# NingZhang1/pyscf_isdf

Hardware: AMD Instinct MI355X
Metric: isdf_build_plus_get_jk_wall_time (lower is better)
Workload: dtype f64

## Files before the change

include/mi355_isdf.h:

```cpp
#ifndef MI355_ISDF_H
#define MI355_ISDF_H

#include <stdint.h>

#ifdef __cplusplus
extern "C" {
#endif

typedef struct isdf_ctx* isdf_handle;

#define ISDF_OK 0
#define ISDF_ERR_ARG 1
#define ISDF_ERR_HIP 2
#define ISDF_ERR_LIB 3
#define ISDF_ERR_NUM 4

int isdf_abi_version(void);

int isdf_create(int device_id, isdf_handle* out);
int isdf_destroy(isdf_handle h);
int isdf_set_stream(isdf_handle h, void* hip_stream);
const char* isdf_last_error(isdf_handle h);
int64_t isdf_workspace_bytes(isdf_handle h);
int isdf_release_workspace(isdf_handle h);
// ... 65 lines not shown

int isdf_fit_prepare(isdf_handle h, const double* d_ao, int nao, int64_t ld,
                     const int64_t* d_ip, int P, double reg_rel, double* d_aoP, double* d_chol,
                     double* reg_used);
int isdf_fit_apply(isdf_handle h, const double* d_chol, const double* d_aoP, int P, int nao,
                   const double* d_ao, int64_t ng, int64_t ld, int forward_only,
                   double* d_theta, int64_t ldt);
int isdf_fit_prepare_cplx(isdf_handle h, const double* d_ao, int nao, int nh, int64_t ld,
                          const int64_t* d_ip, int P, double reg_rel, double* d_aoP, double* d_chol,
                          double* reg_used);
int isdf_fit_apply_cplx(isdf_handle h, const double* d_chol, const double* d_aoP, int P, int nao, int nh,
                        const double* d_ao, int64_t ng, int64_t ld, int forward_only,
                        double* d_theta, int64_t ldt);
int isdf_fit_global(isdf_handle h, const double* d_ao, int nao, int64_t ngrids, int64_t ld,
                    const int64_t* d_ip, int P, double reg_rel, double* d_theta, int64_t ldt,
                    double* d_aoP, double* reg_used);

int isdf_gather_aoP(isdf_handle h, const double* d_ao, int nao, int64_t ld, const int64_t* d_ip, int P,
                    double* d_aoP);
int isdf_gram_sq(isdf_handle h, const double* d_aoP, int P, int nao, int nh, double* d_A);
int isdf_pair_gram_rows(isdf_handle h, const double* d_aoP, int P, int nao, int nh, const double* d_ao,
                        int64_t ng, int64_t ld, double* d_B, int64_t ldb);
int isdf_block_chol(isdf_handle h, const double* d_A, int P, int nblk, const int32_t* blk_off,
                    double shift_rel, double* d_D, double* shift_used);
int isdf_block_solve(isdf_handle h, const double* d_D, int P, int nblk, const int32_t* blk_off, int side,
                     int trans, double* d_X, int64_t n, int64_t ldx);
int isdf_block_invert(isdf_handle h, const double* d_D, int P, int nblk, const int32_t* blk_off, double* d_Dinv);
int isdf_block_apply(isdf_handle h, const double* d_Dinv, int64_t ldd, int nblk, const int32_t* blk_off,
                     double* d_X, int64_t n, int64_t ldx);
int isdf_pair_rows_block_apply(isdf_handle h, const double* d_aoP, int P, int nao, const double* d_ao, int64_t ng,
                               int64_t ld, const double* d_Dinv, int64_t ldd, int nblk, const int32_t* blk_off,
                               double* d_B, int64_t ldb);
int isdf_pair_rows_squared(isdf_handle h, const double* d_aoP, int rows, int nao, const double* d_ao, int64_t ng,
                           int64_t ld, int* squared);
int isdf_pair_rows_frontier(isdf_handle h, const double* d_aoP, int nnew, int nao, const double* d_ao, int64_t ng,
                            int64_t ld, int squared, const double* d_Dinv, int64_t ldd, int nblk, const int32_t* blk_off,
                            double* d_B, int64_t ldb, int have);

int isdf_gram_prod(isdf_handle h, const double* d_aoP, int P, int nao, const double* d_psiP, int nocc, double* d_A);
int isdf_pair_prod_rows(isdf_handle h, const double* d_aoP, int P, int nao, const double* d_psiP, int nocc,
                        const double* d_ao, int64_t ld, const double* d_psi, int64_t ldpsi, int64_t ng,
                        double* d_B, int64_t ldb);
int isdf_factor_solve_half(isdf_handle h, const double* d_fac, int P, int backward, double* d_X, int64_t n, int64_t ldx);
int isdf_gram_prod_cplx(isdf_handle h, const double* d_aoP, int P, int nao, int nh, const double* d_psiP, int npsi, int npsi_h,
                        double* d_A);
int isdf_pair_prod_rows_cplx(isdf_handle h, const double* d_aoP, int P, int nao, int nh, const double* d_psiP, int npsi,
                             int npsi_h, const double* d_ao, int64_t ld, const double* d_psi, int64_t ldpsi, int64_t ng,
                             double* d_B, int64_t ldb);

int isdf_shift_diag(isdf_handle h, double* d_A, int P, double shift_rel);
int isdf_chol_inplace(isdf_handle h, double* d_A, int P, double shift_rel, double* d_scratch, double* reg_used);

int isdf_factor_solve(isdf_handle h, const double* d_fac, int P, double* d_X, int64_t n, int64_t ldx);

int isdf_bj_probe_vectors(isdf_handle h, double* d_T, int n, const double* d_fac, const double* d_D, int P,
                          int nblk, const int32_t* blk_off);
int isdf_rows_combine(isdf_handle h, const double* d_E, int n, int64_t ldE, int rows, const double* d_Y,
                      int64_t ng, int64_t ldy, double* d_F, int64_t ldf, int accumulate);

int isdf_bj_probe_rows(isdf_handle h, double* d_T, int n, const double* d_fac, const double* d_D, int P, int nblk,
                       const int32_t* blk_off, const double* d_Yp, int64_t ng, int64_t ldy, double* d_F, int64_t ldf);

int isdf_gather_T(isdf_handle h, const double* d_L, int k, int64_t ldL, const int64_t* d_piv,
                  double* d_T);
int isdf_W_from_factor(isdf_handle h, const double* d_F, int P, int kind, double* d_M, int64_t ldm);

int isdf_coulomb_W(isdf_handle h, const double* d_theta, int P, int64_t ldt,
                   const int32_t mesh[3], const double a[9],
                   int row0, int nrows, int batch, int upper_only, double* d_W, int64_t ldw);
int isdf_coulG_half(isdf_handle h, const int32_t mesh[3], const double a[9], double* d_out);
int isdf_spectral_supported(isdf_handle h, const int32_t mesh[3], int batch, int* ok);
int isdf_spectral_rows(isdf_handle h, const double* d_in, int nrows, int64_t ld, const int32_t mesh[3], const int32_t* d_idx,
                       const double* d_scale, int npts, int batch, double* d_out, int64_t ldx);
int isdf_coulomb_rows(isdf_handle h, const double* d_in, int nrows, int64_t ld,
                      const int32_t mesh[3], const double a[9], int batch, double* d_out, int64_t ldo);
int isdf_symmetrize_upper(isdf_handle h, double* d_W, int P, int64_t ldw);
int isdf_symmetrize_mean(isdf_handle h, double* d_W, int P, int64_t ldw, int antisymmetric);

int isdf_get_j(isdf_handle h, const double* d_ao, int nao, int64_t ngrids, int64_t ld,
               const int32_t mesh[3], const double a[9],
               const double* d_dm, int nset, double* d_vj);
int isdf_rho(isdf_handle h, const double* d_ao, int nao, int64_t ng, int64_t ld,
             const double* d_dm, int nset, double* d_rho, int64_t ldrho);
int isdf_coulomb_potential(isdf_handle h, double* d_rho_inout, int nset, int64_t ldrho,
                           const int32_t mesh[3], const double a[9]);
int isdf_vj_from_vR(isdf_handle h, const double* d_ao, int nao, int64_t ng, int64_t ld,
                    const double* d_vR, int nset, int64_t ldv, double* d_vj);

int isdf_get_k_exact(isdf_handle h, const double* d_ao, int nao, int64_t ngrids, int64_t ld,
                     const double* d_C, int nocc, const int32_t mesh[3], const double a[9],
                     int i0, int ni, int max_rows, double* d_vk);

int isdf_get_k(isdf_handle h, const double* d_aoP, int P, int nao,
               const double* d_W, int64_t ldw, int row0, int nrows,
               const double* d_dm, int nset, double* d_vk);

int isdf_coulG_q(isdf_handle h, const int32_t mesh[3], const double a[9], const double q[3], int wrap_around,
                 double omega, double* d_out);

int isdf_coulomb_Wq(isdf_handle h, const double* d_theta, int P, int64_t ldt, const int32_t mesh[3],
                    const double* d_coulG, double weight, int row0, int nrows, int batch,
                    int upper_only, double* d_Wre, double* d_Wim, int64_t ldw);
int isdf_symmetrize_hermitian(isdf_handle h, double* d_Wre, double* d_Wim, int P, int64_t ldw);
int isdf_finish_Wq(isdf_handle h, const double* d_Wre, const double* d_Wim, int P, int64_t ldw,
                   const double* d_phase, double* d_Wc);
int isdf_get_k_pair(isdf_handle h, const double* d_A1, const double* d_A2, const double* d_D2,
                    const double* d_Wq, int P, int nao, double scale, double* d_vk);

int isdf_get_k_exact_kpt(isdf_handle h, const double* d_u1r, const double* d_u1i, int nao, int64_t ld1,
                         const double* d_m2r, const double* d_m2i, int nocc, int64_t ld2, const int32_t mesh[3],
                         const double* d_coulG, double weight, int i0, int ni, int max_rows, double* d_vk_re,
                         double* d_vk_im);

int isdf_coulomb_rows_q(isdf_handle h, const double* d_rows, int nrows, int64_t ld, const int32_t mesh[3],
                        const double* d_coulG, double* d_re, double* d_im);
int isdf_nyquist_spectra(isdf_handle h, const double* d_rows, int nrows, int64_t ld, const int32_t mesh[3], int axis,
                         double* d_re, double* d_im);
int isdf_zhadamard_planes(isdf_handle h, double* d_Ar, double* d_Ai, int64_t lda, const double* d_Br, const double* d_Bi,
                          int64_t ldb, int rows, int64_t cols);
int isdf_rho_k(isdf_handle h, const double* d_ur, const double* d_ui, int nao, int64_t ng, int64_t ld,
               const double* d_DTr, const double* d_DTi, double scale, double* d_rho);
int isdf_vj_k(isdf_handle h, const double* d_ur, const double* d_ui, int nao, int64_t ng, int64_t ld,
              const double* d_vR, double* d_vj_re, double* d_vj_im);

int isdf_pp_local_potential(isdf_handle h, int natm, const double* coords, const double* pp_par,
                            const int32_t mesh[3], const double a[9], double* d_vlocR);
int isdf_pp_projector_overlaps(isdf_handle h, const int32_t* atm, int natm, const int32_t* bas, int nbas,
                               const double* env, int nenv, const double* coords, const double kpt[3],
                               const int32_t* proj_tab, const double* proj_rl, int nproj,
                               const int32_t mesh[3], const double a[9], double* d_out);

int isdf_pp_local_force(isdf_handle h, const double* d_rho, int nset, int64_t ldrho, int natm, const double* coords,
                        const double* pp_par, const int32_t mesh[3], const double a[9], double* d_out);
int isdf_pp_projector_overlaps_ip(isdf_handle h, const int32_t* atm, int natm, const int32_t* bas, int nbas,
                                  const double* env, int nenv, const double* coords, const double kpt[3],
                                  const int32_t* proj_tab, const double* proj_rl, int nproj,
                                  const int32_t mesh[3], const double a[9], double* d_out);
int isdf_rowdot3(isdf_handle h, int M, int64_t K, double alpha, const double* d_A, int64_t lda, int64_t astride, const double* d_s,
                 const double* d_B, int64_t ldb, int accumulate, double* d_out, int64_t ldo);

int isdf_gemm_nn(isdf_handle h, int M, int64_t N, int K, double alpha, const double* d_A, int64_t lda, const double* d_B,
                 int64_t ldb, double beta, double* d_C, int64_t ldc);
int isdf_hadamard_rows(isdf_handle h, double* d_X, int64_t ldx, const double* d_Y, int64_t ldy, int rows, int64_t cols);

int isdf_uniform_grid(isdf_handle h, const int32_t mesh[3], const double a[9], double* d_coords_soa);
int isdf_rho_pair(isdf_handle h, const double* d_aoA, int nA, const double* d_aoB, int nB, int64_t ng, int64_t ld,
                  const double* d_dm, int nset, double* d_rho, int64_t ldrho);
int isdf_mg_embed_density(isdf_handle h, const double* d_field, int nset, const int32_t mesh_sub[3], double scale,
                          double* d_spec, const int32_t mesh[3], int accumulate);
int isdf_mg_restrict_potential(isdf_handle h, const double* d_spec, int nset, const int32_t mesh[3],
                               const int32_t mesh_sub[3], double scale, double* d_field);
int isdf_mg_coulomb_kernel(isdf_handle h, double* d_spec, int nset, const int32_t mesh[3], const double a[9]);
int isdf_lda_exchange(isdf_handle h, const double* d_rho, int64_t n, double* d_exc, double* d_vxc);
int isdf_lda_vwn_add(isdf_handle h, const double* d_rho, int64_t n, double* d_exc, double* d_vxc);
int isdf_gga_b88(isdf_handle h, const double* d_rho, const double* d_grad, int64_t gstride, int64_t n, double* d_exc,
                 double* d_vrho, double* d_w, int64_t wstride);
int isdf_xc_fused(isdf_handle h, const double* d_rho, const double* d_grad, int64_t gstride, int64_t n, double c_slater, double c_b88,
                  double c_vwn, int vwn_rpa, double c_lyp, double* d_exc, double* d_vrho, double* d_w, int64_t wstride);
int isdf_gga_lyp_polarised(isdf_handle h, const double* d_rho, const double* d_grad, int64_t gcstride, int64_t sstride, int64_t n,
                           double weight, int accumulate, double* d_ec, double* d_vrho, double* d_w, int64_t wcstride,
                           int64_t osstride);
int isdf_lda_exchange_fxc(isdf_handle h, const double* d_rho, int64_t n, double* d_fxc);
int isdf_lda_vwn_fxc_add(isdf_handle h, const double* d_rho, int64_t n, double* d_fxc);
int isdf_gga_b88_fxc(isdf_handle h, const double* d_rho0, int64_t r0stride, int64_t n, const double* d_rho1, int64_t r1xstride,
                     int64_t r1nstride, int nset, double* d_wv, int64_t wxstride, int64_t wnstride, double* d_fxc, int64_t fstride);
int isdf_xc_fxc_apply(isdf_handle h, int nx, const double* d_fxc, int64_t fxstride, int64_t fystride, int64_t n, const double* d_rho1,
                      int64_t r1xstride, int64_t r1nstride, int nset, double* d_wv, int64_t wxstride, int64_t wnstride, int accumulate);
int isdf_dot(isdf_handle h, const double* d_x, const double* d_y, int64_t n, double* result);

int isdf_pack_table_pm(isdf_handle h, const double* d_tab, const int32_t mesh[3], const int32_t* d_idx, int npts, double scale,
                       double* d_s, double* d_a, int64_t ldx);
int isdf_herm_kscale_nt(isdf_handle h, int M, int N, int64_t K, double alpha, const double* d_A, int64_t lda, const double* d_B,
                        int64_t ldb, const double* d_s, const double* d_a, double beta, double* d_Cre, double* d_Cim, int64_t ldc);

int isdf_gemm_nt(isdf_handle h, int M, int N, int64_t K, double alpha, const double* d_A, int64_t lda,
                 const double* d_B, int64_t ldb, const double* d_kscale, double beta, double* d_C,
                 int64_t ldc);

int isdf_gemm_nt_had3(isdf_handle h, int M, int N, int64_t K, double alpha, const double* d_A, int64_t lda, const double* d_H,
                      int64_t ldh, const double* d_B, int64_t ldb, int64_t bstride, double beta, double* d_C, int64_t ldc,
                      int64_t cstride);

#ifdef __cplusplus
}
#endif
#endif
```

pyscf_isdf_amd/backend.py:

```python
import ctypes
import os
import numpy as np
import torch
from . import lib as _lib

_vp = ctypes.c_void_p


def _np_ptr(a):
    return a.ctypes.data_as(_vp)


class HipBackend:
    name = 'hip-gfx950'

    def __init__(self, device=0):
        if not torch.cuda.is_available():
            raise _lib.IsdfError('no GPU visible to torch; the ISDF path has no CPU fallback')
        self.device = torch.device('cuda', device)
        torch.cuda.set_device(self.device)
        self.handle = _lib.Handle(device)
        if os.environ.get('ISDF_TRSM') == 'subst':
            self.set_option('trsm_substitution', 1)
        if os.environ.get('ISDF_OWN_FFT') in ('0', '1', '2'):
# ... 330 lines not shown
                         len(blk_off) - 1, _np_ptr(blk_off))

    def rows_combine(self, E, Y, F, accumulate=False):
        self._stream()
        assert E.stride(1) == 1 and Y.stride(1) == 1 and F.stride(1) == 1 and E.shape[1] == Y.shape[0]
        self.handle.call('isdf_rows_combine', self._p(E), E.shape[0], E.stride(0), E.shape[1], self._p(Y), Y.shape[1],
                         Y.stride(0), self._p(F), F.stride(0), int(bool(accumulate)))

    def gather_T(self, L, k, piv, T):
        self._stream()
        assert T.is_contiguous() and T.shape == (k, k)
        self.handle.call('isdf_gather_T', self._p(L), int(k), L.stride(0), self._p(piv), self._p(T))

    def W_from_factor(self, F, kind, M):
        self._stream()
        assert F.is_contiguous()
        self.handle.call('isdf_W_from_factor', self._p(F), M.shape[0], int(kind), self._p(M), M.stride(0))

    def fit_global(self, ao, ngrids, ip, reg_rel, theta, aoP):
        self._stream()
        assert ip.dtype == torch.int64 and aoP.is_contiguous()
        reg = ctypes.c_double(0.0)
        self.handle.call('isdf_fit_global', self._p(ao), ao.shape[0], int(ngrids), ao.stride(0), self._p(ip),
                         ip.numel(), float(reg_rel), self._p(theta), theta.stride(0), self._p(aoP), ctypes.byref(reg))
        return reg.value

    def coulomb_W(self, theta, mesh, a, row0, nrows, batch, W, upper_only=False):
        self._stream()
        mesh = np.ascontiguousarray(mesh, dtype=np.int32)
        a = np.ascontiguousarray(a, dtype=np.float64)
        self.handle.call('isdf_coulomb_W', self._p(theta), theta.shape[0], theta.stride(0), _np_ptr(mesh), _np_ptr(a),
                         int(row0), int(nrows), int(batch), int(bool(upper_only)), self._p(W), W.stride(0))

    def coulomb_rows(self, rows, mesh, a, batch, out=None):
        self._stream()
        out = rows if out is None else out
        mesh = np.ascontiguousarray(mesh, dtype=np.int32)
        a = np.ascontiguousarray(a, dtype=np.float64)
        self.handle.call('isdf_coulomb_rows', self._p(rows), rows.shape[0], rows.stride(0), _np_ptr(mesh), _np_ptr(a),
                         int(batch), self._p(out), out.stride(0))

    def spectral_supported(self, mesh, batch=512):
        ok = ctypes.c_int(0)
        mesh = np.ascontiguousarray(mesh, dtype=np.int32)
        self.handle.call('isdf_spectral_supported', _np_ptr(mesh), int(batch), ctypes.byref(ok))
        return bool(ok.value)

    def coulG_half(self, mesh, a):
        self._stream()
        mesh = np.ascontiguousarray(mesh, dtype=np.int32)
        a = np.ascontiguousarray(a, dtype=np.float64)
        out = self.empty((int(mesh[0]) * int(mesh[1]) * (int(mesh[2]) // 2 + 1),))
        self.handle.call('isdf_coulG_half', _np_ptr(mesh), _np_ptr(a), self._p(out))
        return self.to_host(out).reshape(int(mesh[0]), int(mesh[1]), int(mesh[2]) // 2 + 1)

    def spectral_rows(self, rows, mesh, idx, scale, out, batch=512):
        self._stream()
        mesh = np.ascontiguousarray(mesh, dtype=np.int32)
        assert rows.is_contiguous() and out.stride(1) == 1 and idx.dtype == torch.int32 and out.stride(0) % 2 == 0
        self.handle.call('isdf_spectral_rows', self._p(rows), rows.shape[0], rows.stride(0), _np_ptr(mesh), self._p(idx),
                         self._p(scale), int(idx.numel()), int(batch), self._p(out), out.stride(0))

    def symmetrize_upper(self, W):
        self._stream()
        self.handle.call('isdf_symmetrize_upper', self._p(W), W.shape[0], W.stride(0))

    def symmetrize_mean(self, W, antisymmetric=False):
        self._stream()
        self.handle.call('isdf_symmetrize_mean', self._p(W), W.shape[0], W.stride(0), int(bool(antisymmetric)))

    def get_j(self, ao, ngrids, mesh, a, dm, vj):
        self._stream()
        mesh = np.ascontiguousarray(mesh, dtype=np.int32)
        a = np.ascontiguousarray(a, dtype=np.float64)
        assert dm.is_contiguous() and vj.is_contiguous()
        self.handle.call('isdf_get_j', self._p(ao), ao.shape[0], int(ngrids), ao.stride(0), _np_ptr(mesh), _np_ptr(a),
                         self._p(dm), dm.shape[0], self._p(vj))

    def rho(self, ao, ng, dm, rho):
        self._stream()
        self.handle.call('isdf_rho', self._p(ao), ao.shape[0], int(ng), ao.stride(0), self._p(dm), dm.shape[0],
                         self._p(rho), rho.stride(0))

    def coulomb_potential(self, rho, mesh, a):
        self._stream()
        mesh = np.ascontiguousarray(mesh, dtype=np.int32)
        a = np.ascontiguousarray(a, dtype=np.float64)
        self.handle.call('isdf_coulomb_potential', self._p(rho), rho.shape[0], rho.stride(0), _np_ptr(mesh), _np_ptr(a))

    def vj_from_vR(self, ao, ng, vR, vj):
        self._stream()
        self.handle.call('isdf_vj_from_vR', self._p(ao), ao.shape[0], int(ng), ao.stride(0), self._p(vR), vR.shape[0],
                         vR.stride(0), self._p(vj))

    def get_k(self, aoP, W, row0, nrows, dm, vk):
        self._stream()
        assert aoP.is_contiguous() and dm.is_contiguous() and vk.is_contiguous()
        self.handle.call('isdf_get_k', self._p(aoP), aoP.shape[0], aoP.shape[1], self._p(W), W.stride(0), int(row0),
                         int(nrows), self._p(dm), dm.shape[0], self._p(vk))

    def get_k_exact(self, ao, ngrids, C, mesh, a, i0, ni, max_rows, vk):
        self._stream()
        mesh = np.ascontiguousarray(mesh, dtype=np.int32)
        a = np.ascontiguousarray(a, dtype=np.float64)
        assert C.is_contiguous() and vk.is_contiguous()
        self.handle.call('isdf_get_k_exact', self._p(ao), ao.shape[0], int(ngrids), ao.stride(0), self._p(C), C.shape[1],
                         _np_ptr(mesh), _np_ptr(a), int(i0), int(ni), int(max_rows), self._p(vk))

    def gemm_nn(self, A, B, C, alpha=1.0, beta=0.0):
        self._stream()
        self.handle.call('isdf_gemm_nn', A.shape[0], B.shape[1], A.shape[1], float(alpha), self._p(A), A.stride(0), self._p(B),
                         B.stride(0), float(beta), self._p(C), C.stride(0))

    def hadamard_rows(self, X, Y):
        self._stream()
        self.handle.call('isdf_hadamard_rows', self._p(X), X.stride(0), self._p(Y), Y.stride(0), X.shape[0], X.shape[1])

    def gemm_nt(self, A, B, C, alpha=1.0, beta=0.0, kscale=None):
        self._stream()
        M, K = A.shape
        N = B.shape[0]
        assert B.shape[1] == K and tuple(C.shape) == (M, N) and A.stride(1) == 1 and B.stride(1) == 1 and C.stride(1) == 1
        ks = self._p(kscale) if kscale is not None else _vp(0)
        self.handle.call('isdf_gemm_nt', M, N, K, float(alpha), self._p(A), A.stride(0), self._p(B), B.stride(0), ks,
                         float(beta), self._p(C), C.stride(0))

    def gemm_nt_had3(self, A, H, B3, C3, alpha=1.0, beta=0.0):
        self._stream()
        M, K = A.shape
        N = B3.shape[1]
        assert tuple(B3.shape) == (3, N, K) and tuple(C3.shape) == (3, M, N) and A.stride(1) == 1 and B3.stride(2) == 1 and C3.stride(2) == 1
        assert H is None or (tuple(H.shape) == (M, K) and H.stride(1) == 1)
        self.handle.call('isdf_gemm_nt_had3', M, N, K, float(alpha), self._p(A), A.stride(0), self._p(H) if H is not None else _vp(0),
                         H.stride(0) if H is not None else 0, self._p(B3), B3.stride(1), B3.stride(0), float(beta), self._p(C3),
                         C3.stride(1), C3.stride(0))

    def pack_table_pm(self, table, mesh, idx, scale, s, a):
        self._stream()
        mesh = np.ascontiguousarray(mesh, dtype=np.int32)
        assert idx.dtype == torch.int32 and table.is_contiguous() and table.numel() == int(np.prod(mesh))
        assert s.is_contiguous() and a.is_contiguous() and s.numel() == a.numel()
        self.handle.call('isdf_pack_table_pm', self._p(table), _np_ptr(mesh), self._p(idx), int(idx.numel()), float(scale),
                         self._p(s), self._p(a), int(s.numel()))

    def herm_kscale_nt(self, A, B, s, a, Cre, Cim, alpha=1.0, beta=0.0):
        self._stream()
        M, K = A.shape
        N = B.shape[0]
        assert B.shape[1] == K and tuple(Cre.shape) == (M, N) and tuple(Cim.shape) == (M, N) and Cre.stride() == Cim.stride()
        assert A.stride(1) == 1 and B.stride(1) == 1 and Cre.stride(1) == 1 and s.numel() >= K and a.numel() >= K
        self.handle.call('isdf_herm_kscale_nt', M, N, K, float(alpha), self._p(A), A.stride(0), self._p(B), B.stride(0),
                         self._p(s), self._p(a), float(beta), self._p(Cre), self._p(Cim), Cre.stride(0))

    def uniform_grid(self, mesh, a):
        self._stream()
        mesh = np.ascontiguousarray(mesh, dtype=np.int32)
        a = np.ascontiguousarray(a, dtype=np.float64)
        out = self.empty((3, int(np.prod(mesh))))
        self.handle.call('isdf_uniform_grid', _np_ptr(mesh), _np_ptr(a), self._p(out))
        return out

    def rho_pair(self, aoA, aoB, ng, dm, rho):
        self._stream()
        assert aoA.stride(0) == aoB.stride(0) and aoA.stride(1) == 1 and aoB.stride(1) == 1 and dm.is_contiguous()
        assert tuple(dm.shape[1:]) == (aoA.shape[0], aoB.shape[0])
        self.handle.call('isdf_rho_pair', self._p(aoA), aoA.shape[0], self._p(aoB), aoB.shape[0], int(ng), aoA.stride(0),
                         self._p(dm), dm.shape[0], self._p(rho), rho.stride(0))

    def mg_embed_density(self, field, mesh_sub, scale, spec, mesh, accumulate=True):
        self._stream()
        mesh_sub = np.ascontiguousarray(mesh_sub, dtype=np.int32)
        mesh = np.ascontiguousarray(mesh, dtype=np.int32)
        assert field.is_contiguous() and spec.is_contiguous() and spec.dtype == torch.complex128
        assert field.shape[1] == int(np.prod(mesh_sub)) and spec.shape[1] == int(mesh[0]) * int(mesh[1]) * (int(mesh[2]) // 2 + 1)
        self.handle.call('isdf_mg_embed_density', self._p(field), field.shape[0], _np_ptr(mesh_sub), float(scale), self._p(spec),
                         _np_ptr(mesh), int(bool(accumulate)))

    def mg_restrict_potential(self, spec, mesh, mesh_sub, scale, field):
        self._stream()
        mesh_sub = np.ascontiguousarray(mesh_sub, dtype=np.int32)
        mesh = np.ascontiguousarray(mesh, dtype=np.int32)
        assert field.is_contiguous() and spec.is_contiguous() and spec.dtype == torch.complex128
        assert field.shape[1] == int(np.prod(mesh_sub)) and spec.shape[1] == int(mesh[0]) * int(mesh[1]) * (int(mesh[2]) // 2 + 1)
        self.handle.call('isdf_mg_restrict_potential', self._p(spec), spec.shape[0], _np_ptr(mesh), _np_ptr(mesh_sub), float(scale),
                         self._p(field))

    def mg_coulomb_kernel(self, spec, mesh, a):
        self._stream()
        mesh = np.ascontiguousarray(mesh, dtype=np.int32)
        a = np.ascontiguousarray(a, dtype=np.float64)
        assert spec.is_contiguous() and spec.dtype == torch.complex128
        self.handle.call('isdf_mg_coulomb_kernel', self._p(spec), spec.shape[0], _np_ptr(mesh), _np_ptr(a))

    def lda_exchange(self, rho, exc, vxc):
        self._stream()
        assert rho.is_contiguous() and exc.is_contiguous() and vxc.is_contiguous()
        self.handle.call('isdf_lda_exchange', self._p(rho), rho.numel(), self._p(exc), self._p(vxc))

    def lda_vwn_add(self, rho, exc, vxc):
        self._stream()
        assert rho.is_contiguous() and exc.is_contiguous() and vxc.is_contiguous()
        self.handle.call('isdf_lda_vwn_add', self._p(rho), rho.numel(), self._p(exc), self._p(vxc))

    def gga_b88(self, rho, grad, exc, vrho, w):
        self._stream()
        assert rho.is_contiguous() and exc.is_contiguous() and vrho.is_contiguous() and grad.stride(1) == 1 and w.stride(1) == 1
        self.handle.call('isdf_gga_b88', self._p(rho), self._p(grad), grad.stride(0), rho.numel(), self._p(exc), self._p(vrho),
# ... 203 lines not shown
```

pyscf_isdf_amd/csrc/common.h:

```cpp
#pragma once
#include <hip/hip_runtime.h>
#include <rocblas/rocblas.h>
#include <rocsolver/rocsolver.h>
#include <hipfft/hipfft.h>
#include <cstdint>
#include <cstdio>
#include <cstring>
#include <string>
#include <vector>
#include <map>
#include "../../include/mi355_isdf.h"

struct FftPlan {
  hipfftHandle fwd = 0, bwd = 0;
  size_t work_bytes = 0;
};

struct ProfRec {
  hipEvent_t e0 = nullptr, e1 = nullptr;
};
struct ProfEntry {
  std::vector<ProfRec> recs;
  double work = 0.0;
  double ms = 0.0;
  int64_t launches = 0;
};

struct WsKernel {
  double alpha = 0.0;
  double ak[9] = {0};
  int mesh[3] = {0, 0, 0};
  double maxq[3] = {0, 0, 0};
  const double* vq = nullptr;
};

struct isdf_ctx {
  int profiling = 0;
  std::map<std::string, ProfEntry> prof;
  int device = 0;
  hipStream_t stream = nullptr;
  rocblas_handle blas = nullptr;
  std::string err;
  std::map<std::vector<int>, FftPlan> plans;
  std::map<std::string, std::pair<void*, size_t>> ws;
  int num_cu = 256;
  int trsm_substitution = 0;
  int own_fft = 2;
  int gemm_nn_own = 0;
  int attr_gemm_b = 0, attr_gemm_nn = 0, attr_gram_tri = 0, attr_herm = 0;
  int cand_gram = 1;
  int conv_pipe = 1;
  int conv_sub_rows = 0;
  int gram_pivot_tpb = 256;
  int gram_compact = 1;
  int gram_compact_permille = 875;
  int block_apply_waves = 16;
  int block_apply_reg = 1;
  double coul_omega = 0.0;
  double coul_rc = 0.0;
  int coul_sphere = 0;
  WsKernel wsk;
};

int isdf_fail(isdf_handle h, int code, const char* fmt, ...);
void* isdf_ws(isdf_handle h, const char* name, size_t bytes);
int isdf_get_plan(isdf_handle h, const int32_t mesh[3], int batch, FftPlan** out);
int get_coulG_half(isdf_handle h, const int32_t mesh[3], const double a[9], double extra_scale, double** out);
bool conv_rows_own_supported(const int32_t mesh[3], int nb);
bool conv_rows_q_own_supported(isdf_handle h, const int32_t mesh[3], int nb);
bool spectral_rows_own_supported(isdf_handle h, const int32_t mesh[3], int nb);
int spectral_rows_own(isdf_handle h, const double* d_in, int nb, const int32_t mesh[3], const int32_t* d_idx, const double* d_scale,
                      int npts, double* d_out, int64_t ldx, HIP_vector_type<double, 2u>* zbuf);
int conv_rows_q_own(isdf_handle h, const double* d_in, double* d_re, double* d_im, int nb, const int32_t mesh[3], const double* tab,
                    double2* zhalf, double2* zfull);
int conv_rows_own(isdf_handle h, const double* d_in, double* d_out, int nb, const int32_t mesh[3], const double* cg,
                  double2* zbuf);

#define HIP_TRY(h, expr)                                                                    \
  do {                                                                                      \
    hipError_t e_ = (expr);                                                                 \
    if (e_ != hipSuccess)                                                                   \
      return isdf_fail(h, ISDF_ERR_HIP, "%s:%d %s -> %s", __FILE__, __LINE__, #expr,        \
                       hipGetErrorString(e_));                                              \
  } while (0)
#define BLAS_TRY(h, expr)                                                                   \
  do {                                                                                      \
    rocblas_status s_ = (expr);                                                             \
    if (s_ != rocblas_status_success)                                                       \
      return isdf_fail(h, ISDF_ERR_LIB, "%s:%d %s -> rocblas status %d", __FILE__, __LINE__, \
                       #expr, (int)s_);                                                     \
  } while (0)
#define FFT_TRY(h, expr)                                                                    \
  do {                                                                                      \
    hipfftResult r_ = (expr);                                                               \
    if (r_ != HIPFFT_SUCCESS)                                                               \
      return isdf_fail(h, ISDF_ERR_LIB, "%s:%d %s -> hipfft result %d", __FILE__, __LINE__,  \
                       #expr, (int)r_);                                                     \
  } while (0)
#define KERNEL_CHECK(h) HIP_TRY(h, hipGetLastError())
#define ARG_CHECK(h, cond)                                                                  \
  do {                                                                                      \
    if (!(cond)) return isdf_fail(h, ISDF_ERR_ARG, "%s:%d argument check failed: %s",       \
                                  __FILE__, __LINE__, #cond);                               \
  } while (0)

static inline int64_t cdiv(int64_t a, int64_t b) { return (a + b - 1) / b; }

struct ProfScope {
  isdf_handle h;
  ProfRec rec;
  ProfEntry* ent = nullptr;
  ProfScope(isdf_handle h_, const char* name, double work, int64_t launches = 1) : h(h_) {
    if (!h || !h->profiling) return;
    ent = &h->prof[name];
    ent->work += work;
    ent->launches += launches;
    if (hipEventCreate(&rec.e0) != hipSuccess || hipEventCreate(&rec.e1) != hipSuccess) { ent = nullptr; return; }
    (void)hipEventRecord(rec.e0, h->stream);
  }
  ~ProfScope() {
    if (!ent) return;
    (void)hipEventRecord(rec.e1, h->stream);
    ent->recs.push_back(rec);
  }
};

int gemm_nt_f64(isdf_handle h, int M, int N, int64_t K, double alpha, const double* A, int64_t lda,
                const double* B, int64_t ldb, double beta, double* C, int64_t ldc);
int gemm_nt_f64_scaled(isdf_handle h, int M, int N, int64_t K, double alpha, const double* A, int64_t lda,
                       const double* B, int64_t ldb, const double* kscale, double beta, double* C,
                       int64_t ldc);
int trsm_lower_left(isdf_handle h, bool trans, int m, int64_t n, const double* L, int64_t ldl, double* X, int64_t ldx);
int trsm_lower_right(isdf_handle h, bool trans, int m, int64_t n, const double* L, int64_t ldl, double* X, int64_t ldx);
int block_forward_solve(isdf_handle h, const double* D, int64_t ldd, int nblk, const int32_t* blk_off_host, double* X,
                        int64_t ldx, int64_t n);
int block_apply_inverse(isdf_handle h, const double* Dinv, int64_t ldd, int nblk, const int32_t* blk_off_host, double* X,
                        int64_t ldx, int64_t n, bool square_input = false);
int transpose_rm(isdf_handle h, const double* src, int64_t lds, int64_t rows, int64_t cols, double* dst, int64_t ldd);
int tri_left(isdf_handle h, bool trans, int m, int64_t n, const double* L, int64_t ldl, double* X, int64_t ldx);
int tri_right(isdf_handle h, bool trans, int m, int64_t n, const double* L, int64_t ldl, double* X, int64_t ldx);
bool gemm_nn_f64_supported(isdf_handle h, int64_t M, int64_t N, int64_t K, const double* A, int64_t lda, const double* B,
                           int64_t ldb);
int gemm_nn_f64(isdf_handle h, int64_t M, int64_t N, int64_t K, const double* A, int64_t lda, const double* B, int64_t ldb,
                double* C, int64_t ldc, bool square);
int gemm_rm(isdf_handle h, char opA, char opB, int64_t M, int64_t N, int64_t K, double alpha,
            const double* A, int64_t lda, const double* B, int64_t ldb, double beta, double* C,
            int64_t ldc);

__host__ __device__ inline int64_t gram_tri_row(int64_t r) {
  const int64_t tm = r >> 8;
  return 32768 * tm * (tm + 1) + (r & 255) * ((tm + 1) << 8);
}
static inline int64_t gram_tri_size(int64_t m) { return m > 0 ? gram_tri_row(m - 1) + (((m - 1) >> 8) + 1) * 256 : 0; }
struct GramTriUnit { int blk, tm, tn, pad; };
int gram_tri_blocks(isdf_handle h, const double* X, int64_t ldx, int K, const GramTriUnit* d_units, int64_t nunits,
                    const int64_t* d_blk_off, int64_t row0, const int64_t* d_tri_off, double* S, double flop);
```

pyscf_isdf_amd/csrc/coulomb.hip:

```cpp
#include "common.h"

namespace {

struct Recip { double b[9]; };
__device__ inline double g2_of(int ix, int iy, int iz, int n0, int n1, int n2, const Recip& r) {
  const double fx = (ix < (n0 + 1) / 2) ? ix : ix - n0;
  const double fy = (iy < (n1 + 1) / 2) ? iy : iy - n1;
  const double fz = (iz < (n2 + 1) / 2) ? iz : iz - n2;
  const double gx = fx * r.b[0] + fy * r.b[3] + fz * r.b[6];
  const double gy = fx * r.b[1] + fy * r.b[4] + fz * r.b[7];
  const double gz = fx * r.b[2] + fy * r.b[5] + fz * r.b[8];
  return gx * gx + gy * gy + gz * gz;
}

__device__ inline double range_factor(double g2, double omega) {
  if (omega == 0.0) return 1.0;
  const double e = exp(-0.25 * g2 / (omega * omega));
  return omega > 0.0 ? e : 1.0 - e;
}
__device__ inline double kernel_value(double g2, double omega, double rc) {
  const double fourpi = 4.0 * 3.14159265358979323846;
  if (rc > 0.0) return g2 == 0.0 ? 0.5 * fourpi * rc * rc : fourpi / g2 * (1.0 - cos(sqrt(g2) * rc));
  return g2 == 0.0 ? 0.0 : fourpi / g2 * range_factor(g2, omega);
}
// ... 151 lines not shown
  if (rc) return rc;
  double qf[3];
  for (int i = 0; i < 3; ++i)
    qf[i] = (q[0] * a[3 * i] + q[1] * a[3 * i + 1] + q[2] * a[3 * i + 2]) / (2.0 * 3.14159265358979323846);
  const bool nonzero = fabs(q[0]) + fabs(q[1]) + fabs(q[2]) > 1e-9;
  const int wrap = (wrap_around && nonzero) ? 1 : 0;
  if (wrap)
    for (int i = 0; i < 3; ++i)
      if (fabs(rint(qf[i] / (mesh[i] / 2 + 0.5) * 1e9)) >= 1e9)
        return isdf_fail(h, ISDF_ERR_ARG, "isdf_coulG_q: q lies outside the first FFT box (pyscf/pbc/tools/pbc.py:281)");
  if (!nonzero) qf[0] = qf[1] = qf[2] = 0.0;
  const int64_t G = (int64_t)mesh[0] * mesh[1] * mesh[2];
  hipLaunchKernelGGL(coulG_q_kernel, dim3((unsigned)cdiv(G, 256)), dim3(256), 0, h->stream, d_out, mesh[0], mesh[1],
                     mesh[2], rr, qf[0], qf[1], qf[2], wrap, omega, h->coul_rc, h->wsk);
  KERNEL_CHECK(h);
  return ISDF_OK;
}

static int convolve_rows(isdf_handle h, const double* d_in, double* d_out, int nb, const int32_t mesh[3],
                         const double* cg, double2* zbuf) {
  const int64_t gc = (int64_t)mesh[0] * mesh[1] * (mesh[2] / 2 + 1);
  if (h->own_fft && conv_rows_own_supported(mesh, nb)) return conv_rows_own(h, d_in, d_out, nb, mesh, cg, zbuf);
  FftPlan* plan = nullptr;
  int rc = isdf_get_plan(h, mesh, nb, &plan);
  if (rc) return rc;
  const int64_t Gfull = (int64_t)mesh[0] * mesh[1] * mesh[2];
  ProfScope ps(h, "coulomb_conv_d2z_mul_z2d[byte]", 32.0 * (double)Gfull * nb, 3);
  FFT_TRY(h, hipfftExecD2Z(plan->fwd, (hipfftDoubleReal*)d_in, (hipfftDoubleComplex*)zbuf));
  const int64_t total = gc * nb;
  const unsigned nblocks = (unsigned)std::min<int64_t>(cdiv(total, 256), (int64_t)h->num_cu * 16);
  hipLaunchKernelGGL(mul_half_kernel, dim3(nblocks), dim3(256), 0, h->stream, zbuf, cg, gc, total);
  KERNEL_CHECK(h);
  FFT_TRY(h, hipfftExecZ2D(plan->bwd, (hipfftDoubleComplex*)zbuf, (hipfftDoubleReal*)d_out));
  return ISDF_OK;
}

namespace {
__global__ void mirror_upper_kernel(double* __restrict__ W, int P, int64_t ldw) {
  __shared__ double tile[32][33];
  const int bx = blockIdx.x, by = blockIdx.y;
  if (bx < by) return;
  const int tx = threadIdx.x, ty = threadIdx.y;
  for (int i = ty; i < 32; i += 8) {
    const int r = by * 32 + i, cc = bx * 32 + tx;
    tile[i][tx] = (r < P && cc < P) ? W[(int64_t)r * ldw + cc] : 0.0;
  }
  __syncthreads();
  for (int i = ty; i < 32; i += 8) {
    const int r = bx * 32 + i, cc = by * 32 + tx;
    if (r < P && cc < P && r > cc) W[(int64_t)r * ldw + cc] = tile[tx][i];
  }
}
__global__ void mean_symmetric_kernel(double* __restrict__ W, int P, int64_t ldw, double sign) {
  __shared__ double up[32][33], lo[32][33];
  const int bx = blockIdx.x, by = blockIdx.y;
  if (bx < by) return;
  const int tx = threadIdx.x, ty = threadIdx.y;
  for (int i = ty; i < 32; i += 8) {
    const int r = by * 32 + i, cc = bx * 32 + tx;
    up[i][tx] = (r < P && cc < P) ? W[(int64_t)r * ldw + cc] : 0.0;
    const int r2 = bx * 32 + i, c2 = by * 32 + tx;
    lo[i][tx] = (r2 < P && c2 < P) ? W[(int64_t)r2 * ldw + c2] : 0.0;
  }
  __syncthreads();
  for (int i = ty; i < 32; i += 8) {
    const int r = by * 32 + i, cc = bx * 32 + tx;
    if (r < P && cc < P) W[(int64_t)r * ldw + cc] = 0.5 * (up[i][tx] + sign * lo[tx][i]);
    const int r2 = bx * 32 + i, c2 = by * 32 + tx;
    if (bx != by && r2 < P && c2 < P) W[(int64_t)r2 * ldw + c2] = 0.5 * (lo[i][tx] + sign * up[tx][i]);
  }
}
}

extern "C" int isdf_symmetrize_mean(isdf_handle h, double* d_W, int P, int64_t ldw, int antisymmetric) {
  if (!h) return ISDF_ERR_ARG;
  ARG_CHECK(h, d_W && P > 0 && ldw >= P);
  const unsigned nt = (unsigned)cdiv(P, 32);
  hipLaunchKernelGGL(mean_symmetric_kernel, dim3(nt, nt), dim3(32, 8), 0, h->stream, d_W, P, ldw,
                     antisymmetric ? -1.0 : 1.0);
  KERNEL_CHECK(h);
  return ISDF_OK;
}

extern "C" int isdf_symmetrize_upper(isdf_handle h, double* d_W, int P, int64_t ldw) {
  if (!h) return ISDF_ERR_ARG;
  ARG_CHECK(h, d_W && P > 0 && ldw >= P);
  const unsigned nt = (unsigned)cdiv(P, 32);
  hipLaunchKernelGGL(mirror_upper_kernel, dim3(nt, nt), dim3(32, 8), 0, h->stream, d_W, P, ldw);
  KERNEL_CHECK(h);
  return ISDF_OK;
}

extern "C" int isdf_coulomb_W(isdf_handle h, const double* d_theta, int P, int64_t ldt,
                              const int32_t mesh[3], const double a[9], int row0, int nrows,
                              int batch, int upper_only, double* d_W, int64_t ldw) {
  if (!h) return ISDF_ERR_ARG;
  ARG_CHECK(h, d_theta && mesh && a && d_W && P > 0 && batch > 0 && ldw >= P);
  ARG_CHECK(h, row0 >= 0 && nrows >= 0 && row0 + nrows <= P);
  const int64_t G = (int64_t)mesh[0] * mesh[1] * mesh[2];
  const int64_t gc = (int64_t)mesh[0] * mesh[1] * (mesh[2] / 2 + 1);
  ARG_CHECK(h, ldt == G);
  if (nrows == 0) return ISDF_OK;
  if (batch > nrows) batch = nrows;
  double* cg = nullptr;
  int rc = get_coulG_half(h, mesh, a, 1.0, &cg);
  if (rc) return rc;
  double* V = (double*)isdf_ws(h, "coul_V", sizeof(double) * (size_t)batch * G);
  double2* Z = (double2*)isdf_ws(h, "coul_Z", sizeof(double2) * (size_t)batch * gc);
  if (!V || !Z) return ISDF_ERR_HIP;
  const double det = a[0] * (a[4] * a[8] - a[5] * a[7]) - a[1] * (a[3] * a[8] - a[5] * a[6]) +
                     a[2] * (a[3] * a[7] - a[4] * a[6]);
  const double w = fabs(det) / (double)G;
  for (int r = row0; r < row0 + nrows; r += batch) {
    const int nb = std::min(batch, row0 + nrows - r);
    rc = convolve_rows(h, d_theta + (int64_t)r * ldt, V, nb, mesh, cg, Z);
    if (rc) return rc;
    const int c0 = upper_only ? r : 0;
    rc = gemm_nt_f64(h, nb, P - c0, G, w, V, G, d_theta + (int64_t)c0 * ldt, ldt, 0.0,
                     d_W + (int64_t)r * ldw + c0, ldw);
    if (rc) return rc;
  }
  return ISDF_OK;
}

extern "C" int isdf_coulomb_potential(isdf_handle h, double* d_rho, int nset, int64_t ldrho,
                                      const int32_t mesh[3], const double a[9]) {
  if (!h) return ISDF_ERR_ARG;
  ARG_CHECK(h, d_rho && mesh && a && nset > 0);
  const int64_t G = (int64_t)mesh[0] * mesh[1] * mesh[2];
  const int64_t gc = (int64_t)mesh[0] * mesh[1] * (mesh[2] / 2 + 1);
  ARG_CHECK(h, ldrho == G);
  const double det = a[0] * (a[4] * a[8] - a[5] * a[7]) - a[1] * (a[3] * a[8] - a[5] * a[6]) +
                     a[2] * (a[3] * a[7] - a[4] * a[6]);
  double* cg = nullptr;
  int rc = get_coulG_half(h, mesh, a, fabs(det) / (double)G, &cg);
  if (rc) return rc;
  double2* Z = (double2*)isdf_ws(h, "coul_Z", sizeof(double2) * (size_t)nset * gc);
  if (!Z) return ISDF_ERR_HIP;
  return convolve_rows(h, d_rho, d_rho, nset, mesh, cg, Z);
}

extern "C" int isdf_coulomb_rows(isdf_handle h, const double* d_in, int nrows, int64_t ld,
                                 const int32_t mesh[3], const double a[9], int batch, double* d_out,
                                 int64_t ldo) {
  if (!h) return ISDF_ERR_ARG;
  ARG_CHECK(h, d_in && d_out && mesh && a && nrows >= 0 && batch > 0);
  const int64_t G = (int64_t)mesh[0] * mesh[1] * mesh[2];
  const int64_t gc = (int64_t)mesh[0] * mesh[1] * (mesh[2] / 2 + 1);
  ARG_CHECK(h, ld == G && ldo == G);
  if (nrows == 0) return ISDF_OK;
  if (batch > nrows) batch = nrows;
  double* cg = nullptr;
  int rc = get_coulG_half(h, mesh, a, 1.0, &cg);
  if (rc) return rc;
  double2* Z = (double2*)isdf_ws(h, "coul_Z", sizeof(double2) * (size_t)batch * gc);
  if (!Z) return ISDF_ERR_HIP;
  for (int r = 0; r < nrows; r += batch) {
    const int nb = std::min(batch, nrows - r);
    rc = convolve_rows(h, d_in + (int64_t)r * ld, d_out + (int64_t)r * ldo, nb, mesh, cg, Z);
    if (rc) return rc;
  }
  return ISDF_OK;
}

extern "C" int isdf_coulG_half(isdf_handle h, const int32_t mesh[3], const double a[9], double* d_out) {
  if (!h) return ISDF_ERR_ARG;
  ARG_CHECK(h, mesh && a && d_out);
  double* cg = nullptr;
  int rc = get_coulG_half(h, mesh, a, 1.0, &cg);
  if (rc) return rc;
  const int64_t gc = (int64_t)mesh[0] * mesh[1] * (mesh[2] / 2 + 1);
  HIP_TRY(h, hipMemcpyAsync(d_out, cg, sizeof(double) * gc, hipMemcpyDeviceToDevice, h->stream));
  return ISDF_OK;
}

extern "C" int isdf_spectral_supported(isdf_handle h, const int32_t mesh[3], int batch, int* ok) {
  if (!h) return ISDF_ERR_ARG;
  ARG_CHECK(h, mesh && ok && batch > 0);
  *ok = spectral_rows_own_supported(h, mesh, batch) ? 1 : 0;
  return ISDF_OK;
}

extern "C" int isdf_spectral_rows(isdf_handle h, const double* d_in, int nrows, int64_t ld, const int32_t mesh[3],
                                  const int32_t* d_idx, const double* d_scale, int npts, int batch, double* d_out, int64_t ldx) {
  if (!h) return ISDF_ERR_ARG;
  ARG_CHECK(h, d_in && d_out && mesh && d_idx && d_scale && nrows >= 0 && batch > 0 && npts > 0);
  const int64_t G = (int64_t)mesh[0] * mesh[1] * mesh[2];
  const int64_t gc = (int64_t)mesh[0] * mesh[1] * (mesh[2] / 2 + 1);
  ARG_CHECK(h, ld == G && npts <= gc);
  if (nrows == 0) return ISDF_OK;
  if (batch > nrows) batch = nrows;
  if (!spectral_rows_own_supported(h, mesh, batch))
    return isdf_fail(h, ISDF_ERR_ARG, "isdf_spectral_rows: mesh %d x %d x %d is not covered by the plane FFT", mesh[0], mesh[1], mesh[2]);
  double2* Z = (double2*)isdf_ws(h, "coul_Z", sizeof(double2) * (size_t)batch * gc);
  if (!Z) return ISDF_ERR_HIP;
  for (int r = 0; r < nrows; r += batch) {
    const int nb = std::min(batch, nrows - r);
    int rc = spectral_rows_own(h, d_in + (int64_t)r * ld, nb, mesh, d_idx, d_scale, npts, d_out + (int64_t)r * ldx, ldx, Z);
    if (rc) return rc;
  }
  return ISDF_OK;
}
// ... 1 lines not shown
```

pyscf_isdf_amd/csrc/fft_conv.hip:

```cpp
#include "common.h"
#include <type_traits>

namespace {

constexpr int TPB = 256;
constexpr int MAXSTAGE = 12;

struct Axis {
  int n;
  int nstage;
  int radix[MAXSTAGE];
  const double2* tw;
};

__device__ inline double2 cadd(double2 a, double2 b) { return make_double2(a.x + b.x, a.y + b.y); }
__device__ inline double2 csub(double2 a, double2 b) { return make_double2(a.x - b.x, a.y - b.y); }
__device__ inline double2 cmul(double2 a, double2 b) { return make_double2(a.x * b.x - a.y * b.y, a.x * b.y + a.y * b.x); }
template <int SIGN>
__device__ inline double2 mul_si(double2 a) { return SIGN > 0 ? make_double2(-a.y, a.x) : make_double2(a.y, -a.x); }
template <int SIGN>
__device__ inline double2 twid(const double2* __restrict__ tw, int idx) {
  double2 w = tw[idx];
  if (SIGN > 0) w.y = -w.y;
  return w;
// ... 390 lines not shown
      z = stockham_all<1>(z, (z == x) ? y : x, ax, ZC, M);
    }
  }
  for (int c = threadIdx.x; c < n * ZC; c += TPB) {
    const int e = c / ZC, m = c - e * ZC;
    if (m < M) base[(int64_t)e * es + m] = z[c];
  }
}

template <int SIGN, int ZCT>
__device__ inline void fft_fast(double2* buf, const Axis& ax, int Ls, const double2* tw) {
  fft<SIGN, TPB, 2048 / TPB, true, FixedLines<ZCT>>(buf, ax, Ls, ZCT, tw);
}

template <int ZCT>
__global__ __launch_bounds__(TPB) void z_r2c_fast_kernel(const double* __restrict__ in, double2* __restrict__ out,
                                                         int64_t nlines, Axis ax) {
  extern __shared__ double2 lds[];
  const int n = ax.n, nh = n / 2 + 1;
  constexpr int Ls = ZCT + 1;
  double2* x = lds;
  double2* tw = lds + n * Ls;
  for (int k = threadIdx.x; k < n; k += TPB) tw[k] = ax.tw[k];
  const int64_t line0 = (int64_t)blockIdx.x * 2 * ZCT;
  const int nl = (int)min((int64_t)2 * ZCT, nlines - line0);
  const double* src = in + line0 * n;
  const float inv_n = 1.0f / (float)n;
  for (int c = threadIdx.x; c < 2 * ZCT * n; c += TPB) {
    const int l = (int)(((float)c + 0.5f) * inv_n), e = c - l * n;
    const double v = (l < nl) ? src[c] : 0.0;
    ((double*)(x + e * Ls + (l >> 1)))[l & 1] = v;
  }
  __syncthreads();
  fft_fast<-1, ZCT>(x, ax, Ls, tw);
  double2* dstc = out + line0 * nh;
  const float inv_nh = 1.0f / (float)nh;
  for (int c = threadIdx.x; c < nl * nh; c += TPB) {
    const int l = (int)(((float)c + 0.5f) * inv_nh), k = c - l * nh;
    const int m = l >> 1;
    const double2 zk = x[k * Ls + m];
    const double2 zn = x[(k == 0 ? 0 : n - k) * Ls + m];
    double2 r;
    if ((l & 1) == 0) r = make_double2(0.5 * (zk.x + zn.x), 0.5 * (zk.y - zn.y));
    else r = make_double2(0.5 * (zk.y + zn.y), -0.5 * (zk.x - zn.x));
    dstc[c] = r;
  }
}

template <int ZCT>
__global__ __launch_bounds__(TPB) void z_c2r_fast_kernel(const double2* __restrict__ in, double* __restrict__ out,
                                                         int64_t nlines, Axis ax) {
  extern __shared__ double2 lds[];
  const int n = ax.n, nh = n / 2 + 1;
  constexpr int Ls = ZCT + 1;
  double2* x = lds;
  double2* tw = lds + n * Ls;
  for (int k = threadIdx.x; k < n; k += TPB) tw[k] = ax.tw[k];
  const int64_t line0 = (int64_t)blockIdx.x * 2 * ZCT;
  const int nl = (int)min((int64_t)2 * ZCT, nlines - line0);
  const int M = (nl + 1) / 2;
  const double2* src = in + line0 * nh;
  const float inv_nh = 1.0f / (float)nh;
  for (int c = threadIdx.x; c < M * nh; c += TPB) {
    const int m = (int)(((float)c + 0.5f) * inv_nh), k = c - m * nh;
    double2 a = src[(int64_t)(2 * m) * nh + k];
    double2 b = (2 * m + 1 < nl) ? src[(int64_t)(2 * m + 1) * nh + k] : make_double2(0.0, 0.0);
    const bool selfconj = (k == 0) || (2 * k == n);
    if (selfconj) { a.y = 0.0; b.y = 0.0; }
    x[k * Ls + m] = make_double2(a.x - b.y, a.y + b.x);
    if (!selfconj) x[(n - k) * Ls + m] = make_double2(a.x + b.y, -a.y + b.x);
  }
  __syncthreads();
  fft_fast<1, ZCT>(x, ax, Ls, tw);
  double* dst = out + line0 * n;
  const float inv_n = 1.0f / (float)n;
  for (int c = threadIdx.x; c < nl * n; c += TPB) {
    const int l = (int)(((float)c + 0.5f) * inv_n), e = c - l * n;
    dst[c] = ((const double*)(x + e * Ls + (l >> 1)))[l & 1];
  }
}

template <int MODE, int ZCT>
__global__ __launch_bounds__(TPB) void strided_fft_fast_kernel(double2* __restrict__ data, int64_t os, int64_t es, int Mtot,
                                                               Axis ax, int ntile, const double* __restrict__ table) {
  extern __shared__ double2 lds[];
  const int n = ax.n;
  double2* x = lds;
  double2* tw = lds + n * ZCT;
  for (int k = threadIdx.x; k < n; k += TPB) tw[k] = ax.tw[k];
  const int nouter = gridDim.x / ntile;
  const int64_t outer = (MODE == 2) ? blockIdx.x % nouter : blockIdx.x / ntile;
  const int m0 = (int)((MODE == 2) ? blockIdx.x / nouter : blockIdx.x % ntile) * ZCT;
  const int M = min(ZCT, Mtot - m0);
  double2* base = data + outer * os + m0;
  for (int c = threadIdx.x; c < n * ZCT; c += TPB) {
    const int e = c / ZCT, m = c & (ZCT - 1);
    if (m < M) x[c] = base[(int64_t)e * es + m];
  }
  __syncthreads();
  if (MODE == 1) {
    fft_fast<1, ZCT>(x, ax, ZCT, tw);
  } else {
    fft_fast<-1, ZCT>(x, ax, ZCT, tw);
    if (MODE == 2) {
      const double* tb = table + m0;
      for (int c = threadIdx.x; c < n * ZCT; c += TPB) {
        const int e = c / ZCT, m = c & (ZCT - 1);
        if (m < M) {
          const double g = tb[(int64_t)e * es + m];
          double2 v = x[c];
          v.x *= g;
          v.y *= g;
          x[c] = v;
        }
      }
      __syncthreads();
      fft_fast<1, ZCT>(x, ax, ZCT, tw);
    }
  }
  for (int c = threadIdx.x; c < n * ZCT; c += TPB) {
    const int e = c / ZCT, m = c & (ZCT - 1);
    if (m < M) base[(int64_t)e * es + m] = x[c];
  }
}

constexpr int TPBP = 1024;
constexpr int PLANE_ENTRIES = 10240;
constexpr int PIPE_NT = 768;

template <int SIGN, int NT, int N, int RA, int RB, int MMAX>
__device__ __forceinline__ void fft_plane_fixed(double2* buf, int Ls, int M, const double2* tw) {
  static_assert(RA * RB == N, "two stages");
  stage<SIGN, RA, NT, ((N / RA) * MMAX + NT - 1) / NT, true, AnyLines>(buf, N, N, 1, Ls, M, tw, opaque_tid());
  stage<SIGN, RB, NT, ((N / RB) * MMAX + NT - 1) / NT, true, AnyLines>(buf, N, N / RA, RA, Ls, M, tw, opaque_tid());
}

struct PlaneAny {
  static constexpr int NT = TPBP, PER = PLANE_ENTRIES / TPBP;
  static constexpr int KS_HALF = PER, KS_PAIR = PER / 2 + 1, KS_FULL = PER;
  int n1, n2, n2h, npair;
  __device__ PlaneAny(const Axis& az, const Axis& ay) : n1(ay.n), n2(az.n), n2h(az.n / 2 + 1), npair((ay.n + 1) / 2) {}
  __device__ static int tid() { return threadIdx.x; }
  template <int SIGN, bool FULL>
  __device__ __forceinline__ static void transform(double2* buf, const Axis& ax, int Ls, int M, const double2* tw) {
    fft<SIGN, NT, PER, false, AnyLines>(buf, ax, Ls, M, tw);
  }
};
template <int N, int RA, int RB>
struct PlaneSquare {
  static constexpr int NT = PIPE_NT, n1 = N, n2 = N, n2h = N / 2 + 1, npair = (N + 1) / 2;
  static constexpr int KS_HALF = (n1 * n2h + NT - 1) / NT, KS_PAIR = (npair * n2h + NT - 1) / NT, KS_FULL = (N * N + NT - 1) / NT;
  constexpr PlaneSquare() = default;
  __device__ static int tid() { return opaque_tid(); }
  template <int SIGN, bool FULL>
  __device__ __forceinline__ static void transform(double2* buf, const Axis&, int Ls, int M, const double2* tw) {
    fft_plane_fixed<SIGN, NT, N, RA, RB, FULL ? N : N / 2 + 1>(buf, Ls, M, tw);
  }
};

__device__ inline double zero_of(const double*) { return 0.0; }
__device__ inline double2 zero_of(const double2*) { return make_double2(0.0, 0.0); }
template <int NT, int NPRE, class T>
__device__ __forceinline__ void prefetch(T (&pre)[NPRE], const T* __restrict__ src, int count, int tid) {
#pragma unroll
  for (int u = 0; u < NPRE; ++u) {
    const int c = tid + u * NT;
    pre[u] = c < count ? src[c] : zero_of(src);
  }
// ... 319 lines not shown
    static const int big[] = {16, 15, 12, 10, 9, 8, 6, 5, 4, 3, 2};
    int best[MAXSTAGE], nbest = MAXSTAGE + 1, bestmax = 1 << 30;
    int cur[MAXSTAGE];
    struct Rec {
      static void go(int rest, int maxr, int depth, int* cur, int* best, int& nbest, int& bestmax) {
        if (rest == 1) {
          const int mx = depth ? cur[0] : 1;
          if (depth < nbest || (depth == nbest && mx < bestmax)) {
            nbest = depth; bestmax = mx;
            for (int i = 0; i < depth; ++i) best[i] = cur[i];
          }
          return;
        }
        if (depth + 1 > nbest || depth >= MAXSTAGE) return;
        for (int r : big)
          if (r <= maxr && rest % r == 0) { cur[depth] = r; go(rest / r, r, depth + 1, cur, best, nbest, bestmax); }
      }
    };
    Rec::go(n, 16, 0, cur, best, nbest, bestmax);
    if (nbest <= MAXSTAGE) {
      ax->nstage = nbest;
      for (int i = 0; i < nbest; ++i) ax->radix[i] = best[i];
      return true;
    }
  }
  const int order[4] = {4, 2, 3, 5};
  for (int r : order)
    while (n % r == 0 && n > 1) {
      if (ax->nstage >= MAXSTAGE) return false;
      ax->radix[ax->nstage++] = r;
      n /= r;
    }
  for (int p = 7; n > 1 && p <= 13; p += 2)
    while (n % p == 0) {
      if (ax->nstage >= MAXSTAGE) return false;
      ax->radix[ax->nstage++] = p;
      n /= p;
    }
  return n == 1;
}

int make_axes(isdf_handle h, const int32_t mesh[3], Axis ax[3], const char* who) {
  for (int d = 0; d < 3; ++d) {
    if (!factorise(mesh[d], &ax[d])) return isdf_fail(h, ISDF_ERR_ARG, "%s: unsupported mesh dimension %d", who, mesh[d]);
    char name[32];
    snprintf(name, sizeof(name), "fft_tw_%d", mesh[d]);
    const bool fresh = h->ws.find(name) == h->ws.end();
    double2* tw = (double2*)isdf_ws(h, name, sizeof(double2) * (size_t)mesh[d]);
    if (!tw) return ISDF_ERR_HIP;
    if (fresh) {
      std::vector<double2> host(mesh[d]);
      for (int k = 0; k < mesh[d]; ++k) {
        const double t = -2.0 * 3.14159265358979323846 * (double)k / (double)mesh[d];
        host[k] = make_double2(cos(t), sin(t));
      }
      HIP_TRY(h, hipMemcpyAsync(tw, host.data(), sizeof(double2) * (size_t)mesh[d], hipMemcpyHostToDevice, h->stream));
      HIP_TRY(h, hipStreamSynchronize(h->stream));
    }
    ax[d].tw = tw;
  }
  return ISDF_OK;
}

template <bool FWD, class IN, class OUT>
void launch_z(isdf_handle h, bool fast, int L, const IN* in, OUT* out, int64_t nlines, const Axis& ax) {
  const dim3 grid((unsigned)cdiv(nlines, 2 * L));
  const size_t n = ax.n;
  if (fast) {
    const size_t lds = sizeof(double2) * (n * (L + 1) + n);
    with_lines(L, [&](auto z) {
      constexpr int ZCT = decltype(z)::value;
      if constexpr (FWD) z_r2c_fast_kernel<ZCT><<<grid, dim3(TPB), lds, h->stream>>>(in, out, nlines, ax);
      else z_c2r_fast_kernel<ZCT><<<grid, dim3(TPB), lds, h->stream>>>(in, out, nlines, ax);
    });
  } else {
    const size_t lds = sizeof(double2) * 2 * n * (L + 1);
    if constexpr (FWD) z_r2c_kernel<<<grid, dim3(TPB), lds, h->stream>>>(in, out, nlines, ax, L);
    else z_c2r_kernel<<<grid, dim3(TPB), lds, h->stream>>>(in, out, nlines, ax, L);
  }
}

template <int MODE>
void launch_strided(isdf_handle h, bool fast, int L, double2* data, int64_t nouter, int64_t os, int64_t es, int Mtot, const Axis& ax,
                    const double* table) {
  const int nt = (int)cdiv(Mtot, L);
  const dim3 grid((unsigned)(nouter * nt));
  const size_t n = ax.n;
  if (fast)
    with_lines(L, [&](auto z) {
      strided_fft_fast_kernel<MODE, decltype(z)::value><<<grid, dim3(TPB), sizeof(double2) * (n * L + n), h->stream>>>(
          data, os, es, Mtot, ax, nt, table);
    });
  else
    strided_fft_kernel<MODE><<<grid, dim3(TPB), sizeof(double2) * 2 * n * L, h->stream>>>(data, os, es, Mtot, ax, L, nt, table);
}

#define ISDF_PLANE_SIZES(X) X(64, 8, 8) X(72, 9, 8) X(80, 10, 8) X(96, 12, 8) X(100, 10, 10) X(108, 12, 9) X(120, 12, 10)
constexpr int PIPE_ANY = 1024, PIPE_Q_MAX = 96;

template <class F>
bool with_pipe_size(isdf_handle h, const Axis& az, const Axis& ay, int nmax, F f) {
  if (h->conv_pipe == 0 || ay.n != az.n || ay.n > nmax || ay.nstage != 2) return false;
#define ISDF_PLANE_SIZE(NN, RA, RB)                                \
  if (ay.n == NN && ay.radix[0] == RA && ay.radix[1] == RB) {      \
    f(PlaneSquare<NN, RA, RB>{});                                  \
    return true;                                                   \
  }
  ISDF_PLANE_SIZES(ISDF_PLANE_SIZE)
#undef ISDF_PLANE_SIZE
  return false;
}

template <class K>
int raise_lds(isdf_handle h, K kernel) {
  HIP_TRY(h, hipFuncSetAttribute((const void*)kernel, hipFuncAttributeMaxDynamicSharedMemorySize, LDS_MAX));
  return ISDF_OK;
}
dim3 pipe_grid(isdf_handle h, int nplanes) { return dim3((unsigned)std::min<int64_t>(nplanes, h->num_cu)); }

int launch_plane_fwd(isdf_handle h, const double* in, double2* out, const Axis* ax, const PlaneGeo& g, int nplanes, int pipe_max) {
  int rc = ISDF_OK;
  const bool piped = with_pipe_size(h, ax[2], ax[1], pipe_max, [&](auto d) {
    auto kernel = plane_fwd_pipe_kernel<decltype(d)>;
    if ((rc = raise_lds(h, kernel)) == ISDF_OK)
      kernel<<<pipe_grid(h, nplanes), dim3(PIPE_NT), g.bytes, h->stream>>>(in, out, ax[2], ax[1], g.Lz, g.bufsz, nplanes);
  });
  if (!piped && (rc = raise_lds(h, plane_fwd_kernel)) == ISDF_OK)
    plane_fwd_kernel<<<dim3((unsigned)nplanes), dim3(TPBP), g.bytes, h->stream>>>(in, out, ax[2], ax[1], g.Lz, g.bufsz);
  return rc;
}

int launch_plane_inv(isdf_handle h, const double2* in, double* out, const Axis* ax, const PlaneGeo& g, int nplanes, int pipe_max) {
  int rc = ISDF_OK;
  const bool piped = with_pipe_size(h, ax[2], ax[1], pipe_max, [&](auto d) {
    auto kernel = plane_inv_pipe_kernel<decltype(d)>;
    if ((rc = raise_lds(h, kernel)) == ISDF_OK)
      kernel<<<pipe_grid(h, nplanes), dim3(PIPE_NT), g.bytes, h->stream>>>(in, out, ax[2], ax[1], g.Lz, g.bufsz, nplanes);
  });
  if (!piped && (rc = raise_lds(h, plane_inv_kernel)) == ISDF_OK)
    plane_inv_kernel<<<dim3((unsigned)nplanes), dim3(TPBP), g.bytes, h->stream>>>(in, out, ax[2], ax[1], g.Lz, g.bufsz);
  return rc;
}

int launch_plane_c2c_inv(isdf_handle h, const double2* in, double* out_re, double* out_im, const Axis* ax, const PlaneGeo& g,
                         int nplanes) {
  int rc = ISDF_OK;
  const bool piped = with_pipe_size(h, ax[2], ax[1], PIPE_Q_MAX, [&](auto d) {
    if constexpr (decltype(d)::n1 <= PIPE_Q_MAX) {
      auto kernel = plane_c2c_inv_pipe_kernel<decltype(d)>;
      if ((rc = raise_lds(h, kernel)) == ISDF_OK)
        kernel<<<pipe_grid(h, nplanes), dim3(PIPE_NT), g.bytes, h->stream>>>(in, out_re, out_im, ax[2], ax[1], g.Lz, g.bufsz, nplanes);
    } else {
      rc = isdf_fail(h, ISDF_ERR_ARG, "launch_plane_c2c_inv: no pipelined kernel for %d^2", (int)decltype(d)::n1);
    }
  });
  if (!piped && (rc = raise_lds(h, plane_c2c_inv_kernel)) == ISDF_OK)
    plane_c2c_inv_kernel<<<dim3((unsigned)nplanes), dim3(TPBP), g.bytes, h->stream>>>(in, out_re, out_im, ax[2], ax[1], g.Lz, g.bufsz);
  return rc;
}

}

bool conv_rows_own_supported(const int32_t mesh[3], int nb) {
  if (nb < 1 || (int64_t)nb * mesh[0] * mesh[1] * 4 >= 2147483647LL || (int64_t)nb * mesh[1] * (mesh[2] / 2 + 1) >= 2147483647LL)
    return false;
  for (int d = 0; d < 3; ++d) {
    Axis ax;
    if (mesh[d] < 1 || mesh[d] > 1024 || !factorise(mesh[d], &ax)) return false;
    if (lines_per_tile(mesh[d], d == 2 ? 1 : 0) < 1) return false;
  }
  return true;
}

int conv_rows_own(isdf_handle h, const double* d_in, double* d_out, int nb, const int32_t mesh[3], const double* cg,
                  double2* zbuf) {
  const int n0 = mesh[0], n1 = mesh[1], n2 = mesh[2], n2h = n2 / 2 + 1;
  Axis ax[3];
  if (int rc = make_axes(h, mesh, ax, "conv_rows_own")) return rc;
  const int64_t gc = (int64_t)n0 * n1 * n2h;
  const int64_t nlines = (int64_t)nb * n0 * n1;
  ARG_CHECK(h, nlines * 4 < 2147483647LL && (int64_t)nb * cdiv((int64_t)n1 * n2h, 1) < 2147483647LL);
  const int LP = lines_per_tile(n2, 1);
  const int ZY = lines_per_tile(n1, 0), ZX = lines_per_tile(n0, 0);
  if (LP < 1 || ZY < 1 || ZX < 1) return isdf_fail(h, ISDF_ERR_ARG, "conv_rows_own: mesh too large for the LDS tiles");
  const int64_t G = (int64_t)n0 * n1 * n2;
  const int FZ = fast_lines(n2), FY = fast_lines(n1), FX = fast_lines(n0);
  const bool smooth = smooth235(ax[0]) && smooth235(ax[1]) && smooth235(ax[2]);
  const PlaneGeo geo = (h->own_fft == 2 && smooth && FX >= 1) ? plane_geometry(n1, n2, false) : PlaneGeo{0, 0, 0};
  ProfScope ps(h, geo.bytes ? "coulomb_conv_own_3pass[byte]" : "coulomb_conv_own_5pass[byte]", 32.0 * (double)G * nb,
               geo.bytes ? 3 : 5);
  if (geo.bytes) {
    const int sub = h->conv_sub_rows > 0 ? std::min(nb, h->conv_sub_rows) : nb;
    for (int r0 = 0; r0 < nb; r0 += sub) {
      const int nr = std::min(sub, nb - r0);
      double2* zb = zbuf + (int64_t)r0 * gc;
      const int nplanes = (int)((int64_t)nr * n0);
      if (int rc = launch_plane_fwd(h, d_in + (int64_t)r0 * G, zb, ax, geo, nplanes, PIPE_ANY)) return rc;
      launch_strided<2>(h, true, FX, zb, nr, gc, (int64_t)n1 * n2h, n1 * n2h, ax[0], cg);
      if (int rc = launch_plane_inv(h, zb, d_out + (int64_t)r0 * G, ax, geo, nplanes, PIPE_ANY)) return rc;
    }
    KERNEL_CHECK(h);
    return ISDF_OK;
  }
  const bool fast = smooth && FZ >= 1 && FY >= 1 && FX >= 1;
  const int Lz = fast ? FZ : LP, Ly = fast ? FY : ZY, Lx = fast ? FX : ZX;
  launch_z<true>(h, fast, Lz, d_in, zbuf, nlines, ax[2]);
  launch_strided<0>(h, fast, Ly, zbuf, (int64_t)nb * n0, (int64_t)n1 * n2h, (int64_t)n2h, n2h, ax[1], nullptr);
  launch_strided<2>(h, fast, Lx, zbuf, nb, gc, (int64_t)n1 * n2h, n1 * n2h, ax[0], cg);
  launch_strided<1>(h, fast, Ly, zbuf, (int64_t)nb * n0, (int64_t)n1 * n2h, (int64_t)n2h, n2h, ax[1], nullptr);
  launch_z<false>(h, fast, Lz, zbuf, d_out, nlines, ax[2]);
  KERNEL_CHECK(h);
  return ISDF_OK;
}

__global__ void spectral_pack_kernel(const double2* __restrict__ z, int64_t gc, const int32_t* __restrict__ idx,
                                     const double* __restrict__ scale, int npts, double2* __restrict__ out, int64_t ldx2) {
  const int64_t j = (int64_t)blockIdx.x * blockDim.x + threadIdx.x;
  if (j >= ldx2) return;
  const int row = blockIdx.y;
  double2 v = make_double2(0.0, 0.0);
  if (j < npts) {
    const double2 t = z[(int64_t)row * gc + idx[j]];
    const double s = scale[j];
    v = make_double2(t.x * s, t.y * s);
  }
  out[(int64_t)row * ldx2 + j] = v;
}

bool spectral_rows_own_supported(isdf_handle h, const int32_t mesh[3], int nb) {
  if (h->own_fft != 2 || !conv_rows_own_supported(mesh, nb)) return false;
  Axis ax[3];
  for (int d = 0; d < 3; ++d)
    if (!factorise(mesh[d], &ax[d]) || !smooth235(ax[d])) return false;
  return fast_lines(mesh[0]) >= 1 && plane_geometry(mesh[1], mesh[2], false).bytes != 0;
}

int spectral_rows_own(isdf_handle h, const double* d_in, int nb, const int32_t mesh[3], const int32_t* d_idx,
                      const double* d_scale, int npts, double* d_out, int64_t ldx, double2* zbuf) {
  const int n0 = mesh[0], n1 = mesh[1], n2 = mesh[2], n2h = n2 / 2 + 1;
  Axis ax[3];
  if (int rc = make_axes(h, mesh, ax, "spectral_rows_own")) return rc;
  const int64_t gc = (int64_t)n0 * n1 * n2h;
  const PlaneGeo geo = plane_geometry(n1, n2, false);
  const int FX = fast_lines(n0);
  ARG_CHECK(h, geo.bytes && FX >= 1 && (int64_t)nb * n0 < 2147483647LL && nb <= 65535 && (ldx & 1) == 0 && ldx >= 2 * (int64_t)npts);
  ProfScope ps(h, "spectral_rows_own[byte]", (8.0 * (double)n0 * n1 * n2 + 8.0 * (double)ldx) * nb, 3);
  if (int rc = launch_plane_fwd(h, d_in, zbuf, ax, geo, (int)((int64_t)nb * n0), PIPE_ANY)) return rc;
  launch_strided<0>(h, true, FX, zbuf, nb, gc, (int64_t)n1 * n2h, n1 * n2h, ax[0], nullptr);
  const int64_t ldx2 = ldx / 2;
  spectral_pack_kernel<<<dim3((unsigned)cdiv(ldx2, 256), (unsigned)nb), dim3(256), 0, h->stream>>>(zbuf, gc, d_idx, d_scale, npts,
                                                                                                  (double2*)d_out, ldx2);
  KERNEL_CHECK(h);
  return ISDF_OK;
}

bool conv_rows_q_own_supported(isdf_handle h, const int32_t mesh[3], int nb) {
  if (!h->own_fft) return false;
  if (nb < 1 || nb > 65535 || (int64_t)nb * mesh[0] >= 2147483647LL) return false;
  Axis ax[3];
  for (int d = 0; d < 3; ++d)
    if (mesh[d] < 2 || mesh[d] > 1024 || !factorise(mesh[d], &ax[d]) || !smooth235(ax[d])) return false;
  return fast_lines(mesh[0]) >= 1 && plane_geometry(mesh[1], mesh[2], false).bytes && plane_geometry(mesh[1], mesh[2], true).bytes;
}

int conv_rows_q_own(isdf_handle h, const double* d_in, double* d_re, double* d_im, int nb, const int32_t mesh[3],
                    const double* tab, double2* zhalf, double2* zfull) {
  const int n0 = mesh[0], n1 = mesh[1], n2 = mesh[2], n2h = n2 / 2 + 1;
  Axis ax[3];
  if (int rc = make_axes(h, mesh, ax, "conv_rows_q_own")) return rc;
  const int64_t G = (int64_t)n0 * n1 * n2, gc = (int64_t)n0 * n1 * n2h;
  const PlaneGeo geo_r = plane_geometry(n1, n2, false), geo_c = plane_geometry(n1, n2, true);
  const int FX = fast_lines(n0);
  ARG_CHECK(h, geo_r.bytes && geo_c.bytes && FX >= 1 && (int64_t)nb * n0 < 2147483647LL && nb <= 65535);
  ProfScope ps(h, "coulomb_conv_q_own[byte]", 64.0 * (double)G * nb, 5);
  const int nplanes = (int)((int64_t)nb * n0);
  if (int rc = launch_plane_fwd(h, d_in, zhalf, ax, geo_r, nplanes, PIPE_Q_MAX)) return rc;
  launch_strided<0>(h, true, FX, zhalf, nb, gc, (int64_t)n1 * n2h, n1 * n2h, ax[0], nullptr);
  expand_mul_kernel<<<dim3((unsigned)cdiv(G, 256), (unsigned)nb), dim3(256), 0, h->stream>>>(zhalf, zfull, tab, n0, n1, n2,
                                                                                            1.0 / (double)G);
  launch_strided<1>(h, true, FX, zfull, nb, G, (int64_t)n1 * n2, n1 * n2, ax[0], nullptr);
  if (int rc = launch_plane_c2c_inv(h, zfull, d_re, d_im, ax, geo_c, nplanes)) return rc;
  KERNEL_CHECK(h);
  return ISDF_OK;
}
```

pyscf_isdf_amd/csrc/gemm_f64.hip:

```cpp
#include "common.h"
#include <cstdlib>

int gemm_rm(isdf_handle h, char opA, char opB, int64_t M, int64_t N, int64_t K, double alpha,
            const double* A, int64_t lda, const double* B, int64_t ldb, double beta, double* C,
            int64_t ldc) {
  ARG_CHECK(h, M < 2147483647LL && N < 2147483647LL && K < 2147483647LL && lda < 2147483647LL &&
                   ldb < 2147483647LL && ldc < 2147483647LL);
  const rocblas_operation ta = (opA == 'N') ? rocblas_operation_none : rocblas_operation_transpose;
  const rocblas_operation tb = (opB == 'N') ? rocblas_operation_none : rocblas_operation_transpose;
  ProfScope ps(h, "rocblas_dgemm[flop]", 2.0 * M * N * (double)K);
  BLAS_TRY(h, rocblas_dgemm(h->blas, tb, ta, (rocblas_int)N, (rocblas_int)M, (rocblas_int)K, &alpha, B,
                            (rocblas_int)ldb, A, (rocblas_int)lda, &beta, C, (rocblas_int)ldc));
  return ISDF_OK;
}

namespace {

typedef double d4 __attribute__((ext_vector_type(4)));

constexpr int BM = 128, BN = 128, BK = 16;
constexpr int LDT = 17;
constexpr int TPB = 256;

struct GemmArgs {
  const double* A; int64_t lda;
  const double* B; int64_t ldb;
  const double* kscale;
  double* P;
  int64_t ldp, slab_stride;
  int M, N;
  int64_t K, kslab;
  int ntm, ntn, nslab;
  int64_t nunits, nunits_pad;
  double alpha, beta;
  int direct;
};

__device__ __forceinline__ int64_t xcd_unit(int64_t nunits_pad) {
  const int64_t bid = blockIdx.x;
  const int64_t per_xcd = nunits_pad / 8;
  return (bid % 8) * per_xcd + bid / 8;
}

struct Tile { int tm, tn, slab; };
struct KRange { int64_t k0, k1; };

__device__ __forceinline__ Tile decode_tile(int64_t unit, int ntm, int ntn) {
  return {(int)(unit % ntm), (int)((unit / ntm) % ntn), (int)(unit / ((int64_t)ntm * ntn))};
}

__device__ __forceinline__ KRange slab_range(int slab, int64_t kslab, int64_t K) {
  const int64_t k0 = (int64_t)slab * kslab;
  return {k0, (k0 + kslab < K) ? k0 + kslab : K};
}

#define ISDF_STORE_ACC(NI, NJ, ROW0, COL0, M, N, STORE)                                       \
  _Pragma("unroll") for (int i = 0; i < NI; ++i) {                                            \
    _Pragma("unroll") for (int r = 0; r < 4; ++r) {                                           \
      const int row = ROW0 + i * 16 + (lane >> 4) + 4 * r;                                    \
      if (row >= M) continue;                                                                 \
      _Pragma("unroll") for (int j = 0; j < NJ; ++j) {                                        \
        const int col = COL0 + j * 16 + (lane & 15);                                          \
        if (col >= N) continue;                                                               \
        STORE                                                                                 \
      }                                                                                       \
    }                                                                                         \
  }
#define ISDF_SLAB_STORE                                                                       \
  {                                                                                           \
    double* q = out + (int64_t)row * g.ldp + col;                                             \
    const double v = acc[i][j][r];                                                            \
    if (g.direct) *q = (g.beta == 0.0) ? g.alpha * v : g.alpha * v + g.beta * (*q);           \
    else *q = v;                                                                              \
  }

#define ISDF_MFMA16(AF, BF)                                                                   \
    _Pragma("unroll") for (int i = 0; i < 4; ++i)                                             \
      _Pragma("unroll") for (int j = 0; j < 4; ++j)                                           \
        acc[i][j] = __builtin_amdgcn_mfma_f64_16x16x4f64(AF[i], BF[j], acc[i][j], 0, 0, 0);
#define ISDF_ISSUE(XMASK, NX) _Pragma("unroll") for (int q_ = 0; q_ < 8; ++q_) {              \
    __builtin_amdgcn_sched_group_barrier(0x008, 2, 0); __builtin_amdgcn_sched_group_barrier(0x100, 1, 0);                \
    if (q_ < (NX)) __builtin_amdgcn_sched_group_barrier(XMASK, 1, 0); }

template <bool FAST>
__global__ __launch_bounds__(TPB, 2) void gemm_nt_mfma_kernel(GemmArgs g) {
  __shared__ double sA[2][BM * LDT];
  __shared__ double sB[2][BN * LDT];

  const int64_t unit = xcd_unit(g.nunits_pad);
  if (unit >= g.nunits) return;
  const Tile t = decode_tile(unit, g.ntm, g.ntn);
  const KRange kr = slab_range(t.slab, g.kslab, g.K);
  const int64_t k0 = kr.k0, k1 = kr.k1;
  const int nchunks = (int)((k1 - k0 + BK - 1) / BK);

  const int tid = threadIdx.x;
  const int lane = tid & 63, wave = tid >> 6;
  const int wm = wave >> 1, wn = wave & 1;

  const int srow = tid >> 3;
  const int sseg = tid & 7;
  const int arow0 = t.tm * BM + srow, brow0 = t.tn * BN + srow;
  const int mlast = g.M - 1, nlast = g.N - 1;
  const double* __restrict__ Ag = g.A;
  const double* __restrict__ Bg = g.B;
  const int64_t lda = g.lda, ldb = g.ldb;

  double2 ra0, ra1, ra2, ra3, rb0, rb1, rb2, rb3;
#define ISDF_LOAD_ONE(I, RA, RB)                                                              \
  {                                                                                           \
    const int ra = min(arow0 + 32 * I, mlast), rb = min(brow0 + 32 * I, nlast);               \
    const double* pa = Ag + (int64_t)ra * lda + k;                                            \
    const double* pb = Bg + (int64_t)rb * ldb + k;                                            \
    if (FAST) {                                                                               \
      RA = *reinterpret_cast<const double2*>(pa);                                             \
      RB = *reinterpret_cast<const double2*>(pb);                                             \
    } else {                                                                                  \
      RA.x = v0 ? pa[0] : 0.0; RA.y = v1 ? pa[1] : 0.0;                                       \
      RB.x = v0 ? pb[0] : 0.0; RB.y = v1 ? pb[1] : 0.0;                                       \
    }                                                                                         \
    RB.x *= s0; RB.y *= s1;                                                                   \
  }
#define ISDF_LOAD_CHUNK(C)                                                                    \
  {                                                                                           \
    const int64_t k = k0 + (int64_t)(C) * BK + sseg * 2;                                      \
    const bool v0 = FAST || (k < k1), v1 = FAST || (k + 1 < k1);                              \
    double s0 = 1.0, s1 = 1.0;                                                                \
    if (g.kscale) { if (v0) s0 = g.kscale[k]; if (v1) s1 = g.kscale[k + 1]; }                 \
    ISDF_LOAD_ONE(0, ra0, rb0) ISDF_LOAD_ONE(1, ra1, rb1)                                     \
    ISDF_LOAD_ONE(2, ra2, rb2) ISDF_LOAD_ONE(3, ra3, rb3)                                     \
  }
#define ISDF_STORE_ONE(BUF, I, RA, RB)                                                        \
  { double* qa = &sA[BUF][(srow + 32 * I) * LDT + sseg * 2];                                  \
    double* qb = &sB[BUF][(srow + 32 * I) * LDT + sseg * 2];                                  \
    qa[0] = RA.x; qa[1] = RA.y; qb[0] = RB.x; qb[1] = RB.y; }
#define ISDF_STORE_CHUNK(BUF)                                                                 \
  { ISDF_STORE_ONE(BUF, 0, ra0, rb0) ISDF_STORE_ONE(BUF, 1, ra1, rb1)                         \
    ISDF_STORE_ONE(BUF, 2, ra2, rb2) ISDF_STORE_ONE(BUF, 3, ra3, rb3) }

  d4 acc[4][4];
#pragma unroll
  for (int i = 0; i < 4; ++i)
#pragma unroll
    for (int j = 0; j < 4; ++j) acc[i][j] = (d4){0.0, 0.0, 0.0, 0.0};

  const int frow = lane & 15, fk = lane >> 4;
  ISDF_LOAD_CHUNK(0)
  ISDF_STORE_CHUNK(0)
  __syncthreads();
  for (int c = 0; c < nchunks; ++c) {
    const int buf = c & 1;
    if (c + 1 < nchunks) ISDF_LOAD_CHUNK(c + 1)
    const double* pa = &sA[buf][(wm * 64 + frow) * LDT + fk];
    const double* pb = &sB[buf][(wn * 64 + frow) * LDT + fk];
    double a0[4], b0[4], a1[4], b1[4];
#define ISDF_FRAGS(KK, AF, BF)                                                                \
    _Pragma("unroll") for (int i = 0; i < 4; ++i) {                                           \
      AF[i] = pa[i * 16 * LDT + (KK) * 4];                                                    \
      BF[i] = pb[i * 16 * LDT + (KK) * 4];                                                    \
    }
    ISDF_FRAGS(0, a0, b0)
    ISDF_FRAGS(1, a1, b1)
    ISDF_MFMA16(a0, b0)
    ISDF_FRAGS(2, a0, b0)
    ISDF_MFMA16(a1, b1)
    ISDF_FRAGS(3, a1, b1)
    ISDF_MFMA16(a0, b0)
    ISDF_MFMA16(a1, b1)
    if (c + 1 < nchunks) ISDF_STORE_CHUNK(buf ^ 1)
    __syncthreads();
  }
  double* out = g.P + (int64_t)t.slab * g.slab_stride;
  ISDF_STORE_ACC(4, 4, t.tm * BM + wm * 64, t.tn * BN + wn * 64, g.M, g.N, ISDF_SLAB_STORE)
#undef ISDF_LOAD_ONE
// ... 34 lines not shown
    A0 = *reinterpret_cast<const double2*>(pA0 + off);                                        \
    A1 = *reinterpret_cast<const double2*>(pA1 + off);                                        \
    A2 = *reinterpret_cast<const double2*>(pA2 + off);                                        \
    A3 = *reinterpret_cast<const double2*>(pA3 + off);                                        \
    B0 = *reinterpret_cast<const double2*>(pB0 + off);                                        \
    B1 = *reinterpret_cast<const double2*>(pB1 + off);                                        \
    if (SCALED) {                                                                             \
      const double2 sc = *reinterpret_cast<const double2*>(pS + off);                         \
      B0.x *= sc.x; B0.y *= sc.y; B1.x *= sc.x; B1.y *= sc.y;                                 \
    }                                                                                         \
  }
#define ISDF_ST1(P, R) { double* q_ = (P); q_[0] = R.x; q_[1] = R.y; }
#define ISDF_STOREB(BUF, A0, A1, A2, A3, B0, B1)                                              \
  {                                                                                           \
    double* qa = sA + (BUF) * BM2 * LDT + srow * LDT + sseg * 2;                              \
    double* qb = sB + (BUF) * BN * LDT + srow * LDT + sseg * 2;                               \
    ISDF_ST1(qa, A0) ISDF_ST1(qa + 64 * LDT, A1) ISDF_ST1(qa + 128 * LDT, A2)                 \
    ISDF_ST1(qa + 192 * LDT, A3) ISDF_ST1(qb, B0) ISDF_ST1(qb + 64 * LDT, B1)                 \
  }

#pragma unroll
  for (int i = 0; i < 4; ++i)
#pragma unroll
    for (int j = 0; j < 4; ++j) acc[i][j] = (d4){0.0, 0.0, 0.0, 0.0};
  const int frow = lane & 15, fk = lane >> 4;

  const int aoff = (wm * 64 + frow) * LDT + fk, boff = (wn * 64 + frow) * LDT + fk;
  double a0[4], b0[4], a1[4], b1[4];
#define ISDF_FRAGQ(BUF, KK, AF, BF)                                                           \
  {                                                                                           \
    const double* pa = sA + (BUF) * BM2 * LDT + aoff;                                         \
    const double* pb = sB + (BUF) * BN * LDT + boff;                                          \
    _Pragma("unroll") for (int i = 0; i < 4; ++i) {                                           \
      AF[i] = pa[i * 16 * LDT + (KK) * 4];                                                    \
      BF[i] = pb[i * 16 * LDT + (KK) * 4];                                                    \
    }                                                                                         \
  }
#define ISDF_CHUNKB(BUF, LOAD_AHEAD, STORE_NEXT)                                              \
  {                                                                                           \
    ISDF_FRAGQ(BUF, 1, a1, b1)                                                                \
    LOAD_AHEAD                                                                                \
    ISDF_MFMA16(a0, b0)                                                                       \
    ISDF_ISSUE(0x020, 6)                                                                      \
    __builtin_amdgcn_sched_barrier(0);                                                        \
    ISDF_FRAGQ(BUF, 2, a0, b0)                                                                \
    ISDF_MFMA16(a1, b1)                                                                       \
    ISDF_ISSUE(0, 0)                                                                          \
    __builtin_amdgcn_sched_barrier(0);                                                        \
    ISDF_FRAGQ(BUF, 3, a1, b1)                                                                \
    STORE_NEXT                                                                                \
    ISDF_MFMA16(a0, b0)                                                                       \
    ISDF_ISSUE(0x200, 6)                                                                      \
    __builtin_amdgcn_sched_barrier(0);                                                        \
    __syncthreads();                                                                          \
    ISDF_FRAGQ(1 - (BUF), 0, a0, b0)                                                          \
    ISDF_MFMA16(a1, b1)                                                                       \
    ISDF_ISSUE(0, 0)                                                                          \
    __builtin_amdgcn_sched_barrier(0);                                                        \
  }

  ISDF_LOADB(0, xa0, xa1, xa2, xa3, xb0, xb1)
  ISDF_LOADB(1, ya0, ya1, ya2, ya3, yb0, yb1)
  ISDF_STOREB(0, xa0, xa1, xa2, xa3, xb0, xb1)
  __syncthreads();
  ISDF_FRAGQ(0, 0, a0, b0)
  __builtin_amdgcn_sched_barrier(0);
  for (int c = 0; c < nchunks; c += 2) {
    ISDF_CHUNKB(0, ISDF_LOADB(min(c + 2, last), xa0, xa1, xa2, xa3, xb0, xb1), ISDF_STOREB(1, ya0, ya1, ya2, ya3, yb0, yb1))
    ISDF_CHUNKB(1, ISDF_LOADB(min(c + 3, last), ya0, ya1, ya2, ya3, yb0, yb1), ISDF_STOREB(0, xa0, xa1, xa2, xa3, xb0, xb1))
  }
#undef ISDF_LOADB
#undef ISDF_ST1
#undef ISDF_STOREB
#undef ISDF_FRAGQ
#undef ISDF_CHUNKB
}

template <bool SCALED>
__global__ __launch_bounds__(TPB2, 2) void gemm_nt_mfma_kernel_b(GemmArgs g) {
  extern __shared__ double smem[];
  const int64_t unit = xcd_unit(g.nunits_pad);
  if (unit >= g.nunits) return;
  const Tile t = decode_tile(unit, g.ntm, g.ntn);
  const KRange kr = slab_range(t.slab, g.kslab, g.K);
  d4 acc[4][4];
  tile_256x128<SCALED>(g.A, g.lda, g.B, g.ldb, g.kscale, g.M, g.N, t.tm, t.tn, kr.k0, (int)((kr.k1 - kr.k0) / BK), smem, acc);
  const int lane = threadIdx.x & 63, wave = threadIdx.x >> 6;
  double* out = g.P + (int64_t)t.slab * g.slab_stride;
  ISDF_STORE_ACC(4, 4, t.tm * BM2 + (wave >> 1) * 64, t.tn * BN + (wave & 1) * 64, g.M, g.N, ISDF_SLAB_STORE)
}

struct GramTriArgs {
  const double* X; int64_t ldx; int K;
  const GramTriUnit* units;
  const int64_t* blk_off;
  int64_t row0;
  const int64_t* tri_off;
  double* S;
  int64_t nunits, nunits_pad;
};

__global__ __launch_bounds__(TPB2, 2) void gram_tri_mfma_kernel(GramTriArgs t) {
  extern __shared__ double smem[];
  const int64_t unit = xcd_unit(t.nunits_pad);
  if (unit >= t.nunits) return;
  const GramTriUnit u = t.units[unit];
  const int64_t r0 = t.blk_off[u.blk];
  const double* X = t.X + (r0 - t.row0) * t.ldx;
  const int m = (int)(t.blk_off[u.blk + 1] - r0);
  const int64_t ldp = (int64_t)(u.tm + 1) * BM2;
  double* S = t.S + t.tri_off[u.blk] + (gram_tri_row((int64_t)u.tm * BM2) - (int64_t)u.tm * BM2 * ldp);
  d4 acc[4][4];
  tile_256x128<false>(X, t.ldx, X, t.ldx, nullptr, m, m, u.tm, u.tn, 0, t.K / BK, smem, acc);
  const int lane = threadIdx.x & 63, wave = threadIdx.x >> 6;
  ISDF_STORE_ACC(4, 4, u.tm * BM2 + (wave >> 1) * 64, u.tn * BN + (wave & 1) * 64, m, m, S[(int64_t)row * ldp + col] = acc[i][j][r];)
}

constexpr int TPBD = 256;

template <bool SCALED>
__global__ __launch_bounds__(TPBD, 2) void gemm_nt_mfma_kernel_d(GemmArgs g) {
  __shared__ double sB[2][BN * LDT];
  const int64_t unit = xcd_unit(g.nunits_pad);
  if (unit >= g.nunits) return;
  const Tile t = decode_tile(unit, g.ntm, g.ntn);
  const int tm = t.tm, tn = t.tn;
  const KRange kr = slab_range(t.slab, g.kslab, g.K);
  const int64_t k0 = kr.k0;
  const int nchunks = (int)((kr.k1 - k0) / BK);
  const int last = nchunks - 1;

  const int tid = threadIdx.x;
  const int lane = tid & 63, wave = tid >> 6;
  const int frow = lane & 15, fkq = lane >> 4;
  const int mlast = g.M - 1, nlast = g.N - 1;
  const double* pA0 = g.A + (int64_t)min(tm * BM + wave * 32 + frow, mlast) * g.lda + k0 + 4 * fkq;
  const double* pA1 = g.A + (int64_t)min(tm * BM + wave * 32 + 16 + frow, mlast) * g.lda + k0 + 4 * fkq;
  const int srow = tid >> 2, sseg = tid & 3;
  const double* pB0 = g.B + (int64_t)min(tn * BN + srow, nlast) * g.ldb + k0 + 4 * sseg;
  const double* pB1 = g.B + (int64_t)min(tn * BN + srow + 64, nlast) * g.ldb + k0 + 4 * sseg;
  const double* pS = SCALED ? g.kscale + k0 + 4 * sseg : nullptr;

  double2 xa00, xa01, xa10, xa11, xb00, xb01, xb10, xb11;
  double2 ya00, ya01, ya10, ya11, yb00, yb01, yb10, yb11;
#define ISDF_LOADD(C, A00, A01, A10, A11, B00, B01, B10, B11)                                 \
  {                                                                                           \
    const int off = (C) * BK;                                                                 \
    A00 = *reinterpret_cast<const double2*>(pA0 + off);                                       \
    A01 = *reinterpret_cast<const double2*>(pA0 + off + 2);                                   \
    A10 = *reinterpret_cast<const double2*>(pA1 + off);                                       \
    A11 = *reinterpret_cast<const double2*>(pA1 + off + 2);                                   \
    B00 = *reinterpret_cast<const double2*>(pB0 + off);                                       \
    B01 = *reinterpret_cast<const double2*>(pB0 + off + 2);                                   \
    B10 = *reinterpret_cast<const double2*>(pB1 + off);                                       \
    B11 = *reinterpret_cast<const double2*>(pB1 + off + 2);                                   \
    if (SCALED) {                                                                             \
      const double2 s0 = *reinterpret_cast<const double2*>(pS + off);                         \
      const double2 s1 = *reinterpret_cast<const double2*>(pS + off + 2);                     \
      B00.x *= s0.x; B00.y *= s0.y; B01.x *= s1.x; B01.y *= s1.y;                             \
      B10.x *= s0.x; B10.y *= s0.y; B11.x *= s1.x; B11.y *= s1.y;                             \
    }                                                                                         \
  }
#define ISDF_STORED(BUF, B00, B01, B10, B11)                                                  \
  {                                                                                           \
    double* q0 = &sB[BUF][srow * LDT + 4 * sseg];                                             \
    double* q1 = &sB[BUF][(srow + 64) * LDT + 4 * sseg];                                      \
    q0[0] = B00.x; q0[1] = B00.y; q0[2] = B01.x; q0[3] = B01.y;                               \
    q1[0] = B10.x; q1[1] = B10.y; q1[2] = B11.x; q1[3] = B11.y;                               \
  }

  d4 acc[2][8];
#pragma unroll
  for (int i = 0; i < 2; ++i)
#pragma unroll
    for (int j = 0; j < 8; ++j) acc[i][j] = (d4){0.0, 0.0, 0.0, 0.0};

  double bf0[8], bf1[8];
#define ISDF_FRAGD(BUF, J, BF)                                                                \
  {                                                                                           \
    const double* pb = &sB[BUF][frow * LDT + 4 * fkq + (J)];                                  \
    _Pragma("unroll") for (int jn = 0; jn < 8; ++jn) BF[jn] = pb[jn * 16 * LDT];              \
  }
#define ISDF_MFMAD(AV0, AV1, BF)                                                              \
    _Pragma("unroll") for (int jn = 0; jn < 8; ++jn) {                                        \
      acc[0][jn] = __builtin_amdgcn_mfma_f64_16x16x4f64(AV0, BF[jn], acc[0][jn], 0, 0, 0);    \
      acc[1][jn] = __builtin_amdgcn_mfma_f64_16x16x4f64(AV1, BF[jn], acc[1][jn], 0, 0, 0);    \
    }
#define ISDF_CHUNKD(BUF, A00, A01, A10, A11, LOAD_AHEAD, STORE_NEXT)                          \
  {                                                                                           \
    ISDF_FRAGD(BUF, 1, bf1)                                                                   \
    ISDF_MFMAD(A00.x, A10.x, bf0)                                                             \
    ISDF_ISSUE(0, 0)                                                                          \
    __builtin_amdgcn_sched_barrier(0);                                                        \
    ISDF_FRAGD(BUF, 2, bf0)                                                                   \
    ISDF_MFMAD(A00.y, A10.y, bf1)                                                             \
    ISDF_ISSUE(0, 0)                                                                          \
    __builtin_amdgcn_sched_barrier(0);                                                        \
    ISDF_FRAGD(BUF, 3, bf1)                                                                   \
    STORE_NEXT                                                                                \
    ISDF_MFMAD(A01.x, A11.x, bf0)                                                             \
    ISDF_ISSUE(0x200, 4)                                                                      \
    __builtin_amdgcn_sched_barrier(0);                                                        \
    __syncthreads();                                                                          \
    ISDF_FRAGD(1 - (BUF), 0, bf0)                                                             \
    ISDF_MFMAD(A01.y, A11.y, bf1)                                                             \
    LOAD_AHEAD                                                                                \
    ISDF_ISSUE(0x020, 8)                                                                      \
    __builtin_amdgcn_sched_barrier(0);                                                        \
// ... 227 lines not shown
    const int off = (C) * BK;                                                                 \
    const int64_t offb = (C) * bstep;                                                         \
    A0 = *reinterpret_cast<const double2*>(pA0 + off);                                        \
    A1 = *reinterpret_cast<const double2*>(pA1 + off);                                        \
    A2 = *reinterpret_cast<const double2*>(pA2 + off);                                        \
    A3 = *reinterpret_cast<const double2*>(pA3 + off);                                        \
    B0 = *reinterpret_cast<const double2*>(pB0 + offb);                                       \
    B1 = *reinterpret_cast<const double2*>(pB1 + offb);                                       \
  }
#define ISDF_NN_ST1(P, R) { double* q_ = (P); q_[0] = R.x; q_[1] = R.y; }
#define ISDF_NN_STORE(BUF, A0, A1, A2, A3, B0, B1)                                            \
  {                                                                                           \
    double* qa = sA + (BUF) * BM2 * LDT + srow * LDT + sseg * 2;                              \
    double* qb = sB + (BUF) * BK * LDN + krow * LDN + 2 * nseg;                               \
    ISDF_NN_ST1(qa, A0) ISDF_NN_ST1(qa + 64 * LDT, A1) ISDF_NN_ST1(qa + 128 * LDT, A2)        \
    ISDF_NN_ST1(qa + 192 * LDT, A3)                                                           \
    *reinterpret_cast<double2*>(qb) = B0;                                                     \
    *reinterpret_cast<double2*>(qb + 8 * LDN) = B1;                                           \
  }

  d4 acc[4][4];
#pragma unroll
  for (int i = 0; i < 4; ++i)
#pragma unroll
    for (int j = 0; j < 4; ++j) acc[i][j] = (d4){0.0, 0.0, 0.0, 0.0};
  const int frow = lane & 15, fk = lane >> 4;
  const int aoff = (wm * 64 + frow) * LDT + fk, boff = fk * LDN + wn * 64 + frow;
  double a0[4], b0[4], a1[4], b1[4];
#define ISDF_NN_FRAG(BUF, KK, AF, BF)                                                         \
  {                                                                                           \
    const double* pa = sA + (BUF) * BM2 * LDT + aoff;                                         \
    const double* pb = sB + (BUF) * BK * LDN + boff;                                          \
    _Pragma("unroll") for (int i = 0; i < 4; ++i) {                                           \
      AF[i] = pa[i * 16 * LDT + (KK) * 4];                                                    \
      BF[i] = pb[(KK) * 4 * LDN + i * 16];                                                    \
    }                                                                                         \
  }
#define ISDF_NN_CHUNK(BUF, LOAD_AHEAD, STORE_NEXT)                                            \
  {                                                                                           \
    ISDF_NN_FRAG(BUF, 1, a1, b1)                                                              \
    LOAD_AHEAD                                                                                \
    ISDF_MFMA16(a0, b0)                                                                       \
    ISDF_ISSUE(0x020, 6)                                                                      \
    __builtin_amdgcn_sched_barrier(0);                                                        \
    ISDF_NN_FRAG(BUF, 2, a0, b0)                                                              \
    ISDF_MFMA16(a1, b1)                                                                       \
    ISDF_ISSUE(0, 0)                                                                          \
    __builtin_amdgcn_sched_barrier(0);                                                        \
    ISDF_NN_FRAG(BUF, 3, a1, b1)                                                              \
    STORE_NEXT                                                                                \
    ISDF_MFMA16(a0, b0)                                                                       \
    ISDF_ISSUE(0x200, 6)                                                                      \
    __builtin_amdgcn_sched_barrier(0);                                                        \
    __syncthreads();                                                                          \
    ISDF_NN_FRAG(1 - (BUF), 0, a0, b0)                                                        \
    ISDF_MFMA16(a1, b1)                                                                       \
    ISDF_ISSUE(0, 0)                                                                          \
    __builtin_amdgcn_sched_barrier(0);                                                        \
  }

  ISDF_NN_LOAD(0, xa0, xa1, xa2, xa3, xb0, xb1)
  ISDF_NN_LOAD(1, ya0, ya1, ya2, ya3, yb0, yb1)
  ISDF_NN_STORE(0, xa0, xa1, xa2, xa3, xb0, xb1)
  __syncthreads();
  ISDF_NN_FRAG(0, 0, a0, b0)
  __builtin_amdgcn_sched_barrier(0);
  for (int c = 0; c < nchunks; c += 2) {
    ISDF_NN_CHUNK(0, ISDF_NN_LOAD(min(c + 2, last), xa0, xa1, xa2, xa3, xb0, xb1), ISDF_NN_STORE(1, ya0, ya1, ya2, ya3, yb0, yb1))
    ISDF_NN_CHUNK(1, ISDF_NN_LOAD(min(c + 3, last), ya0, ya1, ya2, ya3, yb0, yb1), ISDF_NN_STORE(0, xa0, xa1, xa2, xa3, xb0, xb1))
  }
  ISDF_STORE_ACC(4, 4, tm * BM2 + wm * 64, tn * BN + wn * 64, g.M, g.N,
                 { const double v = acc[i][j][r]; g.C[(int64_t)row * g.ldc + col] = SQ ? v * v : v; })
#undef ISDF_NN_LOAD
#undef ISDF_NN_ST1
#undef ISDF_NN_STORE
#undef ISDF_NN_FRAG
#undef ISDF_NN_CHUNK
}
#undef ISDF_MFMA16
#undef ISDF_ISSUE

__global__ void reduce_slabs_kernel(const double* __restrict__ P, int nslab, int64_t slab_stride,
                                    int M, int N, double alpha, double beta, double* __restrict__ C,
                                    int64_t ldc) {
  const int64_t idx = (int64_t)blockIdx.x * blockDim.x + threadIdx.x;
  if (idx >= (int64_t)M * N) return;
  const int m = (int)(idx / N), n = (int)(idx % N);
  double s = 0.0;
  for (int t = 0; t < nslab; ++t) s += P[(int64_t)t * slab_stride + idx];
  double* q = C + (int64_t)m * ldc + n;
  *q = (beta == 0.0) ? alpha * s : alpha * s + beta * (*q);
}

constexpr int TPBH = 512;

struct HermArgs {
  const double* A; int64_t lda;
  const double* B; int64_t ldb;
  const double* s; const double* a;
  double* Pre; double* Pim;
  int64_t ldp, slab_stride;
  int M, N;
  int64_t K, kslab;
  int ntm, ntn, nslab;
  int64_t nunits, nunits_pad;
  double alpha, beta;
  int direct;
};

__global__ __launch_bounds__(TPBH, 2) void herm_kscale_nt_kernel(HermArgs g) {
  extern __shared__ double smem[];
  double* sA = smem;
  double* sB = smem + 2 * BM * LDT;
  double* sT = smem + 2 * (BM + BN) * LDT;
  const int64_t unit = xcd_unit(g.nunits_pad);
  if (unit >= g.nunits) return;
  const Tile t = decode_tile(unit, g.ntm, g.ntn);
  const int tm = t.tm, tn = t.tn, slab = t.slab;
  const KRange kr = slab_range(slab, g.kslab, g.K);
  const int64_t k0 = kr.k0;
  const int nchunks = (int)((kr.k1 - k0) / BK);

  const int tid = threadIdx.x;
  const int lane = tid & 63, wave = tid >> 6;
  const int wm = wave >> 2, wn = wave & 3;
  const int srow = tid >> 3;
  const int sseg = tid & 7;
  const int mlast = g.M - 1, nlast = g.N - 1;
  const double* pA0 = g.A + (int64_t)min(tm * BM + srow, mlast) * g.lda + k0 + sseg * 2;
  const double* pA1 = g.A + (int64_t)min(tm * BM + srow + 64, mlast) * g.lda + k0 + sseg * 2;
  const double* pB0 = g.B + (int64_t)min(tn * BN + srow, nlast) * g.ldb + k0 + sseg * 2;
  const double* pB1 = g.B + (int64_t)min(tn * BN + srow + 64, nlast) * g.ldb + k0 + sseg * 2;
  const bool tload = tid < 16;
  const double* pT = (tid < 8 ? g.s : g.a) + k0 + sseg * 2;

  double2 ra0, ra1, rb0, rb1, rt = make_double2(0.0, 0.0);
#define ISDF_LOADH(C)                                                                         \
  {                                                                                           \
    const int off = (C) * BK;                                                                 \
    ra0 = *reinterpret_cast<const double2*>(pA0 + off);                                       \
    ra1 = *reinterpret_cast<const double2*>(pA1 + off);                                       \
    rb0 = *reinterpret_cast<const double2*>(pB0 + off);                                       \
    rb1 = *reinterpret_cast<const double2*>(pB1 + off);                                       \
    if (tload) rt = *reinterpret_cast<const double2*>(pT + off);                              \
  }
#define ISDF_STH(P, R) { double* q_ = (P); q_[0] = R.x; q_[1] = R.y; }
#define ISDF_STOREH(BUF)                                                                      \
  {                                                                                           \
    double* qa = sA + (BUF) * BM * LDT + srow * LDT + sseg * 2;                               \
    double* qb = sB + (BUF) * BN * LDT + srow * LDT + sseg * 2;                               \
    ISDF_STH(qa, ra0) ISDF_STH(qa + 64 * LDT, ra1) ISDF_STH(qb, rb0) ISDF_STH(qb + 64 * LDT, rb1) \
    if (tload) ISDF_STH(sT + (BUF) * 2 * BK + (tid >> 3) * BK + sseg * 2, rt)                 \
  }

  d4 cre[4][2], cim[4][2];
#pragma unroll
  for (int i = 0; i < 4; ++i)
#pragma unroll
    for (int j = 0; j < 2; ++j) { cre[i][j] = (d4){0.0, 0.0, 0.0, 0.0}; cim[i][j] = (d4){0.0, 0.0, 0.0, 0.0}; }

  const int frow = lane & 15, fk = lane >> 4;
  const double sgn = (fk & 1) ? 1.0 : -1.0;
  const int aoff = (wm * 64 + frow) * LDT, boff = (wn * 32 + frow) * LDT;
  ISDF_LOADH(0)
  ISDF_STOREH(0)
  __syncthreads();
  for (int c = 0; c < nchunks; ++c) {
    const int buf = c & 1;
    if (c + 1 < nchunks) ISDF_LOADH(c + 1)
    const double* pa = sA + buf * BM * LDT + aoff;
// ... 49 lines not shown
struct SlabPlan { int nslab; int64_t kslab, nunits, nunits_pad; };

SlabPlan plan_slabs(int64_t ntiles, int64_t slots, int M, int N, int64_t K, int out_bytes, int kmult, bool tune) {
  int64_t nslab = cdiv(8 * slots, ntiles);
  const int64_t cap = std::max<int64_t>(1, std::min<int64_t>(std::max<int64_t>(1, K / 2048),
                                                             std::max<int64_t>(1, ((int64_t)2 << 30) / ((int64_t)M * N * out_bytes))));
  nslab = std::max<int64_t>(1, std::min<int64_t>(nslab, cap));
  if (tune && ntiles * nslab > slots) {
    double best = 1e30;
    int64_t pick = nslab;
    for (int64_t c = nslab; c <= std::min<int64_t>(2 * nslab, cap); ++c) {
      const double units = (double)ntiles * c;
      const double waste = (double)(cdiv((int64_t)units, slots) * slots) / units;
      if (waste < best - 1e-9) { best = waste; pick = c; }
    }
    nslab = pick;
  }
  SlabPlan p;
  p.kslab = cdiv(cdiv(K, nslab), kmult) * kmult;
  p.nslab = (int)cdiv(K, p.kslab);
  p.nunits = ntiles * p.nslab;
  p.nunits_pad = cdiv(p.nunits, 8) * 8;
  return p;
}

bool rows_aligned16(const double* p, int64_t ld = 0) { return ld % 2 == 0 && ((uintptr_t)p) % 16 == 0; }

template <class... Kernels>
int raise_lds_once(isdf_handle h, int& done, size_t lds, Kernels... kernels) {
  if (done) return ISDF_OK;
  for (const void* k : {(const void*)kernels...})
    HIP_TRY(h, hipFuncSetAttribute(k, hipFuncAttributeMaxDynamicSharedMemorySize, (int)lds));
  done = 1;
  return ISDF_OK;
}

}

extern "C" int isdf_herm_kscale_nt(isdf_handle h, int M, int N, int64_t K, double alpha, const double* d_A, int64_t lda,
                                   const double* d_B, int64_t ldb, const double* d_s, const double* d_a, double beta,
                                   double* d_Cre, double* d_Cim, int64_t ldc) {
  if (!h) return ISDF_ERR_ARG;
  ARG_CHECK(h, M > 0 && N > 0 && K > 0 && d_A && d_B && d_s && d_a && d_Cre && d_Cim && lda >= K && ldb >= K && ldc >= N);
  ARG_CHECK(h, K % BK == 0 && rows_aligned16(d_A, lda) && rows_aligned16(d_B, ldb) && rows_aligned16(d_s) && rows_aligned16(d_a));
  HermArgs g;
  g.A = d_A; g.lda = lda; g.B = d_B; g.ldb = ldb; g.s = d_s; g.a = d_a;
  g.M = M; g.N = N; g.K = K;
  g.ntm = (int)cdiv(M, BM); g.ntn = (int)cdiv(N, BN);
  const SlabPlan p = plan_slabs((int64_t)g.ntm * g.ntn, h->num_cu, M, N, K, 16, BK, true);
  g.kslab = p.kslab; g.nslab = p.nslab; g.nunits = p.nunits; g.nunits_pad = p.nunits_pad;
  ARG_CHECK(h, g.nunits_pad < 2147483647LL);
  g.alpha = alpha; g.beta = beta;
  const int64_t plane = (int64_t)M * N;
  if (g.nslab == 1) {
    g.direct = 1; g.Pre = d_Cre; g.Pim = d_Cim; g.ldp = ldc; g.slab_stride = 0;
  } else {
    g.direct = 0;
    g.Pre = (double*)isdf_ws(h, "gemm_partials", sizeof(double) * (size_t)g.nslab * 2 * plane);
    if (!g.Pre) return ISDF_ERR_HIP;
    g.Pim = g.Pre + plane;
    g.ldp = N; g.slab_stride = 2 * plane;
  }
  const size_t lds = sizeof(double) * (2 * (BM + BN) * LDT + 4 * BK);
  if (int rc = raise_lds_once(h, h->attr_herm, lds, herm_kscale_nt_kernel)) return rc;
  {
    ProfScope ps(h, "herm_kscale_nt_kernel[flop]", 4.0 * M * N * (double)K);
    hipLaunchKernelGGL(herm_kscale_nt_kernel, dim3((unsigned)g.nunits_pad), dim3(TPBH), lds, h->stream, g);
    KERNEL_CHECK(h);
  }
  if (!g.direct) {
    ProfScope ps(h, "gemm_reduce_slabs_kernel[byte]", 16.0 * (double)plane * (g.nslab + 1));
    const unsigned nb = (unsigned)cdiv(plane, 256);
    hipLaunchKernelGGL(reduce_slabs_kernel, dim3(nb), dim3(256), 0, h->stream, g.Pre, g.nslab, g.slab_stride, M, N, alpha, beta,
                       d_Cre, ldc);
    hipLaunchKernelGGL(reduce_slabs_kernel, dim3(nb), dim3(256), 0, h->stream, g.Pim, g.nslab, g.slab_stride, M, N, alpha, beta,
                       d_Cim, ldc);
    KERNEL_CHECK(h);
  }
  return ISDF_OK;
}

int gemm_nt_f64_scaled(isdf_handle h, int M, int N, int64_t K, double alpha, const double* A, int64_t lda,
                       const double* B, int64_t ldb, const double* kscale, double beta, double* C,
                       int64_t ldc) {
  ARG_CHECK(h, M > 0 && N > 0 && K > 0 && A && B && C && lda >= K && ldb >= K && ldc >= N);
  GemmArgs g;
  g.A = A; g.lda = lda; g.B = B; g.ldb = ldb; g.kscale = kscale;
  g.M = M; g.N = N; g.K = K;
  static const int variant = getenv("ISDF_GEMM_VARIANT") ? atoi(getenv("ISDF_GEMM_VARIANT")) : -1;
  static const int tune = getenv("ISDF_GEMM_SLAB_TUNE") ? atoi(getenv("ISDF_GEMM_SLAB_TUNE")) : 1;
  const bool aligned = rows_aligned16(A, lda) && rows_aligned16(B, ldb) && rows_aligned16(kscale);
  const bool alignedB = aligned && K % 32 == 0, fast = aligned && K % BK == 0;
  const bool fitsB = (double)(cdiv(M, BM2) * BM2) <= 1.15 * (double)M;
  const bool useB = alignedB && M > BM && (variant == 1 || (variant == -1 && fitsB));
  const bool useD = alignedB && !useB && (variant == 3 || variant == -1);
  g.ntm = (int)cdiv(M, useB ? BM2 : BM); g.ntn = (int)cdiv(N, BN);
  const SlabPlan p = plan_slabs((int64_t)g.ntm * g.ntn, (int64_t)h->num_cu * (useB ? 1 : 2), M, N, K, 8, 2 * BK, tune != 0);
  g.kslab = p.kslab; g.nslab = p.nslab; g.nunits = p.nunits; g.nunits_pad = p.nunits_pad;
  g.alpha = alpha; g.beta = beta;
  if (g.nslab == 1) {
    g.direct = 1; g.P = C; g.ldp = ldc; g.slab_stride = 0;
  } else {
    g.direct = 0;
    g.P = (double*)isdf_ws(h, "gemm_partials", sizeof(double) * (size_t)g.nslab * M * N);
    if (!g.P) return ISDF_ERR_HIP;
    g.ldp = N; g.slab_stride = (int64_t)M * N;
  }
  ARG_CHECK(h, g.nunits_pad < 2147483647LL);
  const char* label = useD ? (kscale ? "gemm_nt_mfma_kernel_d<true>[flop]" : "gemm_nt_mfma_kernel_d<false>[flop]") : useB ? (kscale ? "gemm_nt_mfma_kernel_b<true>[flop]" : "gemm_nt_mfma_kernel_b<false>[flop]")
                           : (fast ? "gemm_nt_mfma_kernel<true>[flop]" : "gemm_nt_mfma_kernel<false>[flop]");
  {
    ProfScope ps(h, label, 2.0 * M * N * (double)K);
    if (useD) {
      if (kscale) hipLaunchKernelGGL(gemm_nt_mfma_kernel_d<true>, dim3((unsigned)g.nunits_pad), dim3(TPBD), 0, h->stream, g);
      else hipLaunchKernelGGL(gemm_nt_mfma_kernel_d<false>, dim3((unsigned)g.nunits_pad), dim3(TPBD), 0, h->stream, g);
    } else if (useB) {
      const size_t lds = sizeof(double) * 2 * (BM2 + BN) * LDT;
      if (int rc = raise_lds_once(h, h->attr_gemm_b, lds, gemm_nt_mfma_kernel_b<true>, gemm_nt_mfma_kernel_b<false>)) return rc;
      if (kscale) hipLaunchKernelGGL(gemm_nt_mfma_kernel_b<true>, dim3((unsigned)g.nunits_pad), dim3(TPB2), lds, h->stream, g);
      else hipLaunchKernelGGL(gemm_nt_mfma_kernel_b<false>, dim3((unsigned)g.nunits_pad), dim3(TPB2), lds, h->stream, g);
    } else if (fast) hipLaunchKernelGGL(gemm_nt_mfma_kernel<true>, dim3((unsigned)g.nunits_pad), dim3(TPB), 0, h->stream, g);
    else hipLaunchKernelGGL(gemm_nt_mfma_kernel<false>, dim3((unsigned)g.nunits_pad), dim3(TPB), 0, h->stream, g);
    KERNEL_CHECK(h);
  }
  if (!g.direct) {
    ProfScope ps(h, "gemm_reduce_slabs_kernel[byte]", 8.0 * (double)M * N * (g.nslab + 1));
    hipLaunchKernelGGL(reduce_slabs_kernel, dim3((unsigned)cdiv((int64_t)M * N, 256)), dim3(256), 0, h->stream,
                       g.P, g.nslab, g.slab_stride, M, N, alpha, beta, C, ldc);
    KERNEL_CHECK(h);
  }
  return ISDF_OK;
}

int gemm_nt_f64(isdf_handle h, int M, int N, int64_t K, double alpha, const double* A, int64_t lda,
                const double* B, int64_t ldb, double beta, double* C, int64_t ldc) {
  return gemm_nt_f64_scaled(h, M, N, K, alpha, A, lda, B, ldb, nullptr, beta, C, ldc);
}

extern "C" int isdf_gemm_nt(isdf_handle h, int M, int N, int64_t K, double alpha, const double* d_A,
                            int64_t lda, const double* d_B, int64_t ldb, const double* d_kscale,
                            double beta, double* d_C, int64_t ldc) {
  if (!h) return ISDF_ERR_ARG;
  return gemm_nt_f64_scaled(h, M, N, K, alpha, d_A, lda, d_B, ldb, d_kscale, beta, d_C, ldc);
}

extern "C" int isdf_gemm_nt_had3(isdf_handle h, int M, int N, int64_t K, double alpha, const double* d_A, int64_t lda,
                                 const double* d_H, int64_t ldh, const double* d_B, int64_t ldb, int64_t bstride, double beta,
                                 double* d_C, int64_t ldc, int64_t cstride) {
  if (!h) return ISDF_ERR_ARG;
  ARG_CHECK(h, M > 0 && N > 0 && K > 0 && d_A && d_B && d_C && lda >= K && (!d_H || ldh >= K) && ldb >= K && ldc >= N);
  ARG_CHECK(h, bstride >= 0 && cstride >= (int64_t)(M - 1) * ldc + N);
  const bool fused = K % BK == 0 && rows_aligned16(d_A, lda) && (!d_H || rows_aligned16(d_H, ldh)) && rows_aligned16(d_B, ldb) &&
                     bstride % 2 == 0;
  if (!fused) {
    const double* A = d_A;
    int64_t la = lda;
    if (d_H) {
      double* AH = (double*)isdf_ws(h, "had3_AH", sizeof(double) * (size_t)M * (size_t)K);
      if (!AH) return ISDF_ERR_HIP;
      HIP_TRY(h, hipMemcpy2DAsync(AH, sizeof(double) * (size_t)K, d_A, sizeof(double) * (size_t)lda, sizeof(double) * (size_t)K,
                                  (size_t)M, hipMemcpyDeviceToDevice, h->stream));
      for (int r0 = 0; r0 < M; r0 += 32768) {
        const int nr = M - r0 < 32768 ? M - r0 : 32768;
        if (int rc = isdf_hadamard_rows(h, AH + (int64_t)r0 * K, K, d_H + (int64_t)r0 * ldh, ldh, nr, K)) return rc;
      }
      A = AH; la = K;
    }
    for (int a = 0; a < 3; ++a)
      if (int rc = gemm_nt_f64(h, M, N, K, alpha, A, la, d_B + a * bstride, ldb, beta, d_C + a * cstride, ldc)) return rc;
    return ISDF_OK;
  }
  Had3Args g;
  g.A = d_A; g.lda = lda; g.H = d_H; g.ldh = ldh; g.B = d_B; g.ldb = ldb; g.bstride = bstride;
  g.M = M; g.N = N; g.K = K;
  g.ntm = (int)cdiv(M, BM); g.ntn = (int)cdiv(N, BN3);
  const SlabPlan p = plan_slabs((int64_t)g.ntm * g.ntn, (int64_t)h->num_cu * 2, M, N, K, 24, BK, true);
  g.kslab = p.kslab; g.nslab = p.nslab; g.nunits = p.nunits; g.nunits_pad = p.nunits_pad;
  ARG_CHECK(h, g.nunits_pad < 2147483647LL);
  g.alpha = alpha; g.beta = beta;
  const int64_t plane = (int64_t)M * N;
  if (g.nslab == 1) {
    g.direct = 1; g.P = d_C; g.ldp = ldc; g.pstride = cstride; g.slab_stride = 0;
  } else {
    g.direct = 0;
    g.P = (double*)isdf_ws(h, "gemm_partials", sizeof(double) * (size_t)g.nslab * 3 * plane);
    if (!g.P) return ISDF_ERR_HIP;
    g.ldp = N; g.pstride = plane; g.slab_stride = 3 * plane;
  }
  {
    ProfScope ps(h, d_H ? "gemm_nt_had3_kernel<true>[flop]" : "gemm_nt_had3_kernel<false>[flop]", 6.0 * M * N * (double)K);
    if (d_H) hipLaunchKernelGGL(gemm_nt_had3_kernel<true>, dim3((unsigned)g.nunits_pad), dim3(TPBD), 0, h->stream, g);
    else hipLaunchKernelGGL(gemm_nt_had3_kernel<false>, dim3((unsigned)g.nunits_pad), dim3(TPBD), 0, h->stream, g);
    KERNEL_CHECK(h);
  }
  if (!g.direct) {
    ProfScope ps(h, "gemm_reduce_slabs_kernel[byte]", 24.0 * (double)plane * (g.nslab + 1));
    for (int a = 0; a < 3; ++a)
      hipLaunchKernelGGL(reduce_slabs_kernel, dim3((unsigned)cdiv(plane, 256)), dim3(256), 0, h->stream, g.P + a * plane, g.nslab,
                         g.slab_stride, M, N, alpha, beta, d_C + a * cstride, ldc);
    KERNEL_CHECK(h);
  }
  return ISDF_OK;
}

int gram_tri_blocks(isdf_handle h, const double* X, int64_t ldx, int K, const GramTriUnit* d_units, int64_t nunits,
                    const int64_t* d_blk_off, int64_t row0, const int64_t* d_tri_off, double* S, double flop) {
  ARG_CHECK(h, X && d_units && d_blk_off && d_tri_off && S && nunits > 0 && K > 0 && K % 32 == 0 && ldx >= K &&
                   rows_aligned16(X, ldx));
  GramTriArgs t;
  t.X = X; t.ldx = ldx; t.K = K; t.units = d_units; t.blk_off = d_blk_off; t.row0 = row0; t.tri_off = d_tri_off; t.S = S;
  t.nunits = nunits; t.nunits_pad = cdiv(nunits, 8) * 8;
  ARG_CHECK(h, t.nunits_pad < 2147483647LL);
  const size_t lds = sizeof(double) * 2 * (BM2 + BN) * LDT;
  if (int rc = raise_lds_once(h, h->attr_gram_tri, lds, gram_tri_mfma_kernel)) return rc;
  ProfScope ps(h, "cand_gram_blocks[flop]", flop);
  hipLaunchKernelGGL(gram_tri_mfma_kernel, dim3((unsigned)t.nunits_pad), dim3(TPB2), lds, h->stream, t);
  KERNEL_CHECK(h);
  return ISDF_OK;
}

bool gemm_nn_f64_supported(isdf_handle h, int64_t M, int64_t N, int64_t K, const double* A, int64_t lda, const double* B,
                           int64_t ldb) {
  return h->gemm_nn_own && M > BM && (double)(cdiv(M, BM2) * BM2) <= 1.15 * (double)M && N >= 2 && N % 2 == 0 && K >= 32 && K % 32 == 0 &&
         rows_aligned16(A, lda) && rows_aligned16(B, ldb) && M < 2147483647LL && N < 2147483647LL && K < 2147483647LL;
}

// ... 22 lines not shown
```

pyscf_isdf_amd/csrc/handle.hip:

```cpp
#include "common.h"
#include <cstdarg>

int isdf_fail(isdf_handle h, int code, const char* fmt, ...) {
  char buf[1024];
  va_list ap;
  va_start(ap, fmt);
  vsnprintf(buf, sizeof(buf), fmt, ap);
  va_end(ap);
  if (h) h->err = buf;
  else fprintf(stderr, "mi355_isdf: %s\n", buf);
  return code;
}

void* isdf_ws(isdf_handle h, const char* name, size_t bytes) {
  auto& slot = h->ws[name];
  if (slot.second >= bytes && slot.first) return slot.first;
  if (slot.first) {
    (void)hipStreamSynchronize(h->stream);
    (void)hipFree(slot.first);
    slot.first = nullptr;
    slot.second = 0;
  }
  void* p = nullptr;
  hipError_t e = hipMalloc(&p, bytes ? bytes : 8);
// ... 6 lines not shown
  slot.second = bytes;
  return p;
}

int isdf_get_plan(isdf_handle h, const int32_t mesh[3], int batch, FftPlan** out) {
  std::vector<int> key = {mesh[0], mesh[1], mesh[2], batch};
  auto it = h->plans.find(key);
  if (it != h->plans.end()) {
    *out = &it->second;
    return ISDF_OK;
  }
  FftPlan p;
  int dims[3] = {mesh[0], mesh[1], mesh[2]};
  int64_t G = (int64_t)mesh[0] * mesh[1] * mesh[2];
  int64_t Gc = (int64_t)mesh[0] * mesh[1] * (mesh[2] / 2 + 1);
  ARG_CHECK(h, G < (int64_t)2147483647);
  FFT_TRY(h, hipfftPlanMany(&p.fwd, 3, dims, nullptr, 1, (int)G, nullptr, 1, (int)Gc, HIPFFT_D2Z, batch));
  hipfftResult r2 = hipfftPlanMany(&p.bwd, 3, dims, nullptr, 1, (int)Gc, nullptr, 1, (int)G, HIPFFT_Z2D, batch);
  if (r2 == HIPFFT_SUCCESS) r2 = hipfftSetStream(p.fwd, h->stream);
  if (r2 == HIPFFT_SUCCESS) r2 = hipfftSetStream(p.bwd, h->stream);
  if (r2 != HIPFFT_SUCCESS) {
    (void)hipfftDestroy(p.fwd);
    if (p.bwd) (void)hipfftDestroy(p.bwd);
    return isdf_fail(h, ISDF_ERR_LIB, "hipFFT plan (%d x %d x %d, batch %d) failed: result %d", mesh[0], mesh[1], mesh[2], batch,
                     (int)r2);
  }
  auto res = h->plans.emplace(key, p);
  *out = &res.first->second;
  return ISDF_OK;
}

extern "C" {

int isdf_abi_version(void) { return 21; }

int isdf_set_coulomb_omega(isdf_handle h, double omega) {
  if (!h) return ISDF_ERR_ARG;
  h->coul_omega = omega;
  return ISDF_OK;
}

int isdf_set_coulomb_cutoff(isdf_handle h, double rc) {
  if (!h) return ISDF_ERR_ARG;
  ARG_CHECK(h, rc >= 0.0);
  h->coul_rc = rc;
  return ISDF_OK;
}

int isdf_set_coulomb_ws(isdf_handle h, double alpha, const double ak[9], const int32_t mesh[3], const double maxq[3],
                        const double* d_vq) {
  if (!h) return ISDF_ERR_ARG;
  if (alpha <= 0.0) { h->wsk = WsKernel(); return ISDF_OK; }
  ARG_CHECK(h, ak && mesh && maxq && d_vq && mesh[0] > 0 && mesh[1] > 0 && mesh[2] > 0);
  h->wsk.alpha = alpha;
  for (int i = 0; i < 9; ++i) h->wsk.ak[i] = ak[i];
  for (int i = 0; i < 3; ++i) { h->wsk.mesh[i] = mesh[i]; h->wsk.maxq[i] = maxq[i]; }
  h->wsk.vq = d_vq;
  return ISDF_OK;
}

int isdf_set_option(isdf_handle h, const char* key, int value) {
  if (!h) return ISDF_ERR_ARG;
  ARG_CHECK(h, key != nullptr);
  if (std::string(key) == "trsm_substitution") { h->trsm_substitution = value ? 1 : 0; return ISDF_OK; }
  if (std::string(key) == "own_fft") { h->own_fft = value < 0 ? 0 : (value > 2 ? 2 : value); return ISDF_OK; }
  if (std::string(key) == "gemm_nn_own") { h->gemm_nn_own = value ? 1 : 0; return ISDF_OK; }
  if (std::string(key) == "coul_sphere") { h->coul_sphere = value < 0 ? 0 : value; return ISDF_OK; }
  if (std::string(key) == "conv_pipe") { h->conv_pipe = value != 0; return ISDF_OK; }
  if (std::string(key) == "conv_sub_rows") { h->conv_sub_rows = value < 0 ? 0 : value; return ISDF_OK; }
  if (std::string(key) == "gram_pivot_tpb") {
    if (value != 64 && value != 128 && value != 256) return ISDF_ERR_ARG;
    h->gram_pivot_tpb = value;
    return ISDF_OK;
  }
  if (std::string(key) == "cand_gram") { h->cand_gram = value ? 1 : 0; return ISDF_OK; }
  if (std::string(key) == "gram_compact") { h->gram_compact = value ? 1 : 0; return ISDF_OK; }
  if (std::string(key) == "gram_compact_permille") {
    if (value < 1 || value > 1000) return isdf_fail(h, ISDF_ERR_ARG, "isdf_set_option: gram_compact_permille %d not in [1, 1000]", value);
    h->gram_compact_permille = value;
    return ISDF_OK;
  }
  if (std::string(key) == "block_apply_waves") { h->block_apply_waves = value < 1 ? 1 : value; return ISDF_OK; }
  if (std::string(key) == "block_apply_reg") { h->block_apply_reg = value ? 1 : 0; return ISDF_OK; }
  return isdf_fail(h, ISDF_ERR_ARG, "isdf_set_option: unknown key '%s'", key);
}

int isdf_create(int device_id, isdf_handle* out) {
  if (!out) return ISDF_ERR_ARG;
  *out = nullptr;
  int ndev = 0;
  hipError_t e = hipGetDeviceCount(&ndev);
  if (e != hipSuccess || ndev == 0)
    return isdf_fail(nullptr, ISDF_ERR_HIP, "no HIP device visible (%s)", hipGetErrorString(e));
  if (device_id < 0 || device_id >= ndev)
    return isdf_fail(nullptr, ISDF_ERR_ARG, "device %d out of range (%d devices)", device_id, ndev);
  isdf_ctx* h = new isdf_ctx();
  h->device = device_id;
  if (hipSetDevice(device_id) != hipSuccess) { delete h; return ISDF_ERR_HIP; }
  hipDeviceProp_t prop;
  if (hipGetDeviceProperties(&prop, device_id) == hipSuccess) h->num_cu = prop.multiProcessorCount;
  if (rocblas_create_handle(&h->blas) != rocblas_status_success) {
    delete h;
    return isdf_fail(nullptr, ISDF_ERR_LIB, "rocblas_create_handle failed");
  }
  rocblas_set_pointer_mode(h->blas, rocblas_pointer_mode_host);
  *out = h;
  return ISDF_OK;
}

int isdf_release_workspace(isdf_handle h) {
  if (!h) return ISDF_ERR_ARG;
  (void)hipStreamSynchronize(h->stream);
  for (auto& kv : h->ws)
    if (kv.second.first) (void)hipFree(kv.second.first);
  h->ws.clear();
  for (auto& kv : h->plans) {
    if (kv.second.fwd) hipfftDestroy(kv.second.fwd);
    if (kv.second.bwd) hipfftDestroy(kv.second.bwd);
  }
  h->plans.clear();
  return ISDF_OK;
}

int isdf_destroy(isdf_handle h) {
  if (!h) return ISDF_OK;
  isdf_prof_reset(h);
  isdf_release_workspace(h);
  if (h->blas) rocblas_destroy_handle(h->blas);
  delete h;
  return ISDF_OK;
}

int isdf_set_stream(isdf_handle h, void* hip_stream) {
  if (!h) return ISDF_ERR_ARG;
  h->stream = (hipStream_t)hip_stream;
  BLAS_TRY(h, rocblas_set_stream(h->blas, h->stream));
  for (auto& kv : h->plans) {
    if (kv.second.fwd) FFT_TRY(h, hipfftSetStream(kv.second.fwd, h->stream));
    if (kv.second.bwd) FFT_TRY(h, hipfftSetStream(kv.second.bwd, h->stream));
  }
  return ISDF_OK;
}

const char* isdf_last_error(isdf_handle h) { return h ? h->err.c_str() : "null handle"; }

int isdf_prof_enable(isdf_handle h, int on) {
  if (!h) return ISDF_ERR_ARG;
  h->profiling = on ? 1 : 0;
  return ISDF_OK;
}

int isdf_prof_reset(isdf_handle h) {
  if (!h) return ISDF_ERR_ARG;
  (void)hipStreamSynchronize(h->stream);
  for (auto& kv : h->prof)
    for (auto& r : kv.second.recs) { (void)hipEventDestroy(r.e0); (void)hipEventDestroy(r.e1); }
  h->prof.clear();
  return ISDF_OK;
}

int isdf_prof_count(isdf_handle h) { return h ? (int)h->prof.size() : 0; }

int isdf_prof_get(isdf_handle h, int index, char* name, int name_cap, int64_t* launches, double* total_ms,
                  double* total_work) {
  if (!h || index < 0 || index >= (int)h->prof.size()) return ISDF_ERR_ARG;
  auto it = h->prof.begin();
// ... 23 lines not shown
```

pyscf_isdf_amd/csrc/jk.hip:

```cpp
#include "common.h"

namespace {

constexpr int64_t JCHUNK = 32768;

__global__ void rho_reduce_kernel(const double* __restrict__ T, int64_t ldT,
                                  const double* __restrict__ ao, int64_t ld, int nao, int64_t ng,
                                  double* __restrict__ rho) {
  const int64_t g = (int64_t)blockIdx.x * blockDim.x + threadIdx.x;
  if (g >= ng) return;
  double s = 0.0;
#pragma unroll 4
  for (int mu = 0; mu < nao; ++mu) s = fma(T[(int64_t)mu * ldT + g], ao[(int64_t)mu * ld + g], s);
  rho[g] = s;
}

__global__ void hadamard_kernel(double* __restrict__ M, int64_t ldm, const double* __restrict__ W,
                                int64_t ldw, int64_t rows, int64_t cols) {
  const int64_t c = (int64_t)blockIdx.x * blockDim.x + threadIdx.x;
  const int64_t r = blockIdx.y;
  if (c >= cols) return;
  M[r * ldm + c] *= W[r * ldw + c];
}

__global__ void pair_rows_kernel(const double* __restrict__ ao, int64_t ld, const double* __restrict__ mo, int64_t ldmo,
                                 int nocc, int64_t ng, double* __restrict__ R) {
  const int64_t g = (int64_t)blockIdx.x * blockDim.x + threadIdx.x;
  if (g >= ng) return;
  const int row = blockIdx.y;
  const int i = row / nocc, jj = row % nocc;
  R[(int64_t)row * ng + g] = ao[(int64_t)i * ld + g] * mo[(int64_t)jj * ldmo + g];
}

__global__ void pair_reduce_kernel(const double* __restrict__ R, const double* __restrict__ mo, int64_t ldmo, int nocc,
                                   int64_t ng, double* __restrict__ vdm) {
  const int64_t g = (int64_t)blockIdx.x * blockDim.x + threadIdx.x;
  if (g >= ng) return;
  const int i = blockIdx.y;
  double s = 0.0;
  for (int jj = 0; jj < nocc; ++jj) s = fma(R[((int64_t)i * nocc + jj) * ng + g], mo[(int64_t)jj * ldmo + g], s);
  vdm[(int64_t)i * ng + g] = s;
}

}

extern "C" int isdf_rho(isdf_handle h, const double* d_ao, int nao, int64_t ng, int64_t ld,
                        const double* d_dm, int nset, double* d_rho, int64_t ldrho) {
  if (!h) return ISDF_ERR_ARG;
  ARG_CHECK(h, d_ao && d_dm && d_rho && nao > 0 && ng > 0 && ld >= ng && nset > 0 && ldrho >= ng);
  double* T = (double*)isdf_ws(h, "jk_T", sizeof(double) * (size_t)nao * JCHUNK);
  if (!T) return ISDF_ERR_HIP;
  for (int i = 0; i < nset; ++i) {
    for (int64_t g0 = 0; g0 < ng; g0 += JCHUNK) {
      const int64_t nc = std::min(JCHUNK, ng - g0);
      int rc = gemm_rm(h, 'N', 'N', nao, nc, nao, 1.0, d_dm + (int64_t)i * nao * nao, nao, d_ao + g0, ld, 0.0, T, JCHUNK);
      if (rc) return rc;
      hipLaunchKernelGGL(rho_reduce_kernel, dim3((unsigned)cdiv(nc, 256)), dim3(256), 0, h->stream, T, JCHUNK,
                         d_ao + g0, ld, nao, nc, d_rho + (int64_t)i * ldrho + g0);
      KERNEL_CHECK(h);
    }
  }
  return ISDF_OK;
}

extern "C" int isdf_vj_from_vR(isdf_handle h, const double* d_ao, int nao, int64_t ng, int64_t ld,
                               const double* d_vR, int nset, int64_t ldv, double* d_vj) {
  if (!h) return ISDF_ERR_ARG;
  ARG_CHECK(h, d_ao && d_vR && d_vj && nao > 0 && ng > 0 && ld >= ng && nset > 0 && ldv >= ng);
  for (int i = 0; i < nset; ++i) {
    int rc = gemm_nt_f64_scaled(h, nao, nao, ng, 1.0, d_ao, ld, d_ao, ld, d_vR + (int64_t)i * ldv, 0.0,
                                d_vj + (int64_t)i * nao * nao, nao);
    if (rc) return rc;
  }
  return ISDF_OK;
}

extern "C" int isdf_get_j(isdf_handle h, const double* d_ao, int nao, int64_t ngrids, int64_t ld,
                          const int32_t mesh[3], const double a[9], const double* d_dm, int nset,
                          double* d_vj) {
  if (!h) return ISDF_ERR_ARG;
  ARG_CHECK(h, mesh && ngrids == (int64_t)mesh[0] * mesh[1] * mesh[2]);
  double* rho = (double*)isdf_ws(h, "jk_rho", sizeof(double) * (size_t)nset * ngrids);
  if (!rho) return ISDF_ERR_HIP;
  int rc = isdf_rho(h, d_ao, nao, ngrids, ld, d_dm, nset, rho, ngrids);
  if (rc) return rc;
  rc = isdf_coulomb_potential(h, rho, nset, ngrids, mesh, a);
  if (rc) return rc;
  return isdf_vj_from_vR(h, d_ao, nao, ngrids, ld, rho, nset, ngrids, d_vj);
}

extern "C" int isdf_get_k(isdf_handle h, const double* d_aoP, int P, int nao, const double* d_W,
                          int64_t ldw, int row0, int nrows, const double* d_dm, int nset,
                          double* d_vk) {
  if (!h) return ISDF_ERR_ARG;
  ARG_CHECK(h, d_aoP && d_W && d_dm && d_vk && P > 0 && nao > 0 && ldw >= P && nset > 0);
  ARG_CHECK(h, row0 >= 0 && nrows >= 0 && row0 + nrows <= P);
  const int RCH = 4096;
  const int rch = std::min(RCH, std::max(nrows, 1));
  double* X = (double*)isdf_ws(h, "k_X", sizeof(double) * (size_t)P * nao);
  double* M = (double*)isdf_ws(h, "k_M", sizeof(double) * (size_t)rch * P);
  double* Y = (double*)isdf_ws(h, "k_Y", sizeof(double) * (size_t)rch * nao);
  if (!X || !M || !Y) return ISDF_ERR_HIP;
  for (int i = 0; i < nset; ++i) {
    const double* dm = d_dm + (int64_t)i * nao * nao;
    double* vk = d_vk + (int64_t)i * nao * nao;
    int rc = gemm_rm(h, 'N', 'N', P, nao, nao, 1.0, d_aoP, nao, dm, nao, 0.0, X, nao);
    if (rc) return rc;
    if (nrows == 0) {
      HIP_TRY(h, hipMemsetAsync(vk, 0, sizeof(double) * (size_t)nao * nao, h->stream));
      continue;
    }
    for (int r = row0; r < row0 + nrows; r += rch) {
      const int nr = std::min(rch, row0 + nrows - r);
      rc = gemm_rm(h, 'N', 'T', nr, P, nao, 1.0, X + (int64_t)r * nao, nao, d_aoP, nao, 0.0, M, P);
      if (rc) return rc;
      hipLaunchKernelGGL(hadamard_kernel, dim3((unsigned)cdiv(P, 256), (unsigned)nr), dim3(256), 0, h->stream, M,
                         (int64_t)P, d_W + (int64_t)r * ldw, ldw, (int64_t)nr, (int64_t)P);
      KERNEL_CHECK(h);
      rc = gemm_rm(h, 'N', 'N', nr, nao, P, 1.0, M, P, d_aoP, nao, 0.0, Y, nao);
      if (rc) return rc;
      rc = gemm_rm(h, 'T', 'N', nao, nao, nr, 1.0, d_aoP + (int64_t)r * nao, nao, Y, nao, r == row0 ? 0.0 : 1.0, vk, nao);
      if (rc) return rc;
    }
  }
  return ISDF_OK;
}

extern "C" int isdf_get_k_exact(isdf_handle h, const double* d_ao, int nao, int64_t ngrids, int64_t ld,
                                const double* d_C, int nocc, const int32_t mesh[3], const double a[9],
                                int i0, int ni, int max_rows, double* d_vk) {
  if (!h) return ISDF_ERR_ARG;
  ARG_CHECK(h, d_ao && d_C && mesh && a && d_vk && nao > 0 && nocc > 0 && max_rows >= nocc);
  ARG_CHECK(h, ngrids == (int64_t)mesh[0] * mesh[1] * mesh[2] && ld >= ngrids);
  ARG_CHECK(h, i0 >= 0 && ni >= 0 && i0 + ni <= nao && nocc <= 65535);
  if (ni == 0) return ISDF_OK;
  const int64_t G = ngrids;
  const int bi = std::max(1, std::min(ni, max_rows / nocc));
  double* mo = (double*)isdf_ws(h, "kx_mo", sizeof(double) * (size_t)nocc * G);
  double* R = (double*)isdf_ws(h, "kx_R", sizeof(double) * (size_t)bi * nocc * G);
  double* vdm = (double*)isdf_ws(h, "kx_vdm", sizeof(double) * (size_t)bi * G);
  if (!mo || !R || !vdm) return ISDF_ERR_HIP;
  int rc = gemm_rm(h, 'T', 'N', nocc, G, nao, 1.0, d_C, nocc, d_ao, ld, 0.0, mo, G);
  if (rc) return rc;
  const double det = a[0] * (a[4] * a[8] - a[5] * a[7]) - a[1] * (a[3] * a[8] - a[5] * a[6]) +
                     a[2] * (a[3] * a[7] - a[4] * a[6]);
  const double w = fabs(det) / (double)G;
  for (int r = i0; r < i0 + ni; r += bi) {
    const int nb = std::min(bi, i0 + ni - r);
    ARG_CHECK(h, nb * nocc <= 65535);
    hipLaunchKernelGGL(pair_rows_kernel, dim3((unsigned)cdiv(G, 256), (unsigned)(nb * nocc)), dim3(256), 0, h->stream,
                       d_ao + (int64_t)r * ld, ld, mo, G, nocc, G, R);
    KERNEL_CHECK(h);
    rc = isdf_coulomb_rows(h, R, nb * nocc, G, mesh, a, nb * nocc, R, G);
    if (rc) return rc;
    hipLaunchKernelGGL(pair_reduce_kernel, dim3((unsigned)cdiv(G, 256), (unsigned)nb), dim3(256), 0, h->stream, R, mo, G,
                       nocc, G, vdm);
    KERNEL_CHECK(h);
    rc = gemm_nt_f64(h, nb, nao, G, w, vdm, G, d_ao, ld, 0.0, d_vk + (int64_t)r * nao, nao);
    if (rc) return rc;
  }
  return ISDF_OK;
}

namespace {
__global__ void hadamard_rows_kernel(double* __restrict__ X, int64_t ldx, const double* __restrict__ Y, int64_t ldy,
                                     int64_t cols) {
  const int64_t c = (int64_t)blockIdx.x * blockDim.x + threadIdx.x;
// ... 100 lines not shown
```

pyscf_isdf_amd/fit_route.py:

```python
import numpy as np


class FitRouteMixin:
    def _bj_prepare(self, ao, nh, d_ip, ip_off, aoP, scratch=None):
        be = self.backend
        P = aoP.shape[0]
        be.gather_aoP(ao, d_ip, aoP)
        A = self._buffer('factor', (P, P))
        if getattr(self, '_psi', None) is not None and not nh:
            be.gram_prod(aoP, self._psiP, A)
        else:
            be.gram_sq(aoP, A, nh)
        self._Dinv_key = None
        be.shift_diag(A, self.reg_rel)
        Dblk = self._buffer('Dblk', (P, P))
        self.block_shift_used = be.block_chol(A, ip_off, self.block_shift, Dblk)
        be.block_solve(Dblk, ip_off, 0, 0, A)
        be.block_solve(Dblk, ip_off, 1, 1, A)
        extra = be.chol_inplace(A, 0.0, scratch=scratch)
        self.reg_used = self.reg_rel + extra
        return A, Dblk

    def _block_inverse(self, Dblk, ip_off):
        if not self.block_apply_mfma or int(np.diff(np.asarray(ip_off)).max()) > 1100:
# ... 207 lines not shown
        import torch
        be = self.backend
        ao = getattr(self, 'ao', None)
        if ao is None:
            return np.inf
        nao, G = ao.shape
        rng = np.random.default_rng(7)
        cd = be.to_device(rng.standard_normal((2 * ntest, nao)) / np.sqrt(nao))
        rows = be.empty((2 * ntest, G))
        be.gemm_nn(cd, ao, rows)
        t = rows[:ntest].contiguous()
        be.hadamard_rows(t, rows[ntest:].contiguous())
        Gfull = int(np.prod(mesh))
        if G != Gfull:
            g0, g1 = self._slice
            full = be.zeros((ntest, Gfull))
            full[:, g0:g1] = t
            self.comm.all_reduce_sum(full)
            t = full
        idx = np.flatnonzero(box.ravel()).astype(np.int32)
        scale = np.sqrt(mult.ravel()[idx] * w * cg.ravel()[idx])
        ldx = -(-2 * len(idx) // 128) * 128
        X = be.empty((ntest, ldx))
        be.spectral_rows(t, mesh, be.to_device(idx), be.to_device(scale), X, batch=ntest)
        x = be.to_host(X)[:, :2 * len(idx)]
        e = x[:, 0::2] ** 2 + x[:, 1::2] ** 2
        outside = ~keep.ravel()[idx]
        tot = e.sum(axis=1)
        return float((e[:, outside].sum(axis=1) / np.where(tot > 0, tot, 1.0)).max())

    def _finish_W_spectral(self, W, probe=None):
        be, st = self.backend, self._fit_state
        plan = self._spectral_plan()
        ip_off = np.asarray(st['ip_off'], dtype=np.int64)
        P = W.shape[0]
        mesh = np.asarray(self.mesh, dtype=np.int32)
        G = int(np.prod(mesh))
        if plan is None:
            rows_avail = int(self._bufs['theta'].numel() // G)
            st2 = dict(st, kind='blockjacobi-paneled', rows=self._buffer('theta', (rows_avail, G)),
                       panels=self._panel_plan(ip_off, rows_avail))
            self._fit_state = st2
            try:
                return self._finish_W_paneled(W, probe=probe)
            finally:
                self._fit_state = st
        nbat = int(self.fft_batch or 512)
        big = int(np.diff(ip_off).max())
        self._last_fft_batch = nbat
        ldx = plan['ldx']
        X = self._buffer('theta', (P, ldx))
        piece = self._pair_rows_piece(big)
        scratch = self._buffer('rows_scratch', (nbat + big, G))
        self.w_spectral_fraction = plan['fraction']
        self._last_spectral_ldx = ldx
        if piece:
            self._spectral_rows_two_frontiers(X, scratch, piece, plan, probe)
            return self._spectral_W_finish(X, W, nbat)
        nxt, fill, g0 = 0, 0, 0
        while nxt < P or fill > 0:
            while fill < nbat and nxt < P:
                i = int(np.searchsorted(ip_off, nxt))
                j = i + 1
                while j + 1 < len(ip_off) and fill + (ip_off[j + 1] - nxt) <= nbat + big:
                    j += 1
                b1 = int(ip_off[j])
                self._bj_rows_range(nxt, b1, scratch[fill:fill + (b1 - nxt)])
                fill += b1 - nxt
                nxt = b1
            take = min(nbat, fill)
            rows = scratch[:take]
            if probe is not None:
                be.rows_combine(probe[0][:, g0:g0 + take], rows, probe[1], accumulate=g0 > 0)
            be.spectral_rows(rows, mesh, plan['idx'], plan['scale'], X[g0:g0 + take], batch=take)
            if fill > take:
                scratch[:fill - take].copy_(scratch[take:fill].clone() if fill - take > take else scratch[take:fill])
            g0 += take
            fill -= take
        self._spectral_W_finish(X, W, nbat)

    def _spectral_W_finish(self, X, W, nbat):
        be, st = self.backend, self._fit_state
        P = W.shape[0]
        for b0 in range(0, P, nbat):
            b1 = min(P, b0 + nbat)
            be.gemm_nt(X[b0:b1], X[b0:], W[b0:b1, b0:], alpha=1.0)
        be.symmetrize_upper(W)
        self._bj_finish(st['Afac'], st['Dblk'], st['ip_off'], W)

    def _pair_rows_piece(self, big):
        align = int(getattr(self, 'pair_rows_align', 0) or 0)
        if align <= 0 or not hasattr(self.backend, 'pair_rows_frontier') or getattr(self, '_psi', None) is not None \
                or not self.block_apply_mfma or big > 1100:
            return 0
        return int(self.fft_batch or 512) // align * align

    def _spectral_rows_two_frontiers(self, X, scratch, piece, plan, probe):
        be, st = self.backend, self._fit_state
        ip_off = np.asarray(st['ip_off'], dtype=np.int64)
        P = int(ip_off[-1])
        mesh = np.asarray(self.mesh, dtype=np.int32)
        G = self.ao.shape[1]
        Dinv = self._block_inverse(st['Dblk'], ip_off)
        nbat = int(self.fft_batch or 512)
        squared = be.pair_rows_squared(self.aoP, min(piece, P), self.ao, G)
        app, prod = 0, 0
        while app < P:
            new = min(piece, P - prod)
            j = int(np.searchsorted(ip_off, prod + new, side='right')) - 1
            i = int(np.searchsorted(ip_off, app))
            end = int(ip_off[j])
            be.pair_rows_frontier(self.aoP[prod:prod + new], self.ao, G, squared, Dinv[app:, app:],
                                  (ip_off[i:j + 1] - app).astype(np.int32), scratch, prod - app)
            prod += new
            if end > app:
                rows = scratch[:end - app]
                if probe is not None:
                    be.rows_combine(probe[0][:, app:end], rows, probe[1], accumulate=app > 0)
                be.spectral_rows(rows, mesh, plan['idx'], plan['scale'], X[app:end], batch=min(nbat, end - app))
                tail = prod - end
                if tail > 0:
                    src = scratch[end - app:prod - app]
                    scratch[:tail].copy_(src.clone() if tail > end - app else src)
                app = end

    def _bj_finish(self, Afac, Dblk, ip_off, W, antisymmetric=False):
        be = self.backend
        be.W_from_factor(Afac, 2, W)
        be.W_from_factor(Afac, 0, W)
        be.block_solve(Dblk, ip_off, 0, 1, W)
        be.block_solve(Dblk, ip_off, 1, 0, W)
        be.symmetrize_mean(W, antisymmetric)

    def _bj_clusters(self):
        cell = self.cell
        natm = cell.natm
        parent = list(range(natm))

        def find(i):
            while parent[i] != i:
                parent[i] = parent[parent[i]]
                i = parent[i]
            return i
        r = float(self.bj_cluster_radius or 0.0)
        if r > 0 and natm > 1:
            a = np.asarray(cell.lattice_vectors(), dtype=float)
            frac = np.asarray(cell.atom_coords(), dtype=float).dot(np.linalg.inv(a))
            d = frac[:, None, :] - frac[None, :, :]
            d -= np.round(d)
            dist = np.linalg.norm(d.dot(a), axis=2)
            for i, j in zip(*np.nonzero(np.triu(dist < r, 1))):
                ri, rj = find(int(i)), find(int(j))
                if ri != rj:
                    parent[max(ri, rj)] = min(ri, rj)
        groups = {}
        for i in range(natm):
            groups.setdefault(find(i), []).append(i)
        return [groups[k] for k in sorted(groups)]

    def _bj_blocks(self, counts, clusters):
        per = [int(sum(counts[b] for b in cl)) for cl in clusters]
        off = np.append(0, np.cumsum(per)).astype(np.int32)
        g = max(1, int(self.bj_group))
        if g > 1:
            off = np.unique(np.append(off[::g], off[-1])).astype(np.int32)
        return off

    def _fit_routes(self):
        if self.fit_route not in ('auto', 'blockjacobi', 'cholesky'):
# ... 88 lines not shown
```

pyscf_isdf_amd/isdf.py:

```python
import os
import sys
import time
import warnings
import numpy as np
import torch
from . import gto
from ._common import (UniformGrids, partition_grid_by_atom, _monkhorst_pack_size, _aoslice_by_atom,
                      _default_fft_batch)
from .fit_route import FitRouteMixin
from .sharded import ShardedMixin
from .kpoints import KPointMixin
from .hcore import HcoreMixin
from .eri_surface import EriSurfaceMixin
from .jk_e1 import JKE1Mixin
from .pp_grad import PPGradMixin


class ISDF(FitRouteMixin, ShardedMixin, KPointMixin, HcoreMixin, EriSurfaceMixin, JKE1Mixin, PPGradMixin):
    _keys = {'cell', 'kpts', 'grids', 'mesh', 'blockdim', 'exxdiv', 'c_isdf', 'select', 'tie_rtol'}

    def __init__(self, cell, kpts=np.zeros((1, 3)), c_isdf=12, select='refined', backend=None, comm=None):
        self.cell = cell
        self.stdout = getattr(cell, 'stdout', None) or sys.stdout
        self.verbose = getattr(cell, 'verbose', 0)
        self.max_memory = getattr(cell, 'max_memory', 4000)
        self.kpts_symm = None
        if hasattr(kpts, 'kpts_ibz') and hasattr(kpts, 'transform_dm'):
            self.kpts_symm = kpts
            kpts = kpts.kpts
        self.kpts = np.asarray(kpts).reshape(-1, 3)
        self.grids = UniformGrids(cell, cell.mesh)
        self.blockdim = 240
        self.exxdiv = None
        self.c_isdf = c_isdf
        self.select = select
        self.refine_over = 2.0
        self.pair_space = 'ao'
        self.occ_refit = 'always'
        self.w_spectral = True
        self.w_sphere = 'auto'
        self.w_sphere_tol = 1e-11
        self.w_sort_bins = 256
        self.w_spectral_check_tol = 5e-9
        self.w_spectral_max_c = 18
        self.cand_skip_zero_rows = True
        self.cand_gram = True
        self.cand_ao_cutoff = None
        self.tie_rtol = 1e-10
        self.select_tol = -1.0
        self.reg_rel = 1e-12
        self.reg_used = 0.0
        self.k_ip_factor = None
        self.kpt_pair_q = 'auto'
        self.kpt_w_spectral = False
        self.kpts_band = None
        self.force_sharded = False
        self.fit_route = 'auto'
        self.bj_check_tol = 3e-8
        self.bj_auto_kpts = False
        self.bj_max_c = 12
        self.bj_nprobe = 8
        self.bj_cluster_radius = 2.4
        self.bj_group = 1
        self.bj_check = None
        self.fit_route_used = None
        self.block_shift = 0.0
        self.block_shift_used = 0.0
        self.robust_k = False
        self.explicit_theta = False
        self.fft_batch = None
        self.pair_rows_align = 256
        self.block_apply_mfma = True
        self.max_resident_rows = None
        self.max_device_memory = None
        self.n_panels = 1
        self._backend = backend
        self._comm = comm
        self._rsh_df = {}
        self._built = False
        self._W_omega = {}
        self._fit_state = None
        self._fit_pending = False
        self._psi = self._psiP = None
        self._fit_dm = None
        self._V = None
        self._bufs = {}
        self._ovlp = None
        self.timings = {}
        self.ao = None
        self.aoP = None
        self.W = None
        self.ip = None

    @property
    def _want_theta(self):
        return bool(self.explicit_theta or self.robust_k)

    @property
    def _sharded(self):
        return self.comm.size > 1 or self.force_sharded or getattr(self.comm, 'always', False)

    @property
    def mesh(self):
        return self.grids.mesh

    @mesh.setter
    def mesh(self, mesh):
        self.grids.mesh = np.asarray(mesh)
        self.grids._coords = None

    @property
    def backend(self):
        if self._backend is None:
            from .backend import HipBackend
            dev = 0
            if self._comm is not None:
                dev = self._comm.local_rank
            if os.environ.get('ISDF_ONE_GPU'):
                dev = 0
            self._backend = HipBackend(dev)
        return self._backend

    def reset(self, cell=None):
        if cell is not None:
            self.cell = cell
        self.grids = UniformGrids(self.cell, self.cell.mesh)
# ... 878 lines not shown
```

pyscf_isdf_amd/lib.py:

```python
import ctypes
import os

_HERE = os.path.dirname(os.path.abspath(__file__))
LIB_PATH = os.path.join(_HERE, 'lib', 'libmi355_isdf.so')
ABI_VERSION = 21

_lib = None

c_int, c_i64, c_dbl, c_vp = ctypes.c_int, ctypes.c_int64, ctypes.c_double, ctypes.c_void_p

SIGNATURES = {
    'isdf_abi_version': (c_int, []),
    'isdf_create': (c_int, [c_int, ctypes.POINTER(c_vp)]),
    'isdf_destroy': (c_int, [c_vp]),
    'isdf_set_stream': (c_int, [c_vp, c_vp]),
    'isdf_last_error': (ctypes.c_char_p, [c_vp]),
    'isdf_workspace_bytes': (c_i64, [c_vp]),
    'isdf_set_coulomb_omega': (c_int, [c_vp, c_dbl]),
    'isdf_set_coulomb_cutoff': (c_int, [c_vp, c_dbl]),
    'isdf_set_coulomb_ws': (c_int, [c_vp, c_dbl, c_vp, c_vp, c_vp, c_vp]),
    'isdf_set_option': (c_int, [c_vp, ctypes.c_char_p, c_int]),
    'isdf_release_workspace': (c_int, [c_vp]),
    'isdf_prof_enable': (c_int, [c_vp, c_int]),
    'isdf_prof_reset': (c_int, [c_vp]),
    'isdf_prof_count': (c_int, [c_vp]),
    'isdf_prof_get': (c_int, [c_vp, c_int, ctypes.c_char_p, c_int, ctypes.POINTER(c_i64), ctypes.POINTER(c_dbl), ctypes.POINTER(c_dbl)]),
    'isdf_eval_ao': (c_int, [c_vp, c_vp, c_int, c_vp, c_int, c_vp, c_int, c_vp, c_int, c_vp, c_vp, c_i64, c_vp, c_i64]),
    'isdf_block_row_absmax': (c_int, [c_vp, c_vp, c_int, c_i64, c_int, c_vp, c_vp]),
    'isdf_gather_cols': (c_int, [c_vp, c_vp, c_int, c_i64, c_vp, c_i64, c_vp, c_i64]),
    'isdf_partition_by_atom': (c_int, [c_vp, c_vp, c_i64, c_vp, c_int, c_vp, c_dbl, c_vp]),
    'isdf_select_ip': (c_int, [c_vp, c_vp, c_int, c_i64, c_int, c_vp, c_vp, c_dbl, c_dbl, c_vp, c_i64, c_vp, c_vp]),
    'isdf_select_ip_ws': (c_int, [c_vp, c_vp, c_int, c_i64, c_int, c_vp, c_vp, c_dbl, c_dbl, c_vp, c_i64, c_vp, c_vp, c_vp,
                                  c_i64]),
    'isdf_select_ip_work_bytes': (c_i64, [c_int, c_i64]),
    'isdf_select_ip_gram': (c_int, [c_vp, c_vp, c_int, c_i64, c_int, c_dbl, c_dbl, c_int, c_vp, ctypes.POINTER(ctypes.c_int32)]),
    'isdf_fit_from_chol': (c_int, [c_vp, c_vp, c_int, c_i64, c_i64, c_vp]),
    'isdf_fit_prepare': (c_int, [c_vp, c_vp, c_int, c_i64, c_vp, c_int, c_dbl, c_vp, c_vp, ctypes.POINTER(c_dbl)]),
    'isdf_fit_apply': (c_int, [c_vp, c_vp, c_vp, c_int, c_int, c_vp, c_i64, c_i64, c_int, c_vp, c_i64]),
    'isdf_gather_aoP': (c_int, [c_vp, c_vp, c_int, c_i64, c_vp, c_int, c_vp]),
    'isdf_gram_sq': (c_int, [c_vp, c_vp, c_int, c_int, c_int, c_vp]),
    'isdf_pair_gram_rows': (c_int, [c_vp, c_vp, c_int, c_int, c_int, c_vp, c_i64, c_i64, c_vp, c_i64]),
    'isdf_gram_prod': (c_int, [c_vp, c_vp, c_int, c_int, c_vp, c_int, c_vp]),
    'isdf_pair_prod_rows': (c_int, [c_vp, c_vp, c_int, c_int, c_vp, c_int, c_vp, c_i64, c_vp, c_i64, c_i64, c_vp, c_i64]),
    'isdf_factor_solve_half': (c_int, [c_vp, c_vp, c_int, c_int, c_vp, c_i64, c_i64]),
    'isdf_gram_prod_cplx': (c_int, [c_vp, c_vp, c_int, c_int, c_int, c_vp, c_int, c_int, c_vp]),
    'isdf_pair_prod_rows_cplx': (c_int, [c_vp, c_vp, c_int, c_int, c_int, c_vp, c_int, c_int, c_vp, c_i64, c_vp, c_i64, c_i64,
                                         c_vp, c_i64]),
    'isdf_block_chol': (c_int, [c_vp, c_vp, c_int, c_int, c_vp, c_dbl, c_vp, ctypes.POINTER(c_dbl)]),
    'isdf_block_solve': (c_int, [c_vp, c_vp, c_int, c_int, c_vp, c_int, c_int, c_vp, c_i64, c_i64]),
    'isdf_block_invert': (c_int, [c_vp, c_vp, c_int, c_int, c_vp, c_vp]),
    'isdf_block_apply': (c_int, [c_vp, c_vp, c_i64, c_int, c_vp, c_vp, c_i64, c_i64]),
    'isdf_pair_rows_block_apply': (c_int, [c_vp, c_vp, c_int, c_int, c_vp, c_i64, c_i64, c_vp, c_i64, c_int, c_vp, c_vp, c_i64]),
    'isdf_pair_rows_squared': (c_int, [c_vp, c_vp, c_int, c_int, c_vp, c_i64, c_i64, ctypes.POINTER(c_int)]),
    'isdf_pair_rows_frontier': (c_int, [c_vp, c_vp, c_int, c_int, c_vp, c_i64, c_i64, c_int, c_vp, c_i64, c_int, c_vp, c_vp, c_i64,
                                        c_int]),
    'isdf_shift_diag': (c_int, [c_vp, c_vp, c_int, c_dbl]),
    'isdf_chol_inplace': (c_int, [c_vp, c_vp, c_int, c_dbl, c_vp, ctypes.POINTER(c_dbl)]),
    'isdf_factor_solve': (c_int, [c_vp, c_vp, c_int, c_vp, c_i64, c_i64]),
    'isdf_bj_probe_vectors': (c_int, [c_vp, c_vp, c_int, c_vp, c_vp, c_int, c_int, c_vp]),
    'isdf_rows_combine': (c_int, [c_vp, c_vp, c_int, c_i64, c_int, c_vp, c_i64, c_i64, c_vp, c_i64, c_int]),
    'isdf_bj_probe_rows': (c_int, [c_vp, c_vp, c_int, c_vp, c_vp, c_int, c_int, c_vp, c_vp, c_i64, c_i64, c_vp, c_i64]),
    'isdf_gather_T': (c_int, [c_vp, c_vp, c_int, c_i64, c_vp, c_vp]),
    'isdf_W_from_factor': (c_int, [c_vp, c_vp, c_int, c_int, c_vp, c_i64]),
    'isdf_fit_global': (c_int, [c_vp, c_vp, c_int, c_i64, c_i64, c_vp, c_int, c_dbl, c_vp, c_i64, c_vp, ctypes.POINTER(c_dbl)]),
    'isdf_coulomb_W': (c_int, [c_vp, c_vp, c_int, c_i64, c_vp, c_vp, c_int, c_int, c_int, c_int, c_vp, c_i64]),
    'isdf_coulomb_rows': (c_int, [c_vp, c_vp, c_int, c_i64, c_vp, c_vp, c_int, c_vp, c_i64]),
    'isdf_symmetrize_upper': (c_int, [c_vp, c_vp, c_int, c_i64]),
    'isdf_symmetrize_mean': (c_int, [c_vp, c_vp, c_int, c_i64, c_int]),
    'isdf_get_j': (c_int, [c_vp, c_vp, c_int, c_i64, c_i64, c_vp, c_vp, c_vp, c_int, c_vp]),
    'isdf_rho': (c_int, [c_vp, c_vp, c_int, c_i64, c_i64, c_vp, c_int, c_vp, c_i64]),
    'isdf_coulomb_potential': (c_int, [c_vp, c_vp, c_int, c_i64, c_vp, c_vp]),
    'isdf_vj_from_vR': (c_int, [c_vp, c_vp, c_int, c_i64, c_i64, c_vp, c_int, c_i64, c_vp]),
    'isdf_eval_ao_k': (c_int, [c_vp, c_vp, c_int, c_vp, c_int, c_vp, c_int, c_vp, c_int, c_vp, c_vp, c_int, c_vp, c_i64, c_vp, c_vp, c_i64]),
    'isdf_select_ip_cplx': (c_int, [c_vp, c_vp, c_int, c_int, c_i64, c_int, c_vp, c_vp, c_dbl, c_dbl, c_vp, c_i64, c_vp, c_vp]),
    'isdf_fit_prepare_cplx': (c_int, [c_vp, c_vp, c_int, c_int, c_i64, c_vp, c_int, c_dbl, c_vp, c_vp, ctypes.POINTER(c_dbl)]),
    'isdf_fit_apply_cplx': (c_int, [c_vp, c_vp, c_vp, c_int, c_int, c_int, c_vp, c_i64, c_i64, c_int, c_vp, c_i64]),
    'isdf_coulG_q': (c_int, [c_vp, c_vp, c_vp, c_vp, c_int, c_dbl, c_vp]),
    'isdf_coulomb_Wq': (c_int, [c_vp, c_vp, c_int, c_i64, c_vp, c_vp, c_dbl, c_int, c_int, c_int, c_int, c_vp, c_vp, c_i64]),
    'isdf_symmetrize_hermitian': (c_int, [c_vp, c_vp, c_vp, c_int, c_i64]),
    'isdf_finish_Wq': (c_int, [c_vp, c_vp, c_vp, c_int, c_i64, c_vp, c_vp]),
    'isdf_get_k_pair': (c_int, [c_vp, c_vp, c_vp, c_vp, c_vp, c_int, c_int, c_dbl, c_vp]),
    'isdf_get_k_exact_kpt': (c_int, [c_vp, c_vp, c_vp, c_int, c_i64, c_vp, c_vp, c_int, c_i64, c_vp, c_vp, c_dbl, c_int, c_int, c_int, c_vp, c_vp]),
    'isdf_coulG_half': (c_int, [c_vp, c_vp, c_vp, c_vp]),
    'isdf_spectral_supported': (c_int, [c_vp, c_vp, c_int, ctypes.POINTER(c_int)]),
    'isdf_spectral_rows': (c_int, [c_vp, c_vp, c_int, c_i64, c_vp, c_vp, c_vp, c_int, c_int, c_vp, c_i64]),
    'isdf_coulomb_rows_q': (c_int, [c_vp, c_vp, c_int, c_i64, c_vp, c_vp, c_vp, c_vp]),
    'isdf_nyquist_spectra': (c_int, [c_vp, c_vp, c_int, c_i64, c_vp, c_int, c_vp, c_vp]),
    'isdf_zhadamard_planes': (c_int, [c_vp, c_vp, c_vp, c_i64, c_vp, c_vp, c_i64, c_int, c_i64]),
    'isdf_rho_k': (c_int, [c_vp, c_vp, c_vp, c_int, c_i64, c_i64, c_vp, c_vp, c_dbl, c_vp]),
    'isdf_vj_k': (c_int, [c_vp, c_vp, c_vp, c_int, c_i64, c_i64, c_vp, c_vp, c_vp]),
    'isdf_pp_local_potential': (c_int, [c_vp, c_int, c_vp, c_vp, c_vp, c_vp, c_vp]),
    'isdf_pp_projector_overlaps': (c_int, [c_vp, c_vp, c_int, c_vp, c_int, c_vp, c_int, c_vp, c_vp, c_vp, c_vp, c_int, c_vp, c_vp, c_vp]),
    'isdf_pp_local_force': (c_int, [c_vp, c_vp, c_int, c_i64, c_int, c_vp, c_vp, c_vp, c_vp, c_vp]),
    'isdf_pp_projector_overlaps_ip': (c_int, [c_vp, c_vp, c_int, c_vp, c_int, c_vp, c_int, c_vp, c_vp, c_vp, c_vp, c_int, c_vp, c_vp,
                                              c_vp]),
    'isdf_rowdot3': (c_int, [c_vp, c_int, c_i64, c_dbl, c_vp, c_i64, c_i64, c_vp, c_vp, c_i64, c_int, c_vp, c_i64]),
    'isdf_gemm_nn': (c_int, [c_vp, c_int, c_i64, c_int, c_dbl, c_vp, c_i64, c_vp, c_i64, c_dbl, c_vp, c_i64]),
    'isdf_hadamard_rows': (c_int, [c_vp, c_vp, c_i64, c_vp, c_i64, c_int, c_i64]),
    'isdf_eval_ao_deriv1': (c_int, [c_vp, c_vp, c_int, c_vp, c_int, c_vp, c_int, c_vp, c_int, c_vp, c_vp, c_i64, c_vp, c_i64, c_i64]),
    'isdf_eval_ao_k_deriv1': (c_int, [c_vp, c_vp, c_int, c_vp, c_int, c_vp, c_int, c_vp, c_int, c_vp, c_vp, c_int, c_vp, c_i64, c_vp, c_vp, c_i64, c_i64]),
    'isdf_uniform_grid': (c_int, [c_vp, c_vp, c_vp, c_vp]),
    'isdf_rho_pair': (c_int, [c_vp, c_vp, c_int, c_vp, c_int, c_i64, c_i64, c_vp, c_int, c_vp, c_i64]),
    'isdf_mg_embed_density': (c_int, [c_vp, c_vp, c_int, c_vp, c_dbl, c_vp, c_vp, c_int]),
    'isdf_mg_restrict_potential': (c_int, [c_vp, c_vp, c_int, c_vp, c_vp, c_dbl, c_vp]),
    'isdf_mg_coulomb_kernel': (c_int, [c_vp, c_vp, c_int, c_vp, c_vp]),
    'isdf_lda_exchange': (c_int, [c_vp, c_vp, c_i64, c_vp, c_vp]),
    'isdf_lda_vwn_add': (c_int, [c_vp, c_vp, c_i64, c_vp, c_vp]),
    'isdf_gga_b88': (c_int, [c_vp, c_vp, c_vp, c_i64, c_i64, c_vp, c_vp, c_vp, c_i64]),
    'isdf_xc_fused': (c_int, [c_vp, c_vp, c_vp, c_i64, c_i64, c_dbl, c_dbl, c_dbl, c_int, c_dbl, c_vp, c_vp, c_vp, c_i64]),
    'isdf_gga_lyp_polarised': (c_int, [c_vp, c_vp, c_vp, c_i64, c_i64, c_i64, c_dbl, c_int, c_vp, c_vp, c_vp, c_i64, c_i64]),
    'isdf_lda_exchange_fxc': (c_int, [c_vp, c_vp, c_i64, c_vp]),
    'isdf_lda_vwn_fxc_add': (c_int, [c_vp, c_vp, c_i64, c_vp]),
    'isdf_gga_b88_fxc': (c_int, [c_vp, c_vp, c_i64, c_i64, c_vp, c_i64, c_i64, c_int, c_vp, c_i64, c_i64, c_vp, c_i64]),
    'isdf_xc_fxc_apply': (c_int, [c_vp, c_int, c_vp, c_i64, c_i64, c_i64, c_vp, c_i64, c_i64, c_int, c_vp, c_i64, c_i64, c_int]),
    'isdf_dot': (c_int, [c_vp, c_vp, c_vp, c_i64, c_vp]),
    'isdf_gemm_nt': (c_int, [c_vp, c_int, c_int, c_i64, c_dbl, c_vp, c_i64, c_vp, c_i64, c_vp, c_dbl, c_vp, c_i64]),
    'isdf_gemm_nt_had3': (c_int, [c_vp, c_int, c_int, c_i64, c_dbl, c_vp, c_i64, c_vp, c_i64, c_vp, c_i64, c_i64, c_dbl, c_vp, c_i64,
                                  c_i64]),
    'isdf_pack_table_pm': (c_int, [c_vp, c_vp, c_vp, c_vp, c_int, c_dbl, c_vp, c_vp, c_i64]),
    'isdf_herm_kscale_nt': (c_int, [c_vp, c_int, c_int, c_i64, c_dbl, c_vp, c_i64, c_vp, c_i64, c_vp, c_vp, c_dbl, c_vp, c_vp, c_i64]),
    'isdf_get_k_exact': (c_int, [c_vp, c_vp, c_int, c_i64, c_i64, c_vp, c_int, c_vp, c_vp, c_int, c_int, c_int, c_vp]),
    'isdf_get_k': (c_int, [c_vp, c_vp, c_int, c_int, c_vp, c_i64, c_int, c_int, c_vp, c_int, c_vp]),
}


def load():
    global _lib
    if _lib is not None:
        return _lib
    if not os.path.exists(LIB_PATH):
        raise RuntimeError(
            'libmi355_isdf.so not found at %s — build it with `python -c "import __graft_entry__ as g; '
            'g.build()"` or `make -C pyscf_isdf_amd/csrc`.  There is no CPU fallback.' % LIB_PATH)
    try:
        import torch
    except ImportError:
        pass
    lib = ctypes.CDLL(LIB_PATH, mode=ctypes.RTLD_GLOBAL)
    for name, (res, args) in SIGNATURES.items():
        fn = getattr(lib, name)
        fn.restype = res
        fn.argtypes = args
    v = lib.isdf_abi_version()
    if v != ABI_VERSION:
        raise RuntimeError('libmi355_isdf.so ABI version %d != binding version %d' % (v, ABI_VERSION))
    _lib = lib
    return lib


class IsdfError(RuntimeError):
    pass


class Handle:

    def __init__(self, device=0):
        self.lib = load()
        h = c_vp()
        rc = self.lib.isdf_create(int(device), ctypes.byref(h))
        if rc != 0 or not h.value:
            raise IsdfError('isdf_create(device=%d) failed with status %d (no MI355X visible?)' % (device, rc))
        self.h = h
        self.device = device

    def call(self, name, *args):
        rc = getattr(self.lib, name)(self.h, *args)
        if rc != 0:
            msg = self.lib.isdf_last_error(self.h)
            raise IsdfError('%s failed (status %d): %s' % (name, rc, msg.decode() if msg else ''))

    def close(self):
        if getattr(self, 'h', None) is not None and self.h.value:
            self.lib.isdf_destroy(self.h)
            self.h = c_vp()

    def __del__(self):
        try:
            self.close()
        except Exception:
            pass
```

Measured before the change: 16.73.

## Exploit symmetry in J GEMMs and skip dead FFT line tiles

Adds an upper-triangular mode to the f64 NT GEMM that skips tiles below the diagonal, then mirrors the result. It is used in vj_from_vR by default. The density build for J now folds the density matrix into a lower-triangular form so the row-blocked GEMMs touch only a triangle. The spectral-rows FFT marks which line tiles feed sampled points and skips the rest in the strided pass. Together these remove redundant symmetric work and unused FFT lines, at the cost of extra fold, mirror and marking kernels plus added workspace.

```diff
diff --git a/include/mi355_isdf.h b/include/mi355_isdf.h
--- a/include/mi355_isdf.h
+++ b/include/mi355_isdf.h
@@ -171,6 +171,8 @@
                const double* d_dm, int nset, double* d_vj);
 int isdf_rho(isdf_handle h, const double* d_ao, int nao, int64_t ng, int64_t ld,
              const double* d_dm, int nset, double* d_rho, int64_t ldrho);
+int isdf_rho_j(isdf_handle h, const double* d_ao, int nao, int64_t ng, int64_t ld,
+               const double* d_dm, int nset, double* d_rho, int64_t ldrho);
 int isdf_coulomb_potential(isdf_handle h, double* d_rho_inout, int nset, int64_t ldrho,
                            const int32_t mesh[3], const double a[9]);
 int isdf_vj_from_vR(isdf_handle h, const double* d_ao, int nao, int64_t ng, int64_t ld,
@@ -265,6 +267,9 @@
 int isdf_gemm_nt(isdf_handle h, int M, int N, int64_t K, double alpha, const double* d_A, int64_t lda,
                  const double* d_B, int64_t ldb, const double* d_kscale, double beta, double* d_C,
                  int64_t ldc);
+int isdf_gemm_nt_upper(isdf_handle h, int M, int N, int64_t K, double alpha, const double* d_A, int64_t lda,
+                       const double* d_B, int64_t ldb, const double* d_kscale, double beta, double* d_C,
+                       int64_t ldc);
 
 int isdf_gemm_nt_had3(isdf_handle h, int M, int N, int64_t K, double alpha, const double* d_A, int64_t lda, const double* d_H,
                       int64_t ldh, const double* d_B, int64_t ldb, int64_t bstride, double beta, double* d_C, int64_t ldc,
diff --git a/pyscf_isdf_amd/backend.py b/pyscf_isdf_amd/backend.py
--- a/pyscf_isdf_amd/backend.py
+++ b/pyscf_isdf_amd/backend.py
@@ -436,6 +436,11 @@
         self.handle.call('isdf_rho', self._p(ao), ao.shape[0], int(ng), ao.stride(0), self._p(dm), dm.shape[0],
                          self._p(rho), rho.stride(0))
 
+    def rho_j(self, ao, ng, dm, rho):
+        self._stream()
+        self.handle.call('isdf_rho_j', self._p(ao), ao.shape[0], int(ng), ao.stride(0), self._p(dm), dm.shape[0],
+                         self._p(rho), rho.stride(0))
+
     def coulomb_potential(self, rho, mesh, a):
         self._stream()
         mesh = np.ascontiguousarray(mesh, dtype=np.int32)
@@ -470,13 +475,15 @@
         self._stream()
         self.handle.call('isdf_hadamard_rows', self._p(X), X.stride(0), self._p(Y), Y.stride(0), X.shape[0], X.shape[1])
 
-    def gemm_nt(self, A, B, C, alpha=1.0, beta=0.0, kscale=None):
+    gemm_nt_has_upper = True
+
+    def gemm_nt(self, A, B, C, alpha=1.0, beta=0.0, kscale=None, upper=False):
         self._stream()
         M, K = A.shape
         N = B.shape[0]
         assert B.shape[1] == K and tuple(C.shape) == (M, N) and A.stride(1) == 1 and B.stride(1) == 1 and C.stride(1) == 1
         ks = self._p(kscale) if kscale is not None else _vp(0)
-        self.handle.call('isdf_gemm_nt', M, N, K, float(alpha), self._p(A), A.stride(0), self._p(B), B.stride(0), ks,
+        self.handle.call('isdf_gemm_nt_upper' if upper else 'isdf_gemm_nt', M, N, K, float(alpha), self._p(A), A.stride(0), self._p(B), B.stride(0), ks,
                          float(beta), self._p(C), C.stride(0))
 
     def gemm_nt_had3(self, A, H, B3, C3, alpha=1.0, beta=0.0):
diff --git a/pyscf_isdf_amd/csrc/common.h b/pyscf_isdf_amd/csrc/common.h
--- a/pyscf_isdf_amd/csrc/common.h
+++ b/pyscf_isdf_amd/csrc/common.h
@@ -56,6 +56,10 @@
   int gram_compact_permille = 875;
   int block_apply_waves = 16;
   int block_apply_reg = 1;
+  int gemm_nt_upper = 1;
+  int w_strips_upper = 0;
+  int j_triangular = 1;
+  int spectral_skip_lines = 1;
   double coul_omega = 0.0;
   double coul_rc = 0.0;
   int coul_sphere = 0;
@@ -129,7 +133,8 @@
                 const double* B, int64_t ldb, double beta, double* C, int64_t ldc);
 int gemm_nt_f64_scaled(isdf_handle h, int M, int N, int64_t K, double alpha, const double* A, int64_t lda,
                        const double* B, int64_t ldb, const double* kscale, double beta, double* C,
-                       int64_t ldc);
+                       int64_t ldc, bool upper = false);
+int mirror_upper(isdf_handle h, double* d_W, int P, int64_t ldw);
 int trsm_lower_left(isdf_handle h, bool trans, int m, int64_t n, const double* L, int64_t ldl, double* X, int64_t ldx);
 int trsm_lower_right(isdf_handle h, bool trans, int m, int64_t n, const double* L, int64_t ldl, double* X, int64_t ldx);
 int block_forward_solve(isdf_handle h, const double* D, int64_t ldd, int nblk, const int32_t* blk_off_host, double* X,
diff --git a/pyscf_isdf_amd/csrc/coulomb.hip b/pyscf_isdf_amd/csrc/coulomb.hip
--- a/pyscf_isdf_amd/csrc/coulomb.hip
+++ b/pyscf_isdf_amd/csrc/coulomb.hip
@@ -257,13 +257,17 @@
   return ISDF_OK;
 }
 
-extern "C" int isdf_symmetrize_upper(isdf_handle h, double* d_W, int P, int64_t ldw) {
-  if (!h) return ISDF_ERR_ARG;
+int mirror_upper(isdf_handle h, double* d_W, int P, int64_t ldw) {
   ARG_CHECK(h, d_W && P > 0 && ldw >= P);
   const unsigned nt = (unsigned)cdiv(P, 32);
   hipLaunchKernelGGL(mirror_upper_kernel, dim3(nt, nt), dim3(32, 8), 0, h->stream, d_W, P, ldw);
   KERNEL_CHECK(h);
   return ISDF_OK;
+}
+
+extern "C" int isdf_symmetrize_upper(isdf_handle h, double* d_W, int P, int64_t ldw) {
+  if (!h) return ISDF_ERR_ARG;
+  return mirror_upper(h, d_W, P, ldw);
 }
 
 extern "C" int isdf_coulomb_W(isdf_handle h, const double* d_theta, int P, int64_t ldt,
@@ -291,8 +295,8 @@
     rc = convolve_rows(h, d_theta + (int64_t)r * ldt, V, nb, mesh, cg, Z);
     if (rc) return rc;
     const int c0 = upper_only ? r : 0;
-    rc = gemm_nt_f64(h, nb, P - c0, G, w, V, G, d_theta + (int64_t)c0 * ldt, ldt, 0.0,
-                     d_W + (int64_t)r * ldw + c0, ldw);
+    rc = gemm_nt_f64_scaled(h, nb, P - c0, G, w, V, G, d_theta + (int64_t)c0 * ldt, ldt, nullptr, 0.0,
+                            d_W + (int64_t)r * ldw + c0, ldw, upper_only && h->gemm_nt_upper && h->w_strips_upper);
     if (rc) return rc;
   }
   return ISDF_OK;
diff --git a/pyscf_isdf_amd/csrc/fft_conv.hip b/pyscf_isdf_amd/csrc/fft_conv.hip
--- a/pyscf_isdf_amd/csrc/fft_conv.hip
+++ b/pyscf_isdf_amd/csrc/fft_conv.hip
@@ -496,8 +496,10 @@
 
 template <int MODE, int ZCT>
 __global__ __launch_bounds__(TPB) void strided_fft_fast_kernel(double2* __restrict__ data, int64_t os, int64_t es, int Mtot,
-                                                               Axis ax, int ntile, const double* __restrict__ table) {
+                                                               Axis ax, int ntile, const double* __restrict__ table,
+                                                               const unsigned char* __restrict__ live) {
   extern __shared__ double2 lds[];
+  if (MODE == 0 && live && !live[blockIdx.x % ntile]) return;
   const int n = ax.n;
   double2* x = lds;
   double2* tw = lds + n * ZCT;
@@ -983,14 +985,14 @@
 
 template <int MODE>
 void launch_strided(isdf_handle h, bool fast, int L, double2* data, int64_t nouter, int64_t os, int64_t es, int Mtot, const Axis& ax,
-                    const double* table) {
+                    const double* table, const unsigned char* live = nullptr) {
   const int nt = (int)cdiv(Mtot, L);
   const dim3 grid((unsigned)(nouter * nt));
   const size_t n = ax.n;
   if (fast)
     with_lines(L, [&](auto z) {
       strided_fft_fast_kernel<MODE, decltype(z)::value><<<grid, dim3(TPB), sizeof(double2) * (n * L + n), h->stream>>>(
-          data, os, es, Mtot, ax, nt, table);
+          data, os, es, Mtot, ax, nt, table, live);
     });
   else
     strided_fft_kernel<MODE><<<grid, dim3(TPB), sizeof(double2) * 2 * n * L, h->stream>>>(data, os, es, Mtot, ax, L, nt, table);
@@ -1128,6 +1130,14 @@
   out[(int64_t)row * ldx2 + j] = v;
 }
 
+__global__ void spectral_live_tiles_kernel(const int32_t* __restrict__ idx, int npts, int64_t gc, int nline, int L,
+                                           unsigned char* __restrict__ live) {
+  const int j = blockIdx.x * blockDim.x + threadIdx.x;
+  if (j >= npts) return;
+  const int64_t p = idx[j];
+  if (p >= 0 && p < gc) live[(int)(p % nline) / L] = 1;
+}
+
 bool spectral_rows_own_supported(isdf_handle h, const int32_t mesh[3], int nb) {
   if (h->own_fft != 2 || !conv_rows_own_supported(mesh, nb)) return false;
   Axis ax[3];
@@ -1145,9 +1155,19 @@
   const PlaneGeo geo = plane_geometry(n1, n2, false);
   const int FX = fast_lines(n0);
   ARG_CHECK(h, geo.bytes && FX >= 1 && (int64_t)nb * n0 < 2147483647LL && nb <= 65535 && (ldx & 1) == 0 && ldx >= 2 * (int64_t)npts);
-  ProfScope ps(h, "spectral_rows_own[byte]", (8.0 * (double)n0 * n1 * n2 + 8.0 * (double)ldx) * nb, 3);
+  const bool skip = h->spectral_skip_lines && npts > 0;
+  ProfScope ps(h, "spectral_rows_own[byte]", (8.0 * (double)n0 * n1 * n2 + 8.0 * (double)ldx) * nb, skip ? 4 : 3);
+  unsigned char* live = nullptr;
+  if (skip) {
+    const int nline = n1 * n2h, ntile = (int)cdiv(nline, FX);
+    live = (unsigned char*)isdf_ws(h, "spectral_live", (size_t)ntile);
+    if (!live) return ISDF_ERR_HIP;
+    HIP_TRY(h, hipMemsetAsync(live, 0, (size_t)ntile, h->stream));
+    spectral_live_tiles_kernel<<<dim3((unsigned)cdiv(npts, 256)), dim3(256), 0, h->stream>>>(d_idx, npts, gc, nline, FX, live);
+    KERNEL_CHECK(h);
+  }
   if (int rc = launch_plane_fwd(h, d_in, zbuf, ax, geo, (int)((int64_t)nb * n0), PIPE_ANY)) return rc;
-  launch_strided<0>(h, true, FX, zbuf, nb, gc, (int64_t)n1 * n2h, n1 * n2h, ax[0], nullptr);
+  launch_strided<0>(h, true, FX, zbuf, nb, gc, (int64_t)n1 * n2h, n1 * n2h, ax[0], nullptr, live);
   const int64_t ldx2 = ldx / 2;
   spectral_pack_kernel<<<dim3((unsigned)cdiv(ldx2, 256), (unsigned)nb), dim3(256), 0, h->stream>>>(zbuf, gc, d_idx, d_scale, npts,
                                                                                                   (double2*)d_out, ldx2);
diff --git a/pyscf_isdf_amd/csrc/gemm_f64.hip b/pyscf_isdf_amd/csrc/gemm_f64.hip
--- a/pyscf_isdf_amd/csrc/gemm_f64.hip
+++ b/pyscf_isdf_amd/csrc/gemm_f64.hip
@@ -34,6 +34,7 @@
   int64_t nunits, nunits_pad;
   double alpha, beta;
   int direct;
+  int upper;
 };
 
 __device__ __forceinline__ int64_t xcd_unit(int64_t nunits_pad) {
@@ -48,6 +49,8 @@
 __device__ __forceinline__ Tile decode_tile(int64_t unit, int ntm, int ntn) {
   return {(int)(unit % ntm), (int)((unit / ntm) % ntn), (int)(unit / ((int64_t)ntm * ntn))};
 }
+
+__host__ __device__ __forceinline__ bool tile_below_diag(int tm, int tn, int TM) { return tm * TM >= (tn + 1) * 128; }
 
 __device__ __forceinline__ KRange slab_range(int slab, int64_t kslab, int64_t K) {
   const int64_t k0 = (int64_t)slab * kslab;
@@ -90,6 +93,7 @@
   const int64_t unit = xcd_unit(g.nunits_pad);
   if (unit >= g.nunits) return;
   const Tile t = decode_tile(unit, g.ntm, g.ntn);
+  if (g.upper && tile_below_diag(t.tm, t.tn, BM)) return;
   const KRange kr = slab_range(t.slab, g.kslab, g.K);
   const int64_t k0 = kr.k0, k1 = kr.k1;
   const int nchunks = (int)((k1 - k0 + BK - 1) / BK);
@@ -290,6 +294,7 @@
   const int64_t unit = xcd_unit(g.nunits_pad);
   if (unit >= g.nunits) return;
   const Tile t = decode_tile(unit, g.ntm, g.ntn);
+  if (g.upper && tile_below_diag(t.tm, t.tn, BM2)) return;
   const KRange kr = slab_range(t.slab, g.kslab, g.K);
   d4 acc[4][4];
   tile_256x128<SCALED>(g.A, g.lda, g.B, g.ldb, g.kscale, g.M, g.N, t.tm, t.tn, kr.k0, (int)((kr.k1 - kr.k0) / BK), smem, acc);
@@ -332,6 +337,7 @@
   const int64_t unit = xcd_unit(g.nunits_pad);
   if (unit >= g.nunits) return;
   const Tile t = decode_tile(unit, g.ntm, g.ntn);
+  if (g.upper && tile_below_diag(t.tm, t.tn, BM)) return;
   const int tm = t.tm, tn = t.tn;
   const KRange kr = slab_range(t.slab, g.kslab, g.K);
   const int64_t k0 = kr.k0;
@@ -725,10 +731,11 @@
 
 __global__ void reduce_slabs_kernel(const double* __restrict__ P, int nslab, int64_t slab_stride,
                                     int M, int N, double alpha, double beta, double* __restrict__ C,
-                                    int64_t ldc) {
+                                    int64_t ldc, int upper_tm = 0) {
   const int64_t idx = (int64_t)blockIdx.x * blockDim.x + threadIdx.x;
   if (idx >= (int64_t)M * N) return;
   const int m = (int)(idx / N), n = (int)(idx % N);
+  if (upper_tm && tile_below_diag(m / upper_tm, n / 128, upper_tm)) return;
   double s = 0.0;
   for (int t = 0; t < nslab; ++t) s += P[(int64_t)t * slab_stride + idx];
   double* q = C + (int64_t)m * ldc + n;
@@ -944,11 +951,12 @@
 
 int gemm_nt_f64_scaled(isdf_handle h, int M, int N, int64_t K, double alpha, const double* A, int64_t lda,
                        const double* B, int64_t ldb, const double* kscale, double beta, double* C,
-                       int64_t ldc) {
+                       int64_t ldc, bool upper) {
   ARG_CHECK(h, M > 0 && N > 0 && K > 0 && A && B && C && lda >= K && ldb >= K && ldc >= N);
   GemmArgs g;
   g.A = A; g.lda = lda; g.B = B; g.ldb = ldb; g.kscale = kscale;
   g.M = M; g.N = N; g.K = K;
+  g.upper = upper ? 1 : 0;
   static const int variant = getenv("ISDF_GEMM_VARIANT") ? atoi(getenv("ISDF_GEMM_VARIANT")) : -1;
   static const int tune = getenv("ISDF_GEMM_SLAB_TUNE") ? atoi(getenv("ISDF_GEMM_SLAB_TUNE")) : 1;
   const bool aligned = rows_aligned16(A, lda) && rows_aligned16(B, ldb) && rows_aligned16(kscale);
@@ -969,10 +977,16 @@
     g.ldp = N; g.slab_stride = (int64_t)M * N;
   }
   ARG_CHECK(h, g.nunits_pad < 2147483647LL);
+  const int TM = useB ? BM2 : BM;
+  double entries = (double)M * N;
+  if (upper)
+    for (int tm = 0; tm < g.ntm; ++tm)
+      for (int tn = 0; tn < g.ntn; ++tn)
+        if (tile_below_diag(tm, tn, TM)) entries -= (double)std::min(TM, M - tm * TM) * std::min(BN, N - tn * BN);
   const char* label = useD ? (kscale ? "gemm_nt_mfma_kernel_d<true>[flop]" : "gemm_nt_mfma_kernel_d<false>[flop]") : useB ? (kscale ? "gemm_nt_mfma_kernel_b<true>[flop]" : "gemm_nt_mfma_kernel_b<false>[flop]")
                            : (fast ? "gemm_nt_mfma_kernel<true>[flop]" : "gemm_nt_mfma_kernel<false>[flop]");
   {
-    ProfScope ps(h, label, 2.0 * M * N * (double)K);
+    ProfScope ps(h, label, 2.0 * entries * (double)K);
     if (useD) {
       if (kscale) hipLaunchKernelGGL(gemm_nt_mfma_kernel_d<true>, dim3((unsigned)g.nunits_pad), dim3(TPBD), 0, h->stream, g);
       else hipLaunchKernelGGL(gemm_nt_mfma_kernel_d<false>, dim3((unsigned)g.nunits_pad), dim3(TPBD), 0, h->stream, g);
@@ -986,9 +1000,9 @@
     KERNEL_CHECK(h);
   }
   if (!g.direct) {
-    ProfScope ps(h, "gemm_reduce_slabs_kernel[byte]", 8.0 * (double)M * N * (g.nslab + 1));
+    ProfScope ps(h, "gemm_reduce_slabs_kernel[byte]", 8.0 * entries * (g.nslab + 1));
     hipLaunchKernelGGL(reduce_slabs_kernel, dim3((unsigned)cdiv((int64_t)M * N, 256)), dim3(256), 0, h->stream,
-                       g.P, g.nslab, g.slab_stride, M, N, alpha, beta, C, ldc);
+                       g.P, g.nslab, g.slab_stride, M, N, alpha, beta, C, ldc, upper ? TM : 0);
     KERNEL_CHECK(h);
   }
   return ISDF_OK;
@@ -1004,6 +1018,13 @@
                             double beta, double* d_C, int64_t ldc) {
   if (!h) return ISDF_ERR_ARG;
   return gemm_nt_f64_scaled(h, M, N, K, alpha, d_A, lda, d_B, ldb, d_kscale, beta, d_C, ldc);
+}
+
+extern "C" int isdf_gemm_nt_upper(isdf_handle h, int M, int N, int64_t K, double alpha, const double* d_A,
+                                  int64_t lda, const double* d_B, int64_t ldb, const double* d_kscale,
+                                  double beta, double* d_C, int64_t ldc) {
+  if (!h) return ISDF_ERR_ARG;
+  return gemm_nt_f64_scaled(h, M, N, K, alpha, d_A, lda, d_B, ldb, d_kscale, beta, d_C, ldc, h->gemm_nt_upper != 0);
 }
 
 extern "C" int isdf_gemm_nt_had3(isdf_handle h, int M, int N, int64_t K, double alpha, const double* d_A, int64_t lda,
diff --git a/pyscf_isdf_amd/csrc/handle.hip b/pyscf_isdf_amd/csrc/handle.hip
--- a/pyscf_isdf_amd/csrc/handle.hip
+++ b/pyscf_isdf_amd/csrc/handle.hip
@@ -112,6 +112,10 @@
   }
   if (std::string(key) == "block_apply_waves") { h->block_apply_waves = value < 1 ? 1 : value; return ISDF_OK; }
   if (std::string(key) == "block_apply_reg") { h->block_apply_reg = value ? 1 : 0; return ISDF_OK; }
+  if (std::string(key) == "gemm_nt_upper") { h->gemm_nt_upper = value ? 1 : 0; return ISDF_OK; }
+  if (std::string(key) == "w_strips_upper") { h->w_strips_upper = value ? 1 : 0; return ISDF_OK; }
+  if (std::string(key) == "j_triangular") { h->j_triangular = value ? 1 : 0; return ISDF_OK; }
+  if (std::string(key) == "spectral_skip_lines") { h->spectral_skip_lines = value ? 1 : 0; return ISDF_OK; }
   return isdf_fail(h, ISDF_ERR_ARG, "isdf_set_option: unknown key '%s'", key);
 }
 
diff --git a/pyscf_isdf_amd/csrc/jk.hip b/pyscf_isdf_amd/csrc/jk.hip
--- a/pyscf_isdf_amd/csrc/jk.hip
+++ b/pyscf_isdf_amd/csrc/jk.hip
@@ -67,12 +67,58 @@
                                const double* d_vR, int nset, int64_t ldv, double* d_vj) {
   if (!h) return ISDF_ERR_ARG;
   ARG_CHECK(h, d_ao && d_vR && d_vj && nao > 0 && ng > 0 && ld >= ng && nset > 0 && ldv >= ng);
+  const bool upper = h->gemm_nt_upper != 0;
   for (int i = 0; i < nset; ++i) {
-    int rc = gemm_nt_f64_scaled(h, nao, nao, ng, 1.0, d_ao, ld, d_ao, ld, d_vR + (int64_t)i * ldv, 0.0,
-                                d_vj + (int64_t)i * nao * nao, nao);
+    double* vj = d_vj + (int64_t)i * nao * nao;
+    int rc = gemm_nt_f64_scaled(h, nao, nao, ng, 1.0, d_ao, ld, d_ao, ld, d_vR + (int64_t)i * ldv, 0.0, vj, nao, upper);
     if (rc) return rc;
-  }
-  return ISDF_OK;
+    if (upper && (rc = mirror_upper(h, vj, nao, nao))) return rc;
+  }
+  return ISDF_OK;
+}
+
+namespace {
+constexpr int JTRI_ROWS = 256;
+
+__global__ void fold_lower_kernel(const double* __restrict__ D, int nao, double* __restrict__ Ls) {
+  const int n = blockIdx.x * blockDim.x + threadIdx.x, m = blockIdx.y;
+  if (n >= nao) return;
+  const double d = D[(int64_t)m * nao + n];
+  Ls[(int64_t)m * nao + n] = n < m ? d + D[(int64_t)n * nao + m] : (n == m ? d : 0.0);
+}
+
+int rho_triangular(isdf_handle h, const double* d_ao, int nao, int64_t ng, int64_t ld, const double* d_dm, int nset,
+                   double* d_rho, int64_t ldrho) {
+  ARG_CHECK(h, d_ao && d_dm && d_rho && nao > 0 && nao <= 65535 && ng > 0 && ld >= ng && nset > 0 && ldrho >= ng);
+  double* T = (double*)isdf_ws(h, "jk_T", sizeof(double) * (size_t)nao * JCHUNK);
+  double* Ls = (double*)isdf_ws(h, "jk_Ls", sizeof(double) * (size_t)nao * nao);
+  if (!T || !Ls) return ISDF_ERR_HIP;
+  for (int i = 0; i < nset; ++i) {
+    hipLaunchKernelGGL(fold_lower_kernel, dim3((unsigned)cdiv(nao, 256), (unsigned)nao), dim3(256), 0, h->stream,
+                       d_dm + (int64_t)i * nao * nao, nao, Ls);
+    KERNEL_CHECK(h);
+    for (int64_t g0 = 0; g0 < ng; g0 += JCHUNK) {
+      const int64_t nc = std::min(JCHUNK, ng - g0);
+      for (int r0 = 0; r0 < nao; r0 += JTRI_ROWS) {
+        const int r1 = std::min(nao, r0 + JTRI_ROWS);
+        int rc = gemm_rm(h, 'N', 'N', r1 - r0, nc, r1, 1.0, Ls + (int64_t)r0 * nao, nao, d_ao + g0, ld, 0.0,
+                         T + (int64_t)r0 * JCHUNK, JCHUNK);
+        if (rc) return rc;
+      }
+      hipLaunchKernelGGL(rho_reduce_kernel, dim3((unsigned)cdiv(nc, 256)), dim3(256), 0, h->stream, T, JCHUNK,
+                         d_ao + g0, ld, nao, nc, d_rho + (int64_t)i * ldrho + g0);
+      KERNEL_CHECK(h);
+    }
+  }
+  return ISDF_OK;
+}
+}
+
+extern "C" int isdf_rho_j(isdf_handle h, const double* d_ao, int nao, int64_t ng, int64_t ld, const double* d_dm, int nset,
+                          double* d_rho, int64_t ldrho) {
+  if (!h) return ISDF_ERR_ARG;
+  return h->j_triangular ? rho_triangular(h, d_ao, nao, ng, ld, d_dm, nset, d_rho, ldrho)
+                         : isdf_rho(h, d_ao, nao, ng, ld, d_dm, nset, d_rho, ldrho);
 }
 
 extern "C" int isdf_get_j(isdf_handle h, const double* d_ao, int nao, int64_t ngrids, int64_t ld,
@@ -82,7 +128,7 @@
   ARG_CHECK(h, mesh && ngrids == (int64_t)mesh[0] * mesh[1] * mesh[2]);
   double* rho = (double*)isdf_ws(h, "jk_rho", sizeof(double) * (size_t)nset * ngrids);
   if (!rho) return ISDF_ERR_HIP;
-  int rc = isdf_rho(h, d_ao, nao, ngrids, ld, d_dm, nset, rho, ngrids);
+  int rc = isdf_rho_j(h, d_ao, nao, ngrids, ld, d_dm, nset, rho, ngrids);
   if (rc) return rc;
   rc = isdf_coulomb_potential(h, rho, nset, ngrids, mesh, a);
   if (rc) return rc;
diff --git a/pyscf_isdf_amd/fit_route.py b/pyscf_isdf_amd/fit_route.py
--- a/pyscf_isdf_amd/fit_route.py
+++ b/pyscf_isdf_amd/fit_route.py
@@ -313,9 +313,10 @@
     def _spectral_W_finish(self, X, W, nbat):
         be, st = self.backend, self._fit_state
         P = W.shape[0]
+        upper = dict(upper=True) if getattr(self, 'w_strips_upper', False) and getattr(be, 'gemm_nt_has_upper', False) else {}
         for b0 in range(0, P, nbat):
             b1 = min(P, b0 + nbat)
-            be.gemm_nt(X[b0:b1], X[b0:], W[b0:b1, b0:], alpha=1.0)
+            be.gemm_nt(X[b0:b1], X[b0:], W[b0:b1, b0:], alpha=1.0, **upper)
         be.symmetrize_upper(W)
         self._bj_finish(st['Afac'], st['Dblk'], st['ip_off'], W)
 
diff --git a/pyscf_isdf_amd/isdf.py b/pyscf_isdf_amd/isdf.py
--- a/pyscf_isdf_amd/isdf.py
+++ b/pyscf_isdf_amd/isdf.py
@@ -42,6 +42,7 @@
         self.w_sphere_tol = 1e-11
         self.w_sort_bins = 256
         self.w_spectral_check_tol = 5e-9
+        self.w_strips_upper = False
         self.w_spectral_max_c = 18
         self.cand_skip_zero_rows = True
         self.cand_gram = True
diff --git a/pyscf_isdf_amd/lib.py b/pyscf_isdf_amd/lib.py
--- a/pyscf_isdf_amd/lib.py
+++ b/pyscf_isdf_amd/lib.py
@@ -69,6 +69,7 @@
     'isdf_symmetrize_mean': (c_int, [c_vp, c_vp, c_int, c_i64, c_int]),
     'isdf_get_j': (c_int, [c_vp, c_vp, c_int, c_i64, c_i64, c_vp, c_vp, c_vp, c_int, c_vp]),
     'isdf_rho': (c_int, [c_vp, c_vp, c_int, c_i64, c_i64, c_vp, c_int, c_vp, c_i64]),
+    'isdf_rho_j': (c_int, [c_vp, c_vp, c_int, c_i64, c_i64, c_vp, c_int, c_vp, c_i64]),
     'isdf_coulomb_potential': (c_int, [c_vp, c_vp, c_int, c_i64, c_vp, c_vp]),
     'isdf_vj_from_vR': (c_int, [c_vp, c_vp, c_int, c_i64, c_i64, c_vp, c_int, c_i64, c_vp]),
     'isdf_eval_ao_k': (c_int, [c_vp, c_vp, c_int, c_vp, c_int, c_vp, c_int, c_vp, c_int, c_vp, c_vp, c_int, c_vp, c_i64, c_vp, c_vp, c_i64]),
@@ -115,6 +116,7 @@
     'isdf_xc_fxc_apply': (c_int, [c_vp, c_int, c_vp, c_i64, c_i64, c_i64, c_vp, c_i64, c_i64, c_int, c_vp, c_i64, c_i64, c_int]),
     'isdf_dot': (c_int, [c_vp, c_vp, c_vp, c_i64, c_vp]),
     'isdf_gemm_nt': (c_int, [c_vp, c_int, c_int, c_i64, c_dbl, c_vp, c_i64, c_vp, c_i64, c_vp, c_dbl, c_vp, c_i64]),
+    'isdf_gemm_nt_upper': (c_int, [c_vp, c_int, c_int, c_i64, c_dbl, c_vp, c_i64, c_vp, c_i64, c_vp, c_dbl, c_vp, c_i64]),
     'isdf_gemm_nt_had3': (c_int, [c_vp, c_int, c_int, c_i64, c_dbl, c_vp, c_i64, c_vp, c_i64, c_vp, c_i64, c_i64, c_dbl, c_vp, c_i64,
                                   c_i64]),
     'isdf_pack_table_pm': (c_int, [c_vp, c_vp, c_vp, c_vp, c_int, c_dbl, c_vp, c_vp, c_i64]),
```

After: 16.59 (median of 6 runs). About the same (-0.8%).
